# qitianwu/SGFormer

Measured on AMD Instinct MI355X. Metric: SGFormer fwd+bwd nodes/sec on ogbn-products full-graph, higher is better.
Workload: dtype bf16

## Files before the change

include/sgf.h:

```cpp
#ifndef SGF_H_
#define SGF_H_

#include <stddef.h>
#include <stdint.h>

#ifdef __cplusplus
extern "C" {
#endif

#define SGF_VERSION 670

#define SGF_F32 0
#define SGF_BF16 1
#define SGF_F32_BF16X3 2

#define SGF_OK 0
#define SGF_E_INVALID (-1)
#define SGF_E_WORKSPACE (-2)
#define SGF_E_HIP (-3)
#define SGF_E_UNSUPPORTED (-4)

int sgf_version(void);
const char* sgf_last_error(void);
int sgf_reload_env(void);

size_t sgf_csr_workspace_bytes(int64_t nnz, int64_t n);
int sgf_csr_build(const int64_t* edge_index, int64_t nnz, int64_t n, int64_t* rowptr,
                  int32_t* colind, float* val, int32_t* deg, void* workspace,
                  size_t workspace_bytes, void* stream);

int sgf_csr_transpose(const int64_t* edge_index, int64_t nnz, int64_t n, const int32_t* deg,
                      const int64_t* rowptr, const int32_t* colind, int64_t* t_rowptr,
                      int32_t* t_colind, float* t_val, int32_t* is_symmetric, void* workspace,
                      size_t workspace_bytes, void* stream);

size_t sgf_subgraph_workspace_bytes(int64_t nnz, int64_t n);
int sgf_subgraph_plan(const int64_t* edge_index, int64_t nnz, int64_t n, const int64_t* subset,
                      int64_t m, int32_t* relabel, int64_t* total, void* workspace,
                      size_t workspace_bytes, void* stream);
int sgf_subgraph_emit(const int64_t* edge_index, int64_t nnz, int64_t n, const int32_t* relabel,
                      int32_t relabel_nodes, int64_t total, int64_t* out, int64_t* out_eid,
                      void* workspace, size_t workspace_bytes, void* stream);

size_t sgf_subgraph_csr_plan_workspace_bytes(int64_t m);
size_t sgf_subgraph_csr_emit_workspace_bytes(int64_t m, int64_t total);
int sgf_subgraph_csr_plan(const int64_t* rowptr, const int32_t* colind, int64_t n, const int64_t* subset, int64_t m,
                          int32_t* local_of, int64_t* rowptr_b, int32_t* deg_b, int64_t* total, void* workspace,
                          size_t workspace_bytes, void* stream);
int sgf_subgraph_csr_emit(const int64_t* rowptr, const int32_t* colind, int64_t n, const int64_t* subset, int64_t m,
                          int32_t* local_of, const int64_t* rowptr_b, const int32_t* deg_b, int64_t total, int32_t* colind_b,
                          float* val_b, int64_t* edge_index_b, void* workspace, size_t workspace_bytes, void* stream);

size_t sgf_graph_prologue_workspace_bytes(int64_t m, int64_t n);
int sgf_graph_prologue_plan(const int64_t* edge_index, int64_t m, int64_t n, int32_t to_undirected,
                            int32_t remove_self_loops, int32_t add_self_loops, int64_t* total,
                            void* workspace, size_t workspace_bytes, void* stream);
int sgf_graph_prologue_emit(int64_t m, int64_t n, int32_t to_undirected, int32_t add_self_loops,
                            int64_t total, int64_t* out, void* workspace, size_t workspace_bytes,
                            void* stream);

int sgf_spmm(const int64_t* rowptr, const int32_t* colind, const float* val, const void* x,
             int64_t ldx, int64_t n_cols, void* y, int64_t ldy, int64_t n_rows, int32_t d,
             int32_t dtype, void* stream);

int32_t sgf_spmm_segment_len(void);
int32_t sgf_spmm_arm(int32_t d, int32_t dtype, int64_t ldx, int64_t ldy, int64_t n_cols, int32_t aligned16,
                     int32_t stream);
size_t sgf_spmm_split_workspace_bytes(int64_t long_segments, int32_t d);
int sgf_spmm_split(const int64_t* rowptr, const int32_t* colind, const float* val, const void* x,
                   int64_t ldx, int64_t n_cols, void* y, int64_t ldy, int64_t n_rows, int32_t d, int32_t dtype,
                   int64_t long_len, int64_t long_segments, void* workspace, size_t workspace_bytes,
                   void* stream);

size_t sgf_spmm_packed_bytes(int64_t n, int32_t slot_bytes);
int32_t sgf_spmm_packed_supported(int32_t d, int32_t dtype, int64_t ldx, int64_t ldy, int64_t n_cols, int32_t aligned16,
                                  int32_t slot_bytes);
int sgf_spmm_packed(const int64_t* rowptr, const int32_t* colind, const float* val, const void* x, int64_t ldx,
                    int64_t n_cols, const void* packed, int32_t slot_bytes, const int32_t* overflow, void* y, int64_t ldy,
                    int64_t n_rows, int32_t d, int32_t dtype, int64_t long_len, int64_t long_segments, void* workspace,
                    size_t workspace_bytes, void* stream);

int sgf_spmm_stream(const int64_t* rowptr, const int32_t* colind, const float* val, const void* x,
                    int64_t ldx, int64_t n_cols, void* y, int64_t ldy, int64_t n_rows, int32_t d, int32_t dtype,
                    int64_t long_len, int64_t long_segments, void* workspace, size_t workspace_bytes,
                    void* stream);

size_t sgf_reorder_workspace_bytes(int64_t nnz, int64_t n);
int sgf_reorder(const int64_t* edge_index, int64_t nnz, int64_t n, int32_t iters1, int32_t iters2,
                int32_t* perm, int32_t* inv, int32_t* community, void* workspace, size_t workspace_bytes,
                void* stream);
size_t sgf_spmm_plan_workspace_bytes(int64_t nnz, int64_t n, int32_t rows_per_block);
int sgf_spmm_plan(const int64_t* rowptr, const int32_t* colind, const float* val, int64_t n, int64_t nnz,
                  int32_t rows_per_block, int32_t lds_rows, int64_t long_len, int32_t* ecode, float* eval,
                  int32_t* nlds, int32_t* sh_ptr, int32_t* sh_cols, int64_t* stats, void* workspace,
                  size_t workspace_bytes, void* stream);
int32_t sgf_spmm_lds_rows_len(int32_t dtype);
int32_t sgf_spmm_blocked_arm(int32_t d, int32_t dtype, int64_t ldx, int64_t ldy, int64_t n_rows, int32_t rows_per_block,
                             int32_t lds_rows, int32_t aligned16);
int sgf_spmm_blocked(const int64_t* rowptr, const int32_t* ecode, const float* eval, const int32_t* nlds,
                     const int32_t* sh_ptr, const int32_t* sh_cols, const void* x, int64_t ldx, void* y,
                     int64_t ldy, int64_t n_rows, int32_t d, int32_t dtype, int32_t rows_per_block,
                     int32_t lds_rows, int64_t long_len, int64_t long_segments, void* workspace,
                     size_t workspace_bytes, void* stream);

int sgf_spmm_tile_supported(int32_t d, int32_t dtype);
int sgf_spmm_tile_blocks(const int32_t* comm_sorted, int64_t n, int32_t max_rows, int32_t* blk_row,
                         int64_t blk_cap, int64_t* nb_out, void* stream);
size_t sgf_spmm_tile_plan_workspace_bytes(int64_t nnz, int64_t n, int64_t nb);
int sgf_spmm_tile_plan(const int64_t* rowptr, const int32_t* colind, const float* val, int64_t n, int64_t nnz,
                       const int32_t* blk_row, int64_t nb, int32_t cap, int32_t min_count, int64_t long_len,
                       int32_t* ecode, float* eval, int32_t* nlds, int32_t* sh_ptr, int32_t* sh_cols,
                       int64_t* tile_ptr, int64_t* rem_rowptr, int64_t* stats, void* workspace,
                       size_t workspace_bytes, void* stream);
int sgf_spmm_tile_fill(const int64_t* rowptr, const int32_t* ecode, const float* eval, const int32_t* nlds,
                       int64_t n, int64_t nnz, const int32_t* blk_row, int64_t nb, const int64_t* tile_ptr,
                       int64_t n_frag, const int64_t* rem_rowptr, void* tiles, int32_t* rem_col, float* rem_val,
                       void* stream);
int32_t sgf_spmm_tile_sparse_len(void);
size_t sgf_spmm_tile_pack_workspace_bytes(int64_t n_frag);
int sgf_spmm_tile_pack_layout(const int32_t* blk_row, int64_t nb, const int64_t* tile_ptr, const void* tiles,
                              int64_t n_frag, int32_t* grp, int64_t* pool_units, void* workspace,
                              size_t workspace_bytes, void* stream);
int sgf_spmm_tile_pack(const int32_t* blk_row, int64_t nb, const int64_t* tile_ptr, const void* tiles, int64_t n_frag,
                       const int32_t* grp, void* pool, int64_t pool_units, void* stream);
int sgf_spmm_tile(const int32_t* blk_row, int64_t nb, int32_t block_rows, const int32_t* sh_ptr, const int32_t* sh_cols,
                  const int64_t* tile_ptr, const int32_t* grp, const void* pool, const int64_t* rem_rowptr,
                  const int32_t* rem_col, const float* rem_val, const void* x, int64_t ldx, int64_t n_cols, void* y, int64_t ldy,
                  int64_t n_rows, int32_t d, int32_t dtype, int64_t long_len, int64_t long_segments,
                  void* workspace, size_t workspace_bytes, void* stream);

size_t sgf_neighbor_sample_workspace_bytes(int64_t m, int64_t edge_cap);
int sgf_neighbor_sample_mark(int32_t* local_of, const int32_t* ids, int64_t count, int32_t base, void* stream);
int sgf_neighbor_sample_hop(const int64_t* rowptr, const int32_t* colind, const int32_t* frontier, int64_t m,
                            int32_t frontier_local0, int32_t fanout, uint64_t seed, uint64_t batch, int32_t hop,
                            int32_t* local_of, int32_t n_known, int64_t edge_cap, int32_t* edge_src_local,
                            int32_t* edge_dst_local, int32_t* src_global, int32_t* new_nodes, int64_t* counts,
                            void* workspace, size_t workspace_bytes, void* stream);

size_t sgf_neighbor_sample_batch_workspace_bytes(int64_t batch_size, const int32_t* fanouts, int32_t hops, int64_t* node_cap,
                                                  int64_t* edge_cap);
int sgf_neighbor_sample_batch(const int64_t* rowptr, const int32_t* colind, const int32_t* seeds, int64_t batch_size,
                              const int32_t* fanouts, int32_t hops, uint64_t seed, uint64_t batch, int32_t* local_of,
                              int32_t* nodes, int64_t node_cap, int32_t* edge_src_local, int32_t* edge_dst_local,
                              int64_t edge_cap, int64_t* counts, void* workspace, size_t workspace_bytes, void* stream);

int32_t sgf_sampled_csr_supported(int32_t max_fanout);
size_t sgf_sampled_csr_build_workspace_bytes(int64_t node_cap, int64_t edge_cap);
int sgf_sampled_csr_build(const int32_t* edge_src_local, const int32_t* edge_dst_local, const int64_t* counts,
                          int64_t node_cap, int64_t edge_cap, int32_t max_fanout, int64_t* rowptr_b, int32_t* colind_b,
                          float* val_b, int32_t* deg_b, void* workspace, size_t workspace_bytes, void* stream);
size_t sgf_sampled_csr_transpose_workspace_bytes(int64_t n, int64_t nnz);
int sgf_sampled_csr_transpose(const int64_t* rowptr, const int32_t* colind, const float* val, int64_t n, int64_t nnz,
                              int64_t* t_rowptr, int32_t* t_colind, float* t_val, void* workspace, size_t workspace_bytes,
                              void* stream);

int sgf_gather_rows(const void* src, int64_t lds, int32_t src_dtype, int64_t n_src, const void* idx,
                    int32_t idx_is_int64, int64_t n_out, int32_t d, void* dst, int64_t ldd,
                    int32_t dst_dtype, void* stream);
int sgf_pad_rows(const void* src, int64_t lds, int32_t src_dtype, int64_t n_src, const void* idx, int32_t idx_is_int64,
                 int64_t n_out, int32_t d, int32_t d_pad, void* dst, int64_t ldd, int32_t dst_dtype, void* stream);

int64_t sgf_attn_stats_len(int32_t heads, int32_t d);
size_t sgf_attn_workspace_bytes(int64_t n, int32_t heads, int32_t d);
int32_t sgf_attn_max_blocks(void);
int32_t sgf_attn_tile_rows(int32_t kind, int32_t d, int32_t dtype);

int sgf_attn_fwd_reduce(const void* q, int64_t ldq, const void* k, int64_t ldk, const void* v,
                        int64_t ldv, int64_t n, int32_t heads, int32_t v_heads, int32_t d,
                        int32_t dtype, float* stats, void* workspace, size_t workspace_bytes,
                        void* stream);

int sgf_attn_fwd_apply(const void* q, int64_t ldq, const void* v, int64_t ldv, int64_t n,
                       double n_total, int32_t heads, int32_t v_heads, int32_t d, int32_t dtype,
                       const float* stats, void* out, int64_t ldo, float* den, void* o_heads,
                       void* stream);

int64_t sgf_attn_bstats_len(int32_t heads, int32_t d);

int sgf_attn_bwd_reduce(const void* q, int64_t ldq, const void* g, int64_t ldg, const void* o,
                        int64_t ldo, const float* den, int64_t n, int32_t heads, int32_t d,
                        int32_t dtype, float* bstats, void* workspace, size_t workspace_bytes,
                        void* stream);

int sgf_attn_bwd_apply(const void* q, int64_t ldq, const void* k, int64_t ldk, const void* v,
                       int64_t ldv, const void* g, int64_t ldg, const void* o, int64_t ldo,
                       const float* den, int64_t n, double n_total, int32_t heads,
                       int32_t v_heads, int32_t d, int32_t dtype, const float* stats,
                       float* bstats, void* dq, int64_t lddq, void* dk, int64_t lddk,
                       void* dv, int64_t lddv, void* stream);
int sgf_attn_bwd_reduce_heads(const void* q, int64_t ldq, const void* g, int64_t ldg, const void* o, int64_t ldo,
                              const float* den, int64_t n, int32_t heads, int32_t d, int32_t dtype, float* bstats,
                              void* workspace, size_t workspace_bytes, void* stream);
int sgf_attn_bwd_apply_heads(const void* q, int64_t ldq, const void* k, int64_t ldk, const void* v, int64_t ldv, const void* g,
                             int64_t ldg, const void* o, int64_t ldo, const float* den, int64_t n, double n_total,
                             int32_t heads, int32_t v_heads, int32_t d, int32_t dtype, const float* stats, float* bstats,
                             void* dq, int64_t lddq, void* dk, int64_t lddk, void* dv, int64_t lddv, void* stream);

int64_t sgf_attn_h_bstats_len(int32_t d);
int32_t sgf_attn_h_supported(int32_t d, int32_t dtype);
int sgf_attn_h_fwd(const void* h, int64_t ldh, int64_t n, int32_t d, int32_t dtype, const float* M,
                   const float* m, const float* w, const float* beta, void* out, int64_t ldo,
                   float* den, void* stream);
int sgf_attn_h_bwd_reduce(const void* h, int64_t ldh, const void* g, int64_t ldg, const void* o,
                          int64_t ldo, const float* den, int64_t n, int32_t d, int32_t dtype,
                          float* hstats, void* workspace, size_t workspace_bytes, void* stream);
int sgf_attn_h_bwd_apply(const void* h, int64_t ldh, const void* g, int64_t ldg, const void* o,
                         int64_t ldo, const float* den, int64_t n, int32_t d, int32_t dtype,
                         const float* M, const float* w, const float* D, const float* ds, void* dh,
                         int64_t lddh, void* workspace, size_t workspace_bytes, void* stream);
size_t sgf_attn_h_bwd_apply_workspace_bytes(int64_t n, int32_t d, int32_t dtype);
int32_t sgf_attn_h_bwd_split_supported(int32_t d, int32_t dtype);
int sgf_attn_h_bwd_pre(const void* g, int64_t ldg, const void* o, int64_t ldo, const float* den, int64_t n, int32_t d,
                       int32_t dtype, const float* M, const float* w, void* workspace, size_t workspace_bytes,
                       float* rowscal, void* stream);
int sgf_attn_h_bwd_reduce_scaled(const void* h, int64_t ldh, const void* g, int64_t ldg, const float* rowscal, int64_t n,
                                 int32_t d, int32_t dtype, float* hstats, void* workspace, size_t workspace_bytes,
                                 void* stream);
int sgf_attn_h_bwd_post(const void* h, int64_t ldh, int64_t n, int32_t d, int32_t dtype, const float* D, const float* ds,
                        const void* workspace, size_t workspace_bytes, const void* addend, int64_t ldadd, void* dh,
                        int64_t lddh, void* stream);

size_t sgf_attn_h_small_saved_bytes(int32_t d_in, int32_t d_out);
size_t sgf_attn_h_small_workspace_bytes(int32_t d_in, int32_t d_out);
int sgf_attn_h_small_fwd(const float* G, int64_t ldg, const float* s, float n_rows, float n_total, const float* wq,
                         const float* bq, const float* wk, const float* bk, const float* wv, const float* bv, int64_t ldw,
                         int32_t d_in, int32_t d_out, float* M, int64_t ldm, float* m, float* w, float* beta, void* saved,
                         size_t saved_bytes, void* stream);
int sgf_attn_h_small_bwd(const float* dM, int64_t lddm, const float* dw, const float* dm, const float* dbeta, float n_total,
                         int32_t d_in, int32_t d_out, const void* saved, size_t saved_bytes, float* dG2, int64_t lddg,
                         float* ds, float* gwq, float* gbq, float* gwk, float* gbk, float* gwv, float* gbv, int64_t ldgw,
                         void* workspace, size_t workspace_bytes, void* stream);

size_t sgf_gram_workspace_bytes(int64_t n, int32_t m, int32_t k);
int sgf_gram(const void* a, int64_t lda, int32_t m, const void* b, int64_t ldb, int32_t k,
             int64_t n, int32_t dtype, float* c, int64_t ldc, float* colsum_a, void* workspace,
             size_t workspace_bytes, void* stream);
int sgf_gram2(const void* a, int64_t lda, int32_t m, const void* b1, int64_t ldb1, const void* b2, int64_t ldb2, int32_t k,
              int64_t n, int32_t dtype, float* c1, int64_t ldc1, float* c2, int64_t ldc2, float* colsum_a, void* workspace,
              size_t workspace_bytes, void* stream);

int sgf_ln_fwd(const void* x, int64_t ldx, const void* res, int64_t ldr, float a, float b,
               const float* gamma, const float* beta, int32_t relu, float eps, int64_t n,
               int32_t d, int32_t dtype, void* y, int64_t ldy, float* mean, float* rstd,
               void* stream);

size_t sgf_ln_bwd_workspace_bytes(int64_t n, int32_t d);
int sgf_ln_bwd(const void* dy, int64_t lddy, const void* y, int64_t ldy, const void* x,
               int64_t ldx, const void* res, int64_t ldr, float a, float b, const float* gamma,
               int32_t relu, const float* mean, const float* rstd, int64_t n, int32_t d,
               int32_t dtype, void* dx, int64_t lddx, void* dres, int64_t lddres, float* dgamma,
               float* dbeta, void* workspace, size_t workspace_bytes, void* stream);

size_t sgf_colstats_workspace_bytes(int64_t n, int32_t d);
int sgf_colstats(const void* x, int64_t ldx, const float* shift, int64_t n, int32_t d,
                 int32_t dtype, float* stats, void* workspace, size_t workspace_bytes,
                 void* stream);
int sgf_bn_finalize(const float* sums, const float* shift, double n_total, float eps, float momentum, float* running_mean,
                    float* running_var, int32_t d, float* mean, float* rstd, void* stream);
int sgf_bn_apply(const void* x, int64_t ldx, const float* mean, const float* rstd,
                 const float* gamma, const float* beta, const void* res, int64_t ldr,
                 int32_t relu, int64_t n, int32_t d, int32_t dtype, void* y, int64_t ldy,
                 void* stream);
int sgf_bn_apply_packed(const void* x, int64_t ldx, const float* mean, const float* rstd, const float* gamma,
                        const float* beta, const void* res, int64_t ldr, int32_t relu, int64_t n, int32_t d, int32_t dtype,
                        void* y, int64_t ldy, void* packed, int32_t slot_bytes, int32_t* overflow, void* stream);
int sgf_bn_bwd_stats(const void* dy, int64_t lddy, const void* x, int64_t ldx, const float* mean,
                     const float* rstd, const float* gamma, const float* beta, int32_t relu,
                     int64_t n, int32_t d, int32_t dtype, float* stats, void* workspace,
                     size_t workspace_bytes, void* stream);
int sgf_bn_bwd_stats2(const void* dy, int64_t lddy, const void* dy2, int64_t lddy2, const void* x, int64_t ldx,
                      const float* mean, const float* rstd, const float* gamma, const float* beta, int32_t relu, int64_t n,
                      int32_t d, int32_t dtype, float* stats, void* workspace, size_t workspace_bytes, void* stream);
int32_t sgf_gram_ln_bwd_supported(int32_t m, int32_t k, int32_t dtype);
int sgf_gram_ln_bwd(const void* g, int64_t ldg, const void* xin, int64_t ldx, const float* mean, const float* rstd,
                    const float* gamma, const float* beta, int32_t relu, int32_t m, const void* b, int64_t ldb, int32_t k,
                    int64_t n, int32_t dtype, float* c, int64_t ldc, float* colsum, float* dgamma, float* dbeta, void* workspace,
                    size_t workspace_bytes, void* stream);
int32_t sgf_gram_bn_bwd_supported(int32_t m, int32_t k, int32_t dtype);
int sgf_gram_bn_bwd(const void* g1, int64_t ldg1, const void* g2, int64_t ldg2, const void* z, int64_t ldz, const float* mean,
                    const float* rstd, const float* gamma, const float* beta, int32_t relu, const float* stats, float inv_n,
                    int32_t training, int32_t m, const void* b, int64_t ldb, int32_t k, int64_t n, int32_t dtype, float* c,
                    int64_t ldc, float* colsum, void* workspace, size_t workspace_bytes, void* stream);
int32_t sgf_gram2_bn_bwd_supported(int32_t m, int32_t k, int64_t n, int32_t dtype);
int sgf_gram2_bn_bwd(const void* g, int64_t ldg, const void* z, int64_t ldz, const float* mean, const float* rstd,
                     const float* gamma, const float* beta, int32_t relu, const float* stats, float inv_n, int32_t training,
                     int32_t m, const void* b1, int64_t ldb1, const void* b2, int64_t ldb2, int32_t k, int64_t n, int32_t dtype,
                     void* dz, int64_t lddz, float* c1, int64_t ldc1, float* c2, int64_t ldc2, float* colsum, void* workspace,
                     size_t workspace_bytes, void* stream);
int sgf_bn_bwd_apply(const void* dy, int64_t lddy, const void* x, int64_t ldx, const float* mean,
                     const float* rstd, const float* gamma, const float* beta, int32_t relu,
                     const float* stats, float inv_n, int32_t training, int64_t n, int32_t d,
                     int32_t dtype, void* dx, int64_t lddx, void* stream);

int32_t sgf_combine_fc_supported(int32_t d, int32_t classes, int32_t dtype);
int sgf_combine_fc_fwd(const void* x1, int64_t ld1, float a, const void* x2, int64_t ld2, float b,
                       const float* w, const float* bias, int64_t n, int32_t d, int32_t classes,
                       int32_t dtype, float* logits, int64_t ldl, void* stream);
int sgf_combine_fc_bwd(const float* dlogits, int64_t lddl, const float* w, int64_t n, int32_t d,
                       int32_t classes, float a, float b, int32_t dtype, void* dx1, int64_t ld1, void* dx2,
                       int64_t ld2, void* stream);
int sgf_combine_fc_fwd_mapped(const void* x1, int64_t ld1, float a, const void* x2, int64_t ld2, float b, const float* w,
                              const float* bias, int64_t n, int32_t d, int32_t classes, int32_t dtype, float* logits,
                              int64_t ldl, const int32_t* row_map, void* stream);
int sgf_combine_fc_bwd_mapped(const float* dlogits, int64_t lddl, const float* w, int64_t n, int32_t d, int32_t classes,
                              float a, float b, int32_t dtype, void* dx1, int64_t ld1, void* dx2, int64_t ld2,
                              const int32_t* row_map, void* stream);
int sgf_combine_fc_bwd_g(const float* dlogits, int64_t lddl, const float* w, int64_t n, int32_t d, int32_t classes, float a,
                         float b, int32_t dtype, void* dx1, int64_t ld1, void* dx2, int64_t ld2, const int32_t* row_map,
                         void* g_out, int64_t ldg, void* stream);

int32_t sgf_gcn_epilogue_supported(int32_t d_in, int32_t d_out, int32_t dtype);
size_t sgf_gcn_epilogue_workspace_bytes(int64_t n, int32_t d_out);
int sgf_gcn_epilogue_stats(const void* a, int64_t lda, const void* w, int64_t ldw, const float* bias,
                           int64_t n, int32_t d_in, int32_t d_out, int32_t dtype, void* y, int64_t ldy,
                           const float* shift, float* stats, void* workspace, size_t workspace_bytes,
                           void* stream);
int sgf_gcn_epilogue_dx2(const void* dy, int64_t lddy, const void* w1, const void* w2, int64_t ldw, int64_t n, int32_t d,
                         int32_t dtype, void* dx1, int64_t lddx1, void* dx2, int64_t lddx2, int32_t pair, void* stream);

int32_t sgf_gcn_epilogue_dx2_acc_supported(int32_t d, int32_t dtype);
int sgf_gcn_epilogue_dx2_acc(const void* dz, int64_t lddz, const void* w, int64_t ldw, int64_t n, int32_t d, int32_t dtype,
                             void* dy, int64_t lddy, const void* gadd, int64_t ldg, const void* acc_in, int64_t ldai,
                             void* acc_out, int64_t ldao, void* stream);
int sgf_gcn_epilogue_dx(const void* dy, int64_t lddy, const void* w, int64_t ldw, int64_t n, int32_t d_in,
                        int32_t d_out, int32_t dtype, void* dx, int64_t lddx, void* stream);
int sgf_gcn_epilogue_apply(const void* y, int64_t ldy, const float* mean, const float* rstd, const float* gamma,
                           const float* beta, const void* res, int64_t ldr, int32_t relu, int64_t n, int32_t d,
                           int32_t dtype, void* out, int64_t ldo, void* stream);
int32_t sgf_gcn_bn_bwd_dx_supported(int32_t d, int32_t dtype);
size_t sgf_gcn_bn_bwd_dx_workspace_bytes(int64_t n, int32_t d);
int sgf_gcn_bn_bwd_dx(const void* gy, int64_t ldg, const void* z, int64_t ldz, const float* mean, const float* rstd,
                      const float* gamma, const float* beta, int32_t relu, const float* stats, float inv_n,
                      int32_t training, const void* w, int64_t ldw, int64_t n, int32_t d, int32_t dtype, void* dz,
                      int64_t lddz, void* dy, int64_t lddy, const void* acc_in, void* acc_out, size_t acc_bytes,
                      void* dx0, int64_t lddx0, int32_t add_gy, void* workspace, size_t workspace_bytes, void* stream);
int32_t sgf_gcn_epilogue_cat_supported(int32_t d, int32_t dtype);
int sgf_gcn_epilogue_cat(const void* a1, int64_t lda1, const void* a2, int64_t lda2, const void* w, int64_t ldw,
                         const float* bias, int64_t n, int32_t d, int32_t dtype, void* y, int64_t ldy, const float* shift,
                         float* stats, void* workspace, size_t workspace_bytes, void* stream);
size_t sgf_gcn_epilogue_partial_bytes(int64_t n, int32_t d_out);
size_t sgf_gcn_epilogue_dtype_partial_bytes(int64_t n, int32_t d_out, int32_t dtype);
int sgf_gcn_epilogue_partial(const void* a, int64_t lda, const void* w, int64_t ldw, const float* bias, int64_t n,
                             int32_t d_in, int32_t d_out, int32_t dtype, void* partial, size_t partial_bytes,
                             void* stream);
int sgf_gcn_epilogue_stats_add(const void* a, int64_t lda, const void* w, int64_t ldw, const void* partial,
                               size_t partial_bytes, int64_t n, int32_t d_in, int32_t d_out, int32_t dtype,
                               void* y, int64_t ldy, const float* shift, float* stats, void* workspace,
                               size_t workspace_bytes, void* stream);

int32_t sgf_stem_pair_supported(int32_t d_in, int32_t d_out, int32_t dtype);
int32_t sgf_row_lap_rows(int32_t kind, int32_t d, int32_t dtype);
int sgf_stem_pair(const void* x, int64_t ldx, int64_t n, int32_t d_in, const void* w0, int64_t ldw0,
                  const float* bias0, const void* w1, int64_t ldw1, const float* bias1, int32_t d_out, int32_t dtype,
                  void* y0, int64_t ldy0, void* y1, int64_t ldy1, const float* shift0, float* stats0, void* workspace,
                  size_t workspace_bytes, void* stream);

int sgf_gemm(const void* a, int64_t a_rs, int64_t a_cs, int32_t a_dtype, const void* b, int64_t b_rs, int64_t b_cs,
             int32_t b_dtype, int64_t m, int32_t n, int64_t k, float alpha, const float* alpha_dev, const float* bias,
             float beta, const void* addend, int64_t ldadd, int32_t add_dtype, void* c, int64_t ldc, int32_t c_dtype,
             void* stream);

int sgf_axpby(const void* x1, int64_t ld1, float a, const void* x2, int64_t ld2, float b,
              int64_t n, int32_t d, int32_t dtype, void* y, int64_t ldy, void* stream);

int sgf_dropout(const void* x, int64_t ldx, const void* res, int64_t ldr, float p, uint64_t seed,
                int64_t n, int32_t d, int32_t dtype, void* y, int64_t ldy, void* stream);

int sgf_dropout_dev(const void* x, int64_t ldx, const void* res, int64_t ldr, float p,
                    const uint64_t* seed_slot, int64_t n, int32_t d, int32_t dtype, void* y, int64_t ldy,
                    void* stream);

size_t sgf_nll_workspace_bytes(int64_t m);
int sgf_nll_fwd(const void* logits, int64_t ldl, int64_t n, int32_t c, int32_t dtype,
                const int64_t* labels, const int64_t* idx, int64_t m, float* loss_sum,
                void* workspace, size_t workspace_bytes, void* stream);
int sgf_nll_bwd(const void* logits, int64_t ldl, int64_t n, int32_t c, int32_t dtype,
                const int64_t* labels, const int64_t* idx, int64_t m, const float* gout,
                float inv_denom, void* dlogits, int64_t ldd, void* stream);

#define SGF_BCE_TARGET_F32 0
#define SGF_BCE_TARGET_I64 1
#define SGF_BCE_TARGET_CLASS 2
size_t sgf_bce_workspace_bytes(int64_t m, int32_t c);
// ... 130 lines not shown
```

sgformer_amd/_lib.py:

```python
from __future__ import annotations

import ctypes
import os
from ctypes import c_char_p, c_double, c_float, c_int32, c_int64, c_size_t, c_uint64, c_void_p

_HERE = os.path.dirname(os.path.abspath(__file__))
LIB_PATH = os.path.join(_HERE, "lib", "libsgf.so")

SGF_F32 = 0
SGF_BF16 = 1
SGF_F32_BF16X3 = 2
SGF_OK = 0
SGF_E_INVALID = -1
SGF_E_WORKSPACE = -2
SGF_E_HIP = -3
SGF_E_UNSUPPORTED = -4
SGF_BCE_TARGET_F32 = 0
SGF_BCE_TARGET_I64 = 1
SGF_BCE_TARGET_CLASS = 2
SGF_METRIC_TARGET_F32 = 0
SGF_METRIC_TARGET_I64 = 1

_lib = None

_P = c_void_p
SIGNATURES = {
    "sgf_version": (c_int32, []),
    "sgf_last_error": (c_char_p, []),
    "sgf_reload_env": (c_int32, []),
    "sgf_csr_workspace_bytes": (c_size_t, [c_int64, c_int64]),
    "sgf_csr_build": (c_int32, [_P, c_int64, c_int64, _P, _P, _P, _P, _P, c_size_t, _P]),
    "sgf_csr_transpose": (c_int32, [_P, c_int64, c_int64, _P, _P, _P, _P, _P, _P, _P, _P, c_size_t, _P]),
    "sgf_subgraph_workspace_bytes": (c_size_t, [c_int64, c_int64]),
    "sgf_subgraph_plan": (c_int32, [_P, c_int64, c_int64, _P, c_int64, _P, _P, _P, c_size_t, _P]),
    "sgf_subgraph_emit": (c_int32, [_P, c_int64, c_int64, _P, c_int32, c_int64, _P, _P, _P, c_size_t, _P]),
    "sgf_subgraph_csr_plan_workspace_bytes": (c_size_t, [c_int64]),
    "sgf_subgraph_csr_emit_workspace_bytes": (c_size_t, [c_int64, c_int64]),
    "sgf_subgraph_csr_plan": (c_int32, [_P, _P, c_int64, _P, c_int64, _P, _P, _P, _P, _P, c_size_t, _P]),
    "sgf_subgraph_csr_emit": (c_int32, [_P, _P, c_int64, _P, c_int64, _P, _P, _P, c_int64, _P, _P, _P, _P, c_size_t, _P]),
    "sgf_graph_prologue_workspace_bytes": (c_size_t, [c_int64, c_int64]),
    "sgf_graph_prologue_plan": (c_int32, [_P, c_int64, c_int64, c_int32, c_int32, c_int32, _P, _P, c_size_t, _P]),
    "sgf_graph_prologue_emit": (c_int32, [c_int64, c_int64, c_int32, c_int32, c_int64, _P, _P, c_size_t, _P]),
    "sgf_spmm": (c_int32, [_P, _P, _P, _P, c_int64, c_int64, _P, c_int64, c_int64, c_int32, c_int32, _P]),
    "sgf_spmm_segment_len": (c_int32, []),
    "sgf_spmm_arm": (c_int32, [c_int32, c_int32, c_int64, c_int64, c_int64, c_int32, c_int32]),
    "sgf_spmm_split_workspace_bytes": (c_size_t, [c_int64, c_int32]),
    "sgf_spmm_split": (c_int32, [_P, _P, _P, _P, c_int64, c_int64, _P, c_int64, c_int64, c_int32, c_int32, c_int64,
                                 c_int64, _P, c_size_t, _P]),
    "sgf_spmm_packed_bytes": (c_size_t, [c_int64, c_int32]),
    "sgf_spmm_packed_supported": (c_int32, [c_int32, c_int32, c_int64, c_int64, c_int64, c_int32, c_int32]),
    "sgf_spmm_packed": (c_int32, [_P, _P, _P, _P, c_int64, c_int64, _P, c_int32, _P, _P, c_int64, c_int64, c_int32, c_int32,
                                  c_int64, c_int64, _P, c_size_t, _P]),
    "sgf_spmm_stream": (c_int32, [_P, _P, _P, _P, c_int64, c_int64, _P, c_int64, c_int64, c_int32, c_int32, c_int64,
                                  c_int64, _P, c_size_t, _P]),
    "sgf_reorder_workspace_bytes": (c_size_t, [c_int64, c_int64]),
    "sgf_reorder": (c_int32, [_P, c_int64, c_int64, c_int32, c_int32, _P, _P, _P, _P, c_size_t, _P]),
    "sgf_spmm_plan_workspace_bytes": (c_size_t, [c_int64, c_int64, c_int32]),
    "sgf_spmm_plan": (c_int32, [_P, _P, _P, c_int64, c_int64, c_int32, c_int32, c_int64, _P, _P, _P, _P, _P, _P,
                                _P, c_size_t, _P]),
    "sgf_spmm_lds_rows_len": (c_int32, [c_int32]),
    "sgf_spmm_blocked_arm": (c_int32, [c_int32, c_int32, c_int64, c_int64, c_int64, c_int32, c_int32, c_int32]),
    "sgf_spmm_blocked": (c_int32, [_P, _P, _P, _P, _P, _P, _P, c_int64, _P, c_int64, c_int64, c_int32, c_int32,
                                   c_int32, c_int32, c_int64, c_int64, _P, c_size_t, _P]),
    "sgf_spmm_tile_supported": (c_int32, [c_int32, c_int32]),
    "sgf_spmm_tile_blocks": (c_int32, [_P, c_int64, c_int32, _P, c_int64, _P, _P]),
    "sgf_spmm_tile_plan_workspace_bytes": (c_size_t, [c_int64, c_int64, c_int64]),
    "sgf_spmm_tile_plan": (c_int32, [_P, _P, _P, c_int64, c_int64, _P, c_int64, c_int32, c_int32, c_int64, _P, _P, _P,
                                     _P, _P, _P, _P, _P, _P, c_size_t, _P]),
    "sgf_spmm_tile_fill": (c_int32, [_P, _P, _P, _P, c_int64, c_int64, _P, c_int64, _P, c_int64, _P, _P, _P, _P, _P]),
    "sgf_spmm_tile_sparse_len": (c_int32, []),
    "sgf_spmm_tile_pack_workspace_bytes": (c_size_t, [c_int64]),
    "sgf_spmm_tile_pack_layout": (c_int32, [_P, c_int64, _P, _P, c_int64, _P, _P, _P, c_size_t, _P]),
    "sgf_spmm_tile_pack": (c_int32, [_P, c_int64, _P, _P, c_int64, _P, _P, c_int64, _P]),
    "sgf_spmm_tile": (c_int32, [_P, c_int64, c_int32, _P, _P, _P, _P, _P, _P, _P, _P, _P, c_int64, c_int64, _P, c_int64,
                                c_int64, c_int32, c_int32, c_int64, c_int64, _P, c_size_t, _P]),
    "sgf_neighbor_sample_workspace_bytes": (c_size_t, [c_int64, c_int64]),
    "sgf_neighbor_sample_mark": (c_int32, [_P, _P, c_int64, c_int32, _P]),
    "sgf_neighbor_sample_batch_workspace_bytes": (c_size_t, [c_int64, _P, c_int32, _P, _P]),
    "sgf_neighbor_sample_batch": (c_int32, [_P, _P, _P, c_int64, _P, c_int32, c_uint64, c_uint64, _P, _P, c_int64, _P, _P,
                                            c_int64, _P, _P, c_size_t, _P]),
    "sgf_neighbor_sample_hop": (c_int32, [_P, _P, _P, c_int64, c_int32, c_int32, c_uint64, c_uint64, c_int32, _P, c_int32,
                                          c_int64, _P, _P, _P, _P, _P, _P, c_size_t, _P]),
    "sgf_sampled_csr_supported": (c_int32, [c_int32]),
    "sgf_sampled_csr_build_workspace_bytes": (c_size_t, [c_int64, c_int64]),
    "sgf_sampled_csr_build": (c_int32, [_P, _P, _P, c_int64, c_int64, c_int32, _P, _P, _P, _P, _P, c_size_t, _P]),
    "sgf_sampled_csr_transpose_workspace_bytes": (c_size_t, [c_int64, c_int64]),
    "sgf_sampled_csr_transpose": (c_int32, [_P, _P, _P, c_int64, c_int64, _P, _P, _P, _P, c_size_t, _P]),
    "sgf_gather_rows": (c_int32, [_P, c_int64, c_int32, c_int64, _P, c_int32, c_int64, c_int32, _P, c_int64,
                                  c_int32, _P]),
    "sgf_pad_rows": (c_int32, [_P, c_int64, c_int32, c_int64, _P, c_int32, c_int64, c_int32, c_int32, _P, c_int64,
                               c_int32, _P]),
    "sgf_attn_stats_len": (c_int64, [c_int32, c_int32]),
    "sgf_attn_bstats_len": (c_int64, [c_int32, c_int32]),
    "sgf_attn_workspace_bytes": (c_size_t, [c_int64, c_int32, c_int32]),
    "sgf_attn_max_blocks": (c_int32, []),
    "sgf_attn_tile_rows": (c_int32, [c_int32, c_int32, c_int32]),
    "sgf_row_lap_rows": (c_int32, [c_int32, c_int32, c_int32]),
    "sgf_ew_lap_rows": (c_int64, [c_int32, c_int32, c_int32, c_int32]),
    "sgf_attn_fwd_reduce": (c_int32, [_P, c_int64, _P, c_int64, _P, c_int64, c_int64, c_int32, c_int32,
                                      c_int32, c_int32, _P, _P, c_size_t, _P]),
    "sgf_attn_fwd_apply": (c_int32, [_P, c_int64, _P, c_int64, c_int64, c_double, c_int32, c_int32,
                                     c_int32, c_int32, _P, _P, c_int64, _P, _P, _P]),
    "sgf_attn_bwd_reduce": (c_int32, [_P, c_int64, _P, c_int64, _P, c_int64, _P, c_int64, c_int32,
                                      c_int32, c_int32, _P, _P, c_size_t, _P]),
    "sgf_attn_bwd_apply": (c_int32, [_P, c_int64, _P, c_int64, _P, c_int64, _P, c_int64, _P, c_int64,
                                     _P, c_int64, c_double, c_int32, c_int32, c_int32, c_int32, _P, _P,
                                     _P, c_int64, _P, c_int64, _P, c_int64, _P]),
    "sgf_attn_bwd_reduce_heads": (c_int32, [_P, c_int64, _P, c_int64, _P, c_int64, _P, c_int64, c_int32,
                                            c_int32, c_int32, _P, _P, c_size_t, _P]),
    "sgf_attn_bwd_apply_heads": (c_int32, [_P, c_int64, _P, c_int64, _P, c_int64, _P, c_int64, _P, c_int64,
                                           _P, c_int64, c_double, c_int32, c_int32, c_int32, c_int32, _P, _P,
                                           _P, c_int64, _P, c_int64, _P, c_int64, _P]),
    "sgf_attn_h_bstats_len": (c_int64, [c_int32]),
    "sgf_attn_h_fwd": (c_int32, [_P, c_int64, c_int64, c_int32, c_int32, _P, _P, _P, _P, _P, c_int64, _P, _P]),
    "sgf_attn_h_bwd_reduce": (c_int32, [_P, c_int64, _P, c_int64, _P, c_int64, _P, c_int64, c_int32, c_int32,
                                        _P, _P, c_size_t, _P]),
    "sgf_attn_h_bwd_apply": (c_int32, [_P, c_int64, _P, c_int64, _P, c_int64, _P, c_int64, c_int32, c_int32,
                                       _P, _P, _P, _P, _P, c_int64, _P, c_size_t, _P]),
    "sgf_attn_h_bwd_apply_workspace_bytes": (c_size_t, [c_int64, c_int32, c_int32]),
    "sgf_attn_h_bwd_split_supported": (c_int32, [c_int32, c_int32]),
    "sgf_attn_h_supported": (c_int32, [c_int32, c_int32]),
    "sgf_attn_h_bwd_pre": (c_int32, [_P, c_int64, _P, c_int64, _P, c_int64, c_int32, c_int32, _P, _P, _P, c_size_t, _P, _P]),
    "sgf_attn_h_bwd_reduce_scaled": (c_int32, [_P, c_int64, _P, c_int64, _P, c_int64, c_int32, c_int32, _P, _P, c_size_t,
                                               _P]),
    "sgf_attn_h_bwd_post": (c_int32, [_P, c_int64, c_int64, c_int32, c_int32, _P, _P, _P, c_size_t, _P, c_int64, _P,
                                      c_int64, _P]),
    "sgf_attn_h_small_saved_bytes": (c_size_t, [c_int32, c_int32]),
    "sgf_attn_h_small_workspace_bytes": (c_size_t, [c_int32, c_int32]),
    "sgf_attn_h_small_fwd": (c_int32, [_P, c_int64, _P, c_float, c_float, _P, _P, _P, _P, _P, _P, c_int64, c_int32, c_int32,
                                       _P, c_int64, _P, _P, _P, _P, c_size_t, _P]),
    "sgf_attn_h_small_bwd": (c_int32, [_P, c_int64, _P, _P, _P, c_float, c_int32, c_int32, _P, c_size_t, _P, c_int64, _P,
                                       _P, _P, _P, _P, _P, _P, c_int64, _P, c_size_t, _P]),
    "sgf_gram_workspace_bytes": (c_size_t, [c_int64, c_int32, c_int32]),
    "sgf_gram": (c_int32, [_P, c_int64, c_int32, _P, c_int64, c_int32, c_int64, c_int32, _P, c_int64, _P,
                           _P, c_size_t, _P]),
    "sgf_gram2": (c_int32, [_P, c_int64, c_int32, _P, c_int64, _P, c_int64, c_int32, c_int64, c_int32, _P, c_int64, _P,
                            c_int64, _P, _P, c_size_t, _P]),
    "sgf_ln_fwd": (c_int32, [_P, c_int64, _P, c_int64, c_float, c_float, _P, _P, c_int32, c_float,
                             c_int64, c_int32, c_int32, _P, c_int64, _P, _P, _P]),
    "sgf_ln_bwd_workspace_bytes": (c_size_t, [c_int64, c_int32]),
    "sgf_ln_bwd": (c_int32, [_P, c_int64, _P, c_int64, _P, c_int64, _P, c_int64, c_float, c_float, _P,
                             c_int32, _P, _P, c_int64, c_int32, c_int32, _P, c_int64, _P, c_int64, _P,
                             _P, _P, c_size_t, _P]),
    "sgf_colstats_workspace_bytes": (c_size_t, [c_int64, c_int32]),
    "sgf_colstats": (c_int32, [_P, c_int64, _P, c_int64, c_int32, c_int32, _P, _P, c_size_t, _P]),
    "sgf_bn_finalize": (c_int32, [_P, _P, c_double, c_float, c_float, _P, _P, c_int32, _P, _P, _P]),
    "sgf_bn_apply": (c_int32, [_P, c_int64, _P, _P, _P, _P, _P, c_int64, c_int32, c_int64, c_int32,
                               c_int32, _P, c_int64, _P]),
    "sgf_bn_apply_packed": (c_int32, [_P, c_int64, _P, _P, _P, _P, _P, c_int64, c_int32, c_int64, c_int32, c_int32, _P,
                                      c_int64, _P, c_int32, _P, _P]),
    "sgf_bn_bwd_stats": (c_int32, [_P, c_int64, _P, c_int64, _P, _P, _P, _P, c_int32, c_int64, c_int32,
                                   c_int32, _P, _P, c_size_t, _P]),
    "sgf_bn_bwd_stats2": (c_int32, [_P, c_int64, _P, c_int64, _P, c_int64, _P, _P, _P, _P, c_int32, c_int64, c_int32,
                                    c_int32, _P, _P, c_size_t, _P]),
    "sgf_gram_ln_bwd_supported": (c_int32, [c_int32, c_int32, c_int32]),
    "sgf_gram_ln_bwd": (c_int32, [_P, c_int64, _P, c_int64, _P, _P, _P, _P, c_int32, c_int32, _P, c_int64, c_int32, c_int64,
                                  c_int32, _P, c_int64, _P, _P, _P, _P, c_size_t, _P]),
    "sgf_gram_bn_bwd_supported": (c_int32, [c_int32, c_int32, c_int32]),
    "sgf_gram_bn_bwd": (c_int32, [_P, c_int64, _P, c_int64, _P, c_int64, _P, _P, _P, _P, c_int32, _P, c_float, c_int32,
                                  c_int32, _P, c_int64, c_int32, c_int64, c_int32, _P, c_int64, _P, _P, c_size_t, _P]),
    "sgf_gram2_bn_bwd_supported": (c_int32, [c_int32, c_int32, c_int64, c_int32]),
    "sgf_gram2_bn_bwd": (c_int32, [_P, c_int64, _P, c_int64, _P, _P, _P, _P, c_int32, _P, c_float, c_int32, c_int32, _P, c_int64,
                                   _P, c_int64, c_int32, c_int64, c_int32, _P, c_int64, _P, c_int64, _P, c_int64, _P, _P,
                                   c_size_t, _P]),
    "sgf_bn_bwd_apply": (c_int32, [_P, c_int64, _P, c_int64, _P, _P, _P, _P, c_int32, _P, c_float,
                                   c_int32, c_int64, c_int32, c_int32, _P, c_int64, _P]),
    "sgf_dropout": (c_int32, [_P, c_int64, _P, c_int64, c_float, c_uint64, c_int64, c_int32, c_int32, _P,
                              c_int64, _P]),
    "sgf_dropout_dev": (c_int32, [_P, c_int64, _P, c_int64, c_float, _P, c_int64, c_int32, c_int32, _P,
                                  c_int64, _P]),
    "sgf_nll_workspace_bytes": (c_size_t, [c_int64]),
    "sgf_nll_fwd": (c_int32, [_P, c_int64, c_int64, c_int32, c_int32, _P, _P, c_int64, _P, _P, c_size_t, _P]),
    "sgf_nll_bwd": (c_int32, [_P, c_int64, c_int64, c_int32, c_int32, _P, _P, c_int64, _P, c_float, _P,
                              c_int64, _P]),
    "sgf_bce_workspace_bytes": (c_size_t, [c_int64, c_int32]),
    "sgf_bce_fwd": (c_int32, [_P, c_int64, c_int64, c_int32, c_int32, _P, c_int64, c_int32, _P, c_int64, c_float, _P, _P,
                              c_size_t, _P]),
    "sgf_bce_bwd": (c_int32, [_P, c_int64, c_int64, c_int32, c_int32, _P, c_int64, c_int32, _P, c_int64, _P, c_float, _P,
                              c_int64, _P]),
    "sgf_rocauc_workspace_bytes": (c_size_t, [c_int64, c_int32]),
    "sgf_rocauc_counts": (c_int32, [_P, c_int64, c_int64, c_int32, c_int32, _P, c_int64, c_int32, _P, c_int64, _P, _P,
                                    c_size_t, _P]),
    "sgf_argmax_workspace_bytes": (c_size_t, [c_int64, c_int32]),
    "sgf_argmax_count": (c_int32, [_P, c_int64, c_int64, c_int32, c_int32, _P, c_int64, c_int32, _P, c_int64, _P, _P,
                                   c_size_t, _P]),
    "sgf_head_rows_supported": (c_int32, [c_int32, c_int32, c_int32]),
    "sgf_head_rows_fwd_workspace_bytes": (c_size_t, [c_int64]),
    "sgf_head_rows_bwd_workspace_bytes": (c_size_t, [c_int64, c_int32, c_int32]),
    "sgf_head_rows_fwd": (c_int32, [_P, c_int64, c_float, _P, c_int64, c_float, _P, _P, c_int64, c_int32, c_int32, c_int32,
                                    _P, c_int64, _P, c_int64, _P, _P, _P, _P, _P, c_size_t, _P]),
    "sgf_head_rows_bwd": (c_int32, [_P, c_int64, c_float, _P, c_int64, c_float, _P, c_int64, c_int32, c_int32, c_int32,
                                    _P, c_int64, _P, c_int64, _P, c_int64, _P, _P, _P, c_float, _P, c_int64, _P, c_int64,
                                    _P, _P, _P, c_size_t, _P]),
    "sgf_pair_sigmoid_supported": (c_int32, [c_int32, c_int32, c_int32, c_int32]),
    "sgf_pair_sigmoid_workspace_bytes": (c_size_t, [c_int64, c_int64, c_int32]),
    "sgf_pair_sigmoid_lap_rows": (c_int64, [c_int32, c_int32, c_int32, c_int32, c_int32]),
    "sgf_pair_sigmoid_fwd": (c_int32, [_P, c_int64, _P, c_int64, _P, c_int64, c_int64, c_int64, c_int32, c_int32, c_int32,
                                       c_int32, _P, c_int64, _P, _P]),
    "sgf_pair_sigmoid_bwd_q": (c_int32, [_P, c_int64, _P, c_int64, _P, _P, c_int64, _P, c_int64, _P, c_int64, c_int64,
                                         c_int64, c_int32, c_int32, c_int32, c_int32, _P, c_int64, _P, c_size_t, _P]),
    "sgf_pair_sigmoid_bwd_kv": (c_int32, [_P, c_int64, _P, _P, c_int64, _P, c_int64, _P, c_int64, c_int64, c_int64, c_int32,
                                          c_int32, c_int32, c_int32, _P, c_int64, _P, c_int64, _P, c_size_t, _P]),
    "sgf_pair_softmax_supported": (c_int32, [c_int32, c_int32, c_int32, c_int32]),
    "sgf_pair_softmax_workspace_bytes": (c_size_t, [c_int64, c_int64, c_int32]),
    "sgf_pair_softmax_lap_rows": (c_int64, [c_int32, c_int32, c_int32, c_int32, c_int32]),
    "sgf_pair_softmax_fwd": (c_int32, [_P, c_int64, _P, c_int64, _P, c_int64, c_int64, c_int64, c_int32, c_int32, c_int32,
                                       c_int32, c_float, _P, c_int64, _P, _P]),
    "sgf_pair_softmax_bwd_q": (c_int32, [_P, c_int64, _P, c_int64, _P, _P, c_int64, _P, c_int64, _P, c_int64, c_int64,
                                         c_int64, c_int32, c_int32, c_int32, c_int32, c_float, _P, c_int64, _P, c_size_t,
                                         _P]),
    "sgf_pair_softmax_bwd_kv": (c_int32, [_P, c_int64, _P, _P, c_int64, _P, c_int64, _P, c_int64, c_int64, c_int64, c_int32,
                                          c_int32, c_int32, c_int32, c_float, _P, c_int64, _P, c_int64, _P, c_size_t, _P]),
    "sgf_pair_sigmoid_x3_supported": (c_int32, [c_int32, c_int32, c_int32, c_int32]),
    "sgf_pair_sigmoid_x3_lap_rows": (c_int64, [c_int32, c_int32, c_int32, c_int32, c_int32]),
    "sgf_pair_sigmoid_x3_fwd": (c_int32, [_P, c_int64, _P, c_int64, _P, c_int64, c_int64, c_int64, c_int32, c_int32, c_int32,
                                          c_int32, _P, c_int64, _P, _P]),
    "sgf_pair_sigmoid_x3_bwd_q": (c_int32, [_P, c_int64, _P, c_int64, _P, _P, c_int64, _P, c_int64, _P, c_int64, c_int64,
                                            c_int64, c_int32, c_int32, c_int32, c_int32, _P, c_int64, _P, c_size_t, _P]),
    "sgf_pair_sigmoid_x3_bwd_kv": (c_int32, [_P, c_int64, _P, _P, c_int64, _P, c_int64, _P, c_int64, c_int64, c_int64, c_int32,
                                             c_int32, c_int32, c_int32, _P, c_int64, _P, c_int64, _P, c_size_t, _P]),
    "sgf_pair_softmax_x3_supported": (c_int32, [c_int32, c_int32, c_int32, c_int32]),
    "sgf_pair_softmax_x3_lap_rows": (c_int64, [c_int32, c_int32, c_int32, c_int32, c_int32]),
    "sgf_pair_softmax_x3_fwd": (c_int32, [_P, c_int64, _P, c_int64, _P, c_int64, c_int64, c_int64, c_int32, c_int32, c_int32,
                                          c_int32, c_float, _P, c_int64, _P, _P]),
    "sgf_pair_softmax_x3_bwd_q": (c_int32, [_P, c_int64, _P, c_int64, _P, _P, c_int64, _P, c_int64, _P, c_int64, c_int64,
                                            c_int64, c_int32, c_int32, c_int32, c_int32, c_float, _P, c_int64, _P, c_size_t,
                                            _P]),
    "sgf_pair_softmax_x3_bwd_kv": (c_int32, [_P, c_int64, _P, _P, c_int64, _P, c_int64, _P, c_int64, c_int64, c_int64, c_int32,
                                             c_int32, c_int32, c_int32, c_float, _P, c_int64, _P, c_int64, _P, c_size_t, _P]),
    "sgf_gat_supported": (c_int32, [c_int32, c_int32, c_int32]),
    "sgf_gat_lap_rows": (c_int64, [c_int32, c_int32, c_int32, c_int32]),
    "sgf_gat_scores": (c_int32, [_P, c_int64, _P, _P, c_int64, c_int32, c_int32, c_int32, _P, _P, _P]),
    "sgf_gat_fwd": (c_int32, [_P, _P, _P, c_int64, _P, _P, _P, c_int64, c_int64, c_int32, c_int32, c_int32, c_int32, c_float,
                              c_float, c_uint64, _P, c_int64, _P, _P, _P]),
    "sgf_gat_bwd_dst": (c_int32, [_P, _P, _P, c_int64, _P, c_int64, _P, _P, _P, c_int64, c_int64, c_int32, c_int32, c_int32,
                                  c_int32, c_float, c_float, c_uint64, _P, _P, _P]),
    "sgf_gat_bwd_src": (c_int32, [_P, _P, _P, c_int64, _P, c_int64, _P, _P, _P, _P, _P, _P, _P, c_int64, c_int64, c_int32,
                                  c_int32, c_int32, c_int32, c_float, c_float, c_uint64, _P, _P, c_int64, _P]),
    "sgf_sum_n": (c_int32, [_P, _P, c_int32, c_int64, c_int32, c_int32, _P, c_int64, _P]),
    "sgf_colsum_workspace_bytes": (c_size_t, [c_int64, c_int32]),
    "sgf_colsum": (c_int32, [_P, c_int64, c_int64, c_int32, c_int32, _P, _P, c_size_t, _P]),
    "sgf_combine_fc_supported": (c_int32, [c_int32, c_int32, c_int32]),
    "sgf_combine_fc_fwd": (c_int32, [_P, c_int64, c_float, _P, c_int64, c_float, _P, _P, c_int64, c_int32, c_int32,
                                     c_int32, _P, c_int64, _P]),
    "sgf_combine_fc_bwd": (c_int32, [_P, c_int64, _P, c_int64, c_int32, c_int32, c_float, c_float, c_int32, _P,
                                     c_int64, _P, c_int64, _P]),
    "sgf_combine_fc_fwd_mapped": (c_int32, [_P, c_int64, c_float, _P, c_int64, c_float, _P, _P, c_int64, c_int32, c_int32,
                                     c_int32, _P, c_int64, _P, _P]),
    "sgf_combine_fc_bwd_g": (c_int32, [_P, c_int64, _P, c_int64, c_int32, c_int32, c_float, c_float, c_int32, _P, c_int64, _P,
                                       c_int64, _P, _P, c_int64, _P]),
    "sgf_combine_fc_bwd_mapped": (c_int32, [_P, c_int64, _P, c_int64, c_int32, c_int32, c_float, c_float, c_int32, _P,
                                     c_int64, _P, c_int64, _P, _P]),
    "sgf_gcn_epilogue_supported": (c_int32, [c_int32, c_int32, c_int32]),
    "sgf_gcn_epilogue_workspace_bytes": (c_size_t, [c_int64, c_int32]),
    "sgf_gcn_epilogue_stats": (c_int32, [_P, c_int64, _P, c_int64, _P, c_int64, c_int32, c_int32, c_int32, _P, c_int64,
                                         _P, _P, _P, c_size_t, _P]),
    "sgf_gcn_epilogue_dx": (c_int32, [_P, c_int64, _P, c_int64, c_int64, c_int32, c_int32, c_int32, _P, c_int64, _P]),
    "sgf_gcn_epilogue_dx2": (c_int32, [_P, c_int64, _P, _P, c_int64, c_int64, c_int32, c_int32, _P, c_int64, _P, c_int64,
                                       c_int32, _P]),
    "sgf_gcn_epilogue_dx2_acc_supported": (c_int32, [c_int32, c_int32]),
    "sgf_gcn_epilogue_dx2_acc": (c_int32, [_P, c_int64, _P, c_int64, c_int64, c_int32, c_int32, _P, c_int64, _P, c_int64, _P,
                                           c_int64, _P, c_int64, _P]),
    "sgf_gcn_epilogue_apply": (c_int32, [_P, c_int64, _P, _P, _P, _P, _P, c_int64, c_int32, c_int64, c_int32,
                               c_int32, _P, c_int64, _P]),
    "sgf_gcn_bn_bwd_dx_supported": (c_int32, [c_int32, c_int32]),
    "sgf_gcn_bn_bwd_dx_workspace_bytes": (c_size_t, [c_int64, c_int32]),
    "sgf_gcn_bn_bwd_dx": (c_int32, [_P, c_int64, _P, c_int64, _P, _P, _P, _P, c_int32, _P, c_float, c_int32, _P, c_int64,
                                    c_int64, c_int32, c_int32, _P, c_int64, _P, c_int64, _P, _P, c_size_t, _P, c_int64,
                                    c_int32, _P, c_size_t, _P]),
    "sgf_gcn_epilogue_cat_supported": (c_int32, [c_int32, c_int32]),
    "sgf_gcn_epilogue_cat": (c_int32, [_P, c_int64, _P, c_int64, _P, c_int64, _P, c_int64, c_int32, c_int32, _P, c_int64,
                                       _P, _P, _P, c_size_t, _P]),
    "sgf_gcn_epilogue_partial_bytes": (c_size_t, [c_int64, c_int32]),
    "sgf_gcn_epilogue_dtype_partial_bytes": (c_size_t, [c_int64, c_int32, c_int32]),
    "sgf_gcn_epilogue_partial": (c_int32, [_P, c_int64, _P, c_int64, _P, c_int64, c_int32, c_int32, c_int32, _P,
                                           c_size_t, _P]),
    "sgf_gcn_epilogue_stats_add": (c_int32, [_P, c_int64, _P, c_int64, _P, c_size_t, c_int64, c_int32, c_int32,
                                             c_int32, _P, c_int64, _P, _P, _P, c_size_t, _P]),
    "sgf_stem_pair_supported": (c_int32, [c_int32, c_int32, c_int32]),
    "sgf_stem_pair": (c_int32, [_P, c_int64, c_int64, c_int32, _P, c_int64, _P, _P, c_int64, _P, c_int32, c_int32, _P,
                                c_int64, _P, c_int64, _P, _P, _P, c_size_t, _P]),
    "sgf_gemm": (c_int32, [_P, c_int64, c_int64, c_int32, _P, c_int64, c_int64, c_int32, c_int64, c_int32, c_int64, c_float,
                           _P, _P, c_float, _P, c_int64, c_int32, _P, c_int64, c_int32, _P]),
    "sgf_comm_available": (c_int32, []),
    "sgf_comm_unique_id_bytes": (c_int32, []),
    "sgf_comm_unique_id": (c_int32, [_P]),
    "sgf_comm_create": (c_int32, [_P, c_int32, c_int32, _P]),
    "sgf_comm_destroy": (c_int32, [_P]),
    "sgf_comm_all_reduce_f32": (c_int32, [_P, _P, c_int64, _P]),
    "sgf_comm_all_gather": (c_int32, [_P, _P, _P, c_int64, _P]),
    "sgf_comm_all_to_all": (c_int32, [_P, _P, _P, _P, _P, _P, _P, _P]),
    "sgf_axpby": (c_int32, [_P, c_int64, c_float, _P, c_int64, c_float, c_int64, c_int32, c_int32, _P,
                            c_int64, _P]),
}


class SgfError(RuntimeError):
    """A libsgf call returned a non-zero status (mirrors PyTorch: RuntimeError)."""


def load():
    global _lib
    if _lib is not None:
        return _lib
    if not os.path.exists(LIB_PATH):
        raise SgfError(
            f"libsgf.so not found at {LIB_PATH}: build it with `make` (or "
            "`python -c 'import __graft_entry__ as g; g.build()'`).  sgformer_amd has no CPU / "
            "eager fallback by design.")
    import torch
    lib = ctypes.CDLL(LIB_PATH, mode=ctypes.RTLD_GLOBAL)
    for name, (res, args) in SIGNATURES.items():
        fn = getattr(lib, name)
        fn.restype = res
        fn.argtypes = args
    _lib = lib
    return lib


def available() -> bool:
    return os.path.exists(LIB_PATH)


def check(rc: int, what: str):
    if rc != SGF_OK:
        msg = load().sgf_last_error()
        raise SgfError(f"{what} failed (rc={rc}): {msg.decode() if msg else '?'}")


def call(name: str, *args):
    rc = getattr(load(), name)(*args)
    check(rc, name)
```

sgformer_amd/csrc/spmm.hip:

```cpp
#include "common.h"
#include "spmm_shared.h"

#include <climits>
#include <cstdlib>

namespace sgf {
namespace {

constexpr int kWavesPerBlock = 4;

__device__ __forceinline__ void fma4(float4& acc, float v, const float4& x) {
  acc.x = fmaf(v, x.x, acc.x);
  acc.y = fmaf(v, x.y, acc.y);
  acc.z = fmaf(v, x.z, acc.z);
  acc.w = fmaf(v, x.w, acc.w);
}

template <typename T, int UNROLL>
__global__ __launch_bounds__(kWavesPerBlock * 64) void k_spmm_wave(
    const int64_t* __restrict__ rowptr, const int32_t* __restrict__ colind,
    const float* __restrict__ val, const T* __restrict__ x, int64_t ldx, T* __restrict__ y,
    int64_t ldy, int64_t n_rows, int32_t d, LongQueue lq) {
  const int lane = threadIdx.x & 63;
  const int wid = __builtin_amdgcn_readfirstlane(static_cast<int>(threadIdx.x >> 6));
  const int64_t blk = xcd_remap(blockIdx.x, gridDim.x);
  const int64_t row = blk * kWavesPerBlock + wid;
  if (row >= n_rows) return;
  const int64_t e0 = rowptr[row];
  const int64_t e1 = rowptr[row + 1];
  if (e1 - e0 > lq.long_len) {
    push_long_row(lq, row, e1 - e0, lane, 64);
    return;
  }

  for (int f0 = 0; f0 < d; f0 += 256) {
    const int fc = f0 + lane * 4;
    const bool active = fc < d;
    const T* xl = x + (active ? fc : 0);
    float4 acc = make_float4(0.f, 0.f, 0.f, 0.f);
    int64_t e = e0;
    for (; e + UNROLL <= e1; e += UNROLL) {
      int32_t c[UNROLL];
      float v[UNROLL];
      float4 xv[UNROLL];
#pragma unroll
      for (int u = 0; u < UNROLL; ++u) {
        c[u] = colind[e + u];
        v[u] = val[e + u];
      }
#pragma unroll
      for (int u = 0; u < UNROLL; ++u)
        xv[u] = load4<T>(xl + static_cast<int64_t>(c[u]) * ldx);
#pragma unroll
      for (int u = 0; u < UNROLL; ++u) fma4(acc, v[u], xv[u]);
    }
    for (; e < e1; ++e) {
      const int32_t c = colind[e];
      const float v = val[e];
      const float4 xv = load4<T>(xl + static_cast<int64_t>(c) * ldx);
      fma4(acc, v, xv);
    }
    if (active) store4<T>(y + row * ldy + fc, acc);
  }
}

template <typename T> struct BufRow;
template <> struct BufRow<uint16_t> {
  using Raw = u32x2;
  static __device__ __forceinline__ Raw load(__amdgpu_buffer_rsrc_t r, int voff, uint32_t soff) {
    return __builtin_amdgcn_raw_buffer_load_b64(r, voff, static_cast<int>(soff), 0);
  }
  static __device__ __forceinline__ float4 widen(const Raw& v) {
    float4 f;
    f.x = __uint_as_float(v.x << 16);
    f.y = __uint_as_float(v.x & 0xffff0000u);
    f.z = __uint_as_float(v.y << 16);
    f.w = __uint_as_float(v.y & 0xffff0000u);
    return f;
  }
};
template <> struct BufRow<float> {
  using Raw = u32x4;
  static __device__ __forceinline__ Raw load(__amdgpu_buffer_rsrc_t r, int voff, uint32_t soff) {
    return __builtin_amdgcn_raw_buffer_load_b128(r, voff, static_cast<int>(soff), 0);
  }
  static __device__ __forceinline__ float4 widen(const Raw& v) {
    return make_float4(__uint_as_float(v.x), __uint_as_float(v.y), __uint_as_float(v.z), __uint_as_float(v.w));
  }
};

template <typename T, int N>
__device__ __forceinline__ void gather_batch(__amdgpu_buffer_rsrc_t rsrc, int voff, uint32_t pitch,
                                             const int32_t* __restrict__ colind, const float* __restrict__ val,
                                             int e, float4& acc) {
  int32_t c[N];
  float v[N];
  typename BufRow<T>::Raw raw[N];
#pragma unroll
  for (int u = 0; u < N; ++u) {
    c[u] = colind[e + u];
    v[u] = val[e + u];
  }
#pragma unroll
  for (int u = 0; u < N; ++u) raw[u] = BufRow<T>::load(rsrc, voff, static_cast<uint32_t>(c[u]) * pitch);
#pragma unroll
  for (int u = 0; u < N; ++u) fma4(acc, v[u], BufRow<T>::widen(raw[u]));
}

template <typename T, int UNROLL>
__global__ __launch_bounds__(kWavesPerBlock * 64) void k_spmm_row(
    const int64_t* __restrict__ rowptr, const int32_t* __restrict__ colind, const float* __restrict__ val,
    const T* __restrict__ x, uint32_t pitch, uint32_t x_bytes, T* __restrict__ y, int64_t ldy, int64_t n_rows,
    int32_t d, LongQueue lq) {
  const int lane = threadIdx.x & 63;
  const int wid = __builtin_amdgcn_readfirstlane(static_cast<int>(threadIdx.x >> 6));
  const int64_t blk = xcd_remap(blockIdx.x, gridDim.x);
  const int64_t row = blk * kWavesPerBlock + wid;
  if (row >= n_rows) return;
  const int64_t e0 = rowptr[row];
  const int64_t e1 = rowptr[row + 1];
  if (e1 - e0 > lq.long_len) {
    push_long_row(lq, row, e1 - e0, lane, 64);
    return;
  }
  const __amdgpu_buffer_rsrc_t rsrc = __builtin_amdgcn_make_buffer_rsrc(const_cast<T*>(x), 0, x_bytes, 0x00020000);
  const int fc = lane * 4;
  const bool active = fc < d;
  const int voff = active ? fc * static_cast<int>(sizeof(T)) : 0;
  float4 acc = make_float4(0.f, 0.f, 0.f, 0.f);
  const int32_t* __restrict__ ci = colind + e0;
  const float* __restrict__ va = val + e0;
  const int len = static_cast<int>(e1 - e0);
  int i = 0;
  if (UNROLL <= len) {
    int32_t c0[UNROLL], c1[UNROLL];
    float v0[UNROLL], v1[UNROLL];
    typename BufRow<T>::Raw raw[UNROLL];
#pragma unroll
    for (int u = 0; u < UNROLL; ++u) {
      c0[u] = ci[u];
      v0[u] = va[u];
    }
    for (;;) {
#pragma unroll
      for (int u = 0; u < UNROLL; ++u) raw[u] = BufRow<T>::load(rsrc, voff, static_cast<uint32_t>(c0[u]) * pitch);
      i += UNROLL;
      const bool more_a = i + UNROLL <= len;
      if (more_a) {
#pragma unroll
        for (int u = 0; u < UNROLL; ++u) {
          c1[u] = ci[i + u];
          v1[u] = va[i + u];
        }
      }
#pragma unroll
      for (int u = 0; u < UNROLL; ++u) fma4(acc, v0[u], BufRow<T>::widen(raw[u]));
      if (!more_a) break;
#pragma unroll
      for (int u = 0; u < UNROLL; ++u) raw[u] = BufRow<T>::load(rsrc, voff, static_cast<uint32_t>(c1[u]) * pitch);
      i += UNROLL;
      const bool more_b = i + UNROLL <= len;
      if (more_b) {
#pragma unroll
        for (int u = 0; u < UNROLL; ++u) {
          c0[u] = ci[i + u];
          v0[u] = va[i + u];
        }
      }
#pragma unroll
      for (int u = 0; u < UNROLL; ++u) fma4(acc, v1[u], BufRow<T>::widen(raw[u]));
      if (!more_b) break;
    }
  }
  if (i + 4 <= len) { gather_batch<T, 4>(rsrc, voff, pitch, ci, va, i, acc); i += 4; }
  if (i + 2 <= len) { gather_batch<T, 2>(rsrc, voff, pitch, ci, va, i, acc); i += 2; }
  if (i < len) gather_batch<T, 1>(rsrc, voff, pitch, ci, va, i, acc);
  if (active) store4<T>(y + row * ldy + fc, acc);
}

typedef uint32_t u32x3 __attribute__((ext_vector_type(3)));
constexpr int kPackedMaskBytes = 32;
constexpr int kPackedTail = 128;

struct DenseRowLoader {
  static constexpr bool kAhead = false;
  __amdgpu_buffer_rsrc_t rsrc;
  int voff;
  uint32_t pitch;
  template <int N> struct Batch { u32x2 raw[N]; };
  template <int N> __device__ __forceinline__ void request(Batch<N>& b, const int32_t (&c)[N]) const {
#pragma unroll
    for (int u = 0; u < N; ++u) b.raw[u] = BufRow<uint16_t>::load(rsrc, voff, static_cast<uint32_t>(c[u]) * pitch);
  }
  template <int N> __device__ __forceinline__ void follow(Batch<N>&) const {}
  template <int N> __device__ __forceinline__ void apply(const Batch<N>& b, const float (&v)[N], float4& acc) const {
#pragma unroll
    for (int u = 0; u < N; ++u) fma4(acc, v[u], BufRow<uint16_t>::widen(b.raw[u]));
  }
};

template <int S>
struct PackedRowLoader {
  static constexpr bool kAhead = true;
  __amdgpu_buffer_rsrc_t rsrc;
  int mask_voff;
  int shift;
  uint32_t below;
  const uint4* lut;
  template <int N> struct Batch {
    uint32_t slot[N], mw[N], pre[N];
    u32x3 raw[N];
  };
  template <int N> __device__ __forceinline__ void request(Batch<N>& b, const int32_t (&c)[N]) const {
#pragma unroll
    for (int u = 0; u < N; ++u) {
      b.slot[u] = static_cast<uint32_t>(c[u]) * static_cast<uint32_t>(S);
      b.mw[u] = __builtin_amdgcn_raw_buffer_load_b32(rsrc, mask_voff, static_cast<int>(b.slot[u]), 0);
    }
  }
  template <int N> __device__ __forceinline__ void follow(Batch<N>& b) const {
#pragma unroll
    for (int u = 0; u < N; ++u) {
      const int t = __popc(b.mw[u]);
      int s = t + __builtin_amdgcn_update_dpp(0, t, 0x118, 0xf, 0xf, true);
      s += __builtin_amdgcn_update_dpp(0, s, 0x142, 0xa, 0xf, false);
      s += __builtin_amdgcn_update_dpp(0, s, 0x143, 0xc, 0xf, false);
      b.pre[u] = static_cast<uint32_t>(s - t) + __popc(b.mw[u] & below);
      const uint32_t off = ((b.pre[u] & ~1u) << 1) + (b.slot[u] + kPackedMaskBytes);
      b.raw[u] = __builtin_amdgcn_raw_buffer_load_b96(rsrc, static_cast<int>(off), 0, 0);
    }
  }
  template <int N> __device__ __forceinline__ void apply(const Batch<N>& b, const float (&v)[N], float4& acc) const {
#pragma unroll
    for (int u = 0; u < N; ++u) {
      const uint4 sel = lut[(b.mw[u] >> shift) & 15u];
      const uint32_t sh = b.pre[u] << 4;
      const uint32_t lo = __builtin_amdgcn_alignbit(b.raw[u].y, b.raw[u].x, sh);
      const uint32_t hi = __builtin_amdgcn_alignbit(b.raw[u].z, b.raw[u].y, sh);
      float4 f;
      f.x = __uint_as_float(__builtin_amdgcn_perm(hi, lo, sel.x));
      f.y = __uint_as_float(__builtin_amdgcn_perm(hi, lo, sel.y));
      f.z = __uint_as_float(__builtin_amdgcn_perm(hi, lo, sel.z));
      f.w = __uint_as_float(__builtin_amdgcn_perm(hi, lo, sel.w));
      fma4(acc, v[u], f);
    }
  }
};

template <int N, typename L>
__device__ __forceinline__ void gather_batch_with(const L& ld, const int32_t* __restrict__ colind,
                                                  const float* __restrict__ val, int e, float4& acc) {
  int32_t c[N];
  float v[N];
  typename L::template Batch<N> b;
#pragma unroll
  for (int u = 0; u < N; ++u) {
    c[u] = colind[e + u];
    v[u] = val[e + u];
  }
  ld.request(b, c);
  ld.follow(b);
  ld.apply(b, v, acc);
}

template <int UNROLL, typename L>
__device__ __forceinline__ float4 walk_row(const L& ld, const int32_t* __restrict__ ci, const float* __restrict__ va, int len) {
  float4 acc = make_float4(0.f, 0.f, 0.f, 0.f);
  int i = 0;
  if (UNROLL <= len) {
    int32_t c0[UNROLL], c1[UNROLL];
    float v0[UNROLL], v1[UNROLL];
    typename L::template Batch<UNROLL> ba, bb;
#pragma unroll
    for (int u = 0; u < UNROLL; ++u) {
      c0[u] = ci[u];
      v0[u] = va[u];
    }
    ld.request(ba, c0);
    for (;;) {
      i += UNROLL;
      const bool more_a = i + UNROLL <= len;
      if (more_a) {
#pragma unroll
        for (int u = 0; u < UNROLL; ++u) {
          c1[u] = ci[i + u];
          v1[u] = va[i + u];
        }
      }
      ld.follow(ba);
      if (L::kAhead && more_a) ld.request(bb, c1);
      ld.apply(ba, v0, acc);
      if (!more_a) break;
      if (!L::kAhead) ld.request(bb, c1);
      i += UNROLL;
      const bool more_b = i + UNROLL <= len;
      if (more_b) {
#pragma unroll
        for (int u = 0; u < UNROLL; ++u) {
          c0[u] = ci[i + u];
          v0[u] = va[i + u];
        }
      }
      ld.follow(bb);
      if (L::kAhead && more_b) ld.request(ba, c0);
      ld.apply(bb, v1, acc);
      if (!more_b) break;
      if (!L::kAhead) ld.request(ba, c0);
    }
  }
  if (i + 4 <= len) { gather_batch_with<4>(ld, ci, va, i, acc); i += 4; }
  if (i + 2 <= len) { gather_batch_with<2>(ld, ci, va, i, acc); i += 2; }
  if (i < len) gather_batch_with<1>(ld, ci, va, i, acc);
  return acc;
}

template <int S, int UNROLL>
__global__ __launch_bounds__(kWavesPerBlock * 64) void k_spmm_row_packed(
    const int64_t* __restrict__ rowptr, const int32_t* __restrict__ colind, const float* __restrict__ val,
    const uint16_t* __restrict__ x, uint32_t pitch, uint32_t x_bytes, const void* __restrict__ packed, uint32_t packed_bytes,
    const int32_t* __restrict__ overflow, uint16_t* __restrict__ y, int64_t ldy, int64_t n_rows, LongQueue lq) {
  __shared__ uint4 lut[16];
  if (threadIdx.x < 16) {
    uint32_t s[4];
#pragma unroll
    for (int k = 0; k < 4; ++k) {
      const uint32_t i = __popc(threadIdx.x & ((1u << k) - 1u));
      s[k] = (threadIdx.x >> k) & 1u ? ((2u * i + 1u) << 24) | ((2u * i) << 16) | 0x0c0cu : 0x0c0c0c0cu;
    }
    lut[threadIdx.x] = make_uint4(s[0], s[1], s[2], s[3]);
  }
  __syncthreads();
  const int lane = threadIdx.x & 63;
  const int wid = __builtin_amdgcn_readfirstlane(static_cast<int>(threadIdx.x >> 6));
  const int64_t blk = xcd_remap(blockIdx.x, gridDim.x);
  const int64_t row = blk * kWavesPerBlock + wid;
  if (row >= n_rows) return;
  const int64_t e0 = rowptr[row];
  const int64_t e1 = rowptr[row + 1];
  if (e1 - e0 > lq.long_len) {
    push_long_row(lq, row, e1 - e0, lane, 64);
    return;
  }
  const int32_t* __restrict__ ci = colind + e0;
  const float* __restrict__ va = val + e0;
  const int len = static_cast<int>(e1 - e0);
  float4 acc;
  if (*overflow == 0) {
    PackedRowLoader<S> ld;
    ld.rsrc = __builtin_amdgcn_make_buffer_rsrc(const_cast<void*>(packed), 0, packed_bytes, 0x00020000);
    ld.mask_voff = (lane >> 3) * 4;
    ld.shift = (lane & 7) * 4;
    ld.below = (1u << ld.shift) - 1u;
    ld.lut = lut;
    acc = walk_row<UNROLL>(ld, ci, va, len);
  } else {
    DenseRowLoader ld;
    ld.rsrc = __builtin_amdgcn_make_buffer_rsrc(const_cast<uint16_t*>(x), 0, x_bytes, 0x00020000);
    ld.voff = lane * 8;
    ld.pitch = pitch;
    acc = walk_row<UNROLL>(ld, ci, va, len);
  }
  store4<uint16_t>(y + row * ldy + lane * 4, acc);
}

constexpr int kSegRows = 4;

template <typename T, int G>
__global__ __launch_bounds__(kWavesPerBlock * 64) void k_spmm_seg(
    const int64_t* __restrict__ rowptr, const int32_t* __restrict__ colind, const float* __restrict__ val,
    const T* __restrict__ x, uint32_t pitch, uint32_t x_bytes, T* __restrict__ y, int64_t ldy, int64_t n_rows,
    int32_t d, int32_t chunk_blocks, LongQueue lq) {
  using Raw = typename BufRow<T>::Raw;
  const int lane = threadIdx.x & 63;
  const int wid = __builtin_amdgcn_readfirstlane(static_cast<int>(threadIdx.x >> 6));
  const int64_t blk = xcd_remap(blockIdx.x, gridDim.x, chunk_blocks);
  const int64_t r_first = (blk * kWavesPerBlock + wid) * kSegRows;
  if (r_first >= n_rows) return;
  const int nr = n_rows - r_first < kSegRows ? static_cast<int>(n_rows - r_first) : kSegRows;
  const __amdgpu_buffer_rsrc_t rsrc = __builtin_amdgcn_make_buffer_rsrc(const_cast<T*>(x), 0, x_bytes, 0x00020000);
  const int fc = lane * 4;
  const bool active = fc < d;
  const int voff = active ? fc * static_cast<int>(sizeof(T)) : 0;
  T* __restrict__ yl = y + r_first * ldy + (active ? fc : 0);

  const int64_t e_first = rowptr[r_first];
  const int64_t end_abs = rowptr[r_first + 1 + (lane < nr ? lane : nr - 1)];
  const int64_t begin_abs = __shfl_up(end_abs, 1, 64);
  const int64_t len_i = end_abs - (lane == 0 ? e_first : begin_abs);
  const bool long_i = lane < nr && len_i > lq.long_len;
  auto lane64 = [&](int64_t v, int i) -> int64_t {
    const uint32_t lo = __builtin_amdgcn_readlane(static_cast<int>(v & 0xffffffff), i);
    const uint32_t hi = __builtin_amdgcn_readlane(static_cast<int>(v >> 32), i);
    return static_cast<int64_t>((static_cast<uint64_t>(hi) << 32) | lo);
  };
  const int64_t total64 = lane64(end_abs, nr - 1) - e_first;
  const int32_t* __restrict__ ci = colind + e_first;
  const float* __restrict__ va = val + e_first;

  if (__ballot(long_i) != 0 || total64 >= (static_cast<int64_t>(1) << 31)) {
    for (int r = 0; r < nr; ++r) {
      const int64_t re = lane64(end_abs, r);
      const int64_t rb = r == 0 ? e_first : lane64(end_abs, r - 1);
      if (re - rb > lq.long_len) {
        push_long_row(lq, r_first + r, re - rb, lane, 64);
        continue;
      }
      float4 acc = make_float4(0.f, 0.f, 0.f, 0.f);
      for (int64_t e = rb; e < re; ++e)
        fma4(acc, val[e], BufRow<T>::widen(BufRow<T>::load(rsrc, voff, static_cast<uint32_t>(colind[e]) * pitch)));
      if (active) store4<T>(yl + r * ldy, acc);
    }
    return;
  }

  const int rel_v = static_cast<int>(end_abs - e_first);
  const int total = static_cast<int>(total64);
  int row = 0;
  int row_end = __builtin_amdgcn_readlane(rel_v, 0);
  float4 acc = make_float4(0.f, 0.f, 0.f, 0.f);
  auto boundary = [&](int p) {
    while (p == row_end && row < nr) {
      if (active) store4<T>(yl + row * ldy, acc);
      acc = make_float4(0.f, 0.f, 0.f, 0.f);
      ++row;
      row_end = row < nr ? __builtin_amdgcn_readlane(rel_v, row < kSegRows ? row : kSegRows - 1) : 0x7fffffff;
    }
  };

  int pos = 0;
  int32_t c0[G], c1[G];
  float v0[G], v1[G];
  Raw raw[G];
  if (G <= total) {
#pragma unroll
    for (int u = 0; u < G; ++u) {
      c0[u] = ci[u];
      v0[u] = va[u];
    }
    for (;;) {
#pragma unroll
      for (int u = 0; u < G; ++u) raw[u] = BufRow<T>::load(rsrc, voff, static_cast<uint32_t>(c0[u]) * pitch);
      const bool more_a = pos + 2 * G <= total;
      if (more_a) {
#pragma unroll
        for (int u = 0; u < G; ++u) {
          c1[u] = ci[pos + G + u];
          v1[u] = va[pos + G + u];
        }
      }
#pragma unroll
      for (int u = 0; u < G; ++u) {
        if (pos + u == row_end) boundary(pos + u);
        fma4(acc, v0[u], BufRow<T>::widen(raw[u]));
      }
      pos += G;
      if (!more_a) break;
#pragma unroll
      for (int u = 0; u < G; ++u) raw[u] = BufRow<T>::load(rsrc, voff, static_cast<uint32_t>(c1[u]) * pitch);
      const bool more_b = pos + 2 * G <= total;
      if (more_b) {
#pragma unroll
        for (int u = 0; u < G; ++u) {
          c0[u] = ci[pos + G + u];
          v0[u] = va[pos + G + u];
        }
      }
#pragma unroll
      for (int u = 0; u < G; ++u) {
        if (pos + u == row_end) boundary(pos + u);
        fma4(acc, v1[u], BufRow<T>::widen(raw[u]));
      }
      pos += G;
      if (!more_b) break;
    }
  }
  if (pos < total) {
    const int g = total - pos;
#pragma unroll
    for (int u = 0; u < G; ++u) {
      const int p = pos + (u < g ? u : g - 1);
      c0[u] = ci[p];
      v0[u] = va[p];
    }
#pragma unroll
    for (int u = 0; u < G; ++u) raw[u] = BufRow<T>::load(rsrc, voff, static_cast<uint32_t>(c0[u]) * pitch);
#pragma unroll
    for (int u = 0; u < G; ++u) {
      if (u < g) {
        if (pos + u == row_end) boundary(pos + u);
        fma4(acc, v0[u], BufRow<T>::widen(raw[u]));
      }
    }
    pos = total;
  }
  boundary(total);
}

template <int G>
__global__ __launch_bounds__(kWavesPerBlock * 64) void k_spmm_seg_bf16x2(
    const int64_t* __restrict__ rowptr, const int32_t* __restrict__ colind, const float* __restrict__ val,
    const uint16_t* __restrict__ x, uint32_t pitch, uint32_t x_bytes, uint16_t* __restrict__ y, int64_t ldy,
    int64_t n_rows, int32_t d, int32_t chunk_blocks, LongQueue lq) {
  constexpr int P = G / 2;
  const int lane = threadIdx.x & 63;
  const int wid = __builtin_amdgcn_readfirstlane(static_cast<int>(threadIdx.x >> 6));
  const int64_t blk = xcd_remap(blockIdx.x, gridDim.x, chunk_blocks);
  const int64_t r_first = (blk * kWavesPerBlock + wid) * kSegRows;
  if (r_first >= n_rows) return;
  const int nr = n_rows - r_first < kSegRows ? static_cast<int>(n_rows - r_first) : kSegRows;
  const __amdgpu_buffer_rsrc_t rsrc =
      __builtin_amdgcn_make_buffer_rsrc(const_cast<uint16_t*>(x), 0, x_bytes, 0x00020000);
  const int q = lane & 31;
  const bool hi = lane >= 32;
  const uint32_t hmask = hi ? 0xffffffffu : 0u;
  const int fc = q * 8;
  const bool active = fc < d;
  const uint32_t lanebase = active ? static_cast<uint32_t>(fc) * 2u : 0u;
  uint16_t* __restrict__ yl = y + r_first * ldy + (active ? fc : 0);

  auto lane64 = [&](int64_t v, int i) -> int64_t {
    const uint32_t lo = __builtin_amdgcn_readlane(static_cast<int>(v & 0xffffffff), i);
    const uint32_t hi32 = __builtin_amdgcn_readlane(static_cast<int>(v >> 32), i);
    return static_cast<int64_t>((static_cast<uint64_t>(hi32) << 32) | lo);
  };
  const int64_t e_first = rowptr[r_first];
  const int64_t end_abs = rowptr[r_first + 1 + (lane < nr ? lane : nr - 1)];
  const int64_t begin_abs = __shfl_up(end_abs, 1, 64);
  const int64_t len_i = end_abs - (lane == 0 ? e_first : begin_abs);
  const bool long_i = lane < nr && len_i > lq.long_len;
  const int64_t total64 = lane64(end_abs, nr - 1) - e_first;
  const int32_t* __restrict__ ci = colind + e_first;
  const float* __restrict__ va = val + e_first;

  float acc[8];
#pragma unroll
  for (int k = 0; k < 8; ++k) acc[k] = 0.f;
  auto fma8 = [&](float v, const u32x4& r) {
    acc[0] = fmaf(v, __uint_as_float(r.x << 16), acc[0]);
    acc[1] = fmaf(v, __uint_as_float(r.x & 0xffff0000u), acc[1]);
    acc[2] = fmaf(v, __uint_as_float(r.y << 16), acc[2]);
    acc[3] = fmaf(v, __uint_as_float(r.y & 0xffff0000u), acc[3]);
    acc[4] = fmaf(v, __uint_as_float(r.z << 16), acc[4]);
    acc[5] = fmaf(v, __uint_as_float(r.z & 0xffff0000u), acc[5]);
    acc[6] = fmaf(v, __uint_as_float(r.w << 16), acc[6]);
    acc[7] = fmaf(v, __uint_as_float(r.w & 0xffff0000u), acc[7]);
  };
  auto flush_row = [&](int local_row) {
    float t[8];
#pragma unroll
    for (int k = 0; k < 8; ++k) t[k] = acc[k] + __shfl_xor(acc[k], 32, 64);
    if (active && !hi) {
      uint4 o;
      o.x = static_cast<uint32_t>(f32_to_bf16(t[0])) | (static_cast<uint32_t>(f32_to_bf16(t[1])) << 16);
      o.y = static_cast<uint32_t>(f32_to_bf16(t[2])) | (static_cast<uint32_t>(f32_to_bf16(t[3])) << 16);
      o.z = static_cast<uint32_t>(f32_to_bf16(t[4])) | (static_cast<uint32_t>(f32_to_bf16(t[5])) << 16);
      o.w = static_cast<uint32_t>(f32_to_bf16(t[6])) | (static_cast<uint32_t>(f32_to_bf16(t[7])) << 16);
      *reinterpret_cast<uint4*>(yl + local_row * ldy) = o;
    }
#pragma unroll
    for (int k = 0; k < 8; ++k) acc[k] = 0.f;
  };
  auto pair_load = [&](int32_t ca, int32_t cb) -> u32x4 {
    const uint32_t sa = static_cast<uint32_t>(ca) * pitch, sb = static_cast<uint32_t>(cb) * pitch;
    const uint32_t voff = lanebase + (sa ^ ((sa ^ sb) & hmask));
    return __builtin_amdgcn_raw_buffer_load_b128(rsrc, static_cast<int>(voff), 0, 0);
  };
  auto pick = [&](float a, float b) -> float {
    const uint32_t ua = __float_as_uint(a), ub = __float_as_uint(b);
    return __uint_as_float(ua ^ ((ua ^ ub) & hmask));
  };

  if (__ballot(long_i) != 0 || total64 >= (static_cast<int64_t>(1) << 31)) {
    for (int r = 0; r < nr; ++r) {
      const int64_t re = lane64(end_abs, r);
      const int64_t rb = r == 0 ? e_first : lane64(end_abs, r - 1);
      if (re - rb > lq.long_len) {
        push_long_row(lq, r_first + r, re - rb, lane, 64);
        continue;
      }
      for (int64_t e = rb; e < re; ++e) {
        const u32x4 raw = pair_load(colind[e], colind[e]);
        if (!hi) fma8(val[e], raw);
      }
      flush_row(r);
    }
    return;
  }

  const int rel_v = static_cast<int>(end_abs - e_first);
  const int total = static_cast<int>(total64);
  int row = 0;
  int row_end = __builtin_amdgcn_readlane(rel_v, 0);
  auto boundary = [&](int p) {
    while (p == row_end && row < nr) {
      flush_row(row);
      ++row;
      row_end = row < nr ? __builtin_amdgcn_readlane(rel_v, row < kSegRows ? row : kSegRows - 1) : 0x7fffffff;
    }
  };
  auto apply_pair = [&](int p, float v_a, float v_b, const u32x4& raw) {
    if (p == row_end) boundary(p);
    if (p + 1 == row_end) {
      if (!hi) fma8(v_a, raw);
      boundary(p + 1);
      if (hi) fma8(v_b, raw);
    } else {
      fma8(pick(v_a, v_b), raw);
    }
  };

  int pos = 0;
  int32_t c0[G], c1[G];
  float v0[G], v1[G];
  u32x4 raw[P];
  if (G <= total) {
#pragma unroll
    for (int u = 0; u < G; ++u) {
      c0[u] = ci[u];
      v0[u] = va[u];
    }
    for (;;) {
#pragma unroll
      for (int j = 0; j < P; ++j) raw[j] = pair_load(c0[2 * j], c0[2 * j + 1]);
      const bool more_a = pos + 2 * G <= total;
      if (more_a) {
#pragma unroll
        for (int u = 0; u < G; ++u) {
          c1[u] = ci[pos + G + u];
          v1[u] = va[pos + G + u];
        }
      }
#pragma unroll
      for (int j = 0; j < P; ++j) apply_pair(pos + 2 * j, v0[2 * j], v0[2 * j + 1], raw[j]);
      pos += G;
      if (!more_a) break;
#pragma unroll
      for (int j = 0; j < P; ++j) raw[j] = pair_load(c1[2 * j], c1[2 * j + 1]);
      const bool more_b = pos + 2 * G <= total;
      if (more_b) {
#pragma unroll
        for (int u = 0; u < G; ++u) {
          c0[u] = ci[pos + G + u];
          v0[u] = va[pos + G + u];
        }
      }
#pragma unroll
      for (int j = 0; j < P; ++j) apply_pair(pos + 2 * j, v1[2 * j], v1[2 * j + 1], raw[j]);
      pos += G;
      if (!more_b) break;
    }
  }
  if (pos < total) {
    const int g = total - pos;
#pragma unroll
    for (int u = 0; u < G; ++u) {
      const int p = pos + (u < g ? u : g - 1);
      c0[u] = ci[p];
      v0[u] = u < g ? va[p] : 0.f;
    }
#pragma unroll
    for (int j = 0; j < P; ++j) raw[j] = pair_load(c0[2 * j], c0[2 * j + 1]);
#pragma unroll
    for (int j = 0; j < P; ++j) {
// ... 315 lines not shown

constexpr int kBlk2Stage = 8;

template <int DG, int LB>
__global__ __launch_bounds__(512, 2) void k_spmm_blk2(
    const int64_t* __restrict__ rowptr, const int32_t* __restrict__ ecode, const float* __restrict__ eval,
    const int32_t* __restrict__ nlds, const int32_t* __restrict__ sh_ptr, const int32_t* __restrict__ sh_cols,
    const uint16_t* __restrict__ x, uint32_t pitch, uint32_t x_bytes, uint16_t* __restrict__ y, int64_t ldy,
    int64_t n_rows, int32_t d, int32_t rows_per_block, int32_t lds_rows, int32_t chunk_blocks, LongQueue lq,
    int32_t dbg) {
  extern __shared__ __align__(16) unsigned char smem_raw[];
  unsigned char* const tile = smem_raw;
  const int lane = threadIdx.x & 63;
  const int wid = __builtin_amdgcn_readfirstlane(static_cast<int>(threadIdx.x >> 6));
  const int nw = static_cast<int>(blockDim.x >> 6);
  uint2* const scratch = reinterpret_cast<uint2*>(smem_raw + static_cast<size_t>(lds_rows) * 512) + wid * (2 * kPiece);
  const int64_t blk = xcd_remap(blockIdx.x, gridDim.x, chunk_blocks);
  const int q = lane & 31;
  const int hi = lane >> 5;
  const bool active = q * 8 < d;
  const uint32_t lanebase = active ? static_cast<uint32_t>(q) * 16u : 0u;
  const __amdgpu_buffer_rsrc_t rsrc =
      __builtin_amdgcn_make_buffer_rsrc(const_cast<uint16_t*>(x), 0, x_bytes, 0x00020000);
  auto row_load = [&](uint32_t col) -> u32x4 {
    return __builtin_amdgcn_raw_buffer_load_b128(rsrc, static_cast<int>(col * pitch + lanebase), 0, 0);
  };

  const int s0 = sh_ptr[blk];
  const int ns = sh_ptr[blk + 1] - s0;
  for (int u0 = 2 * wid; u0 < ns && !(dbg & 1); u0 += 2 * nw * kBlk2Stage) {
    u32x4 r[kBlk2Stage];
#pragma unroll
    for (int k = 0; k < kBlk2Stage; ++k) {
      const int u = u0 + 2 * nw * k + hi;
      const int uu = u < ns ? u : ns - 1;
      r[k] = row_load(static_cast<uint32_t>(sh_cols[s0 + uu]));
    }
#pragma unroll
    for (int k = 0; k < kBlk2Stage; ++k) {
      const int u = u0 + 2 * nw * k + hi;
      if (u < ns) *reinterpret_cast<u32x4*>(tile + u * 512 + q * 16) = r[k];
    }
  }
  __syncthreads();

  const int64_t r_first = blk * rows_per_block + static_cast<int64_t>(wid) * kBlkRowsPerWave;
  if (r_first >= n_rows) return;
  const int nr = n_rows - r_first < kBlkRowsPerWave ? static_cast<int>(n_rows - r_first) : kBlkRowsPerWave;
  const int64_t nnz = rowptr[n_rows];
  const int64_t rp_v = rowptr[r_first + (lane < nr ? lane : nr)];
  const int32_t nl_v = nlds[r_first + (lane < nr ? lane : nr - 1)];
  auto rp = [&](int i) -> int64_t {
    const uint32_t lo = __builtin_amdgcn_readlane(static_cast<int>(rp_v & 0xffffffff), i);
    const uint32_t hi32 = __builtin_amdgcn_readlane(static_cast<int>(rp_v >> 32), i);
    return static_cast<int64_t>((static_cast<uint64_t>(hi32) << 32) | lo);
  };
  uint16_t* const yl = y + (active ? q * 8 : 0);
  auto store_row = [&](int64_t row, const float (&a)[8]) {
    float t[8];
#pragma unroll
    for (int k = 0; k < 8; ++k) t[k] = a[k] + __shfl_xor(a[k], 32, 64);
    if (active && !hi) {
      uint4 o;
      o.x = static_cast<uint32_t>(f32_to_bf16(t[0])) | (static_cast<uint32_t>(f32_to_bf16(t[1])) << 16);
      o.y = static_cast<uint32_t>(f32_to_bf16(t[2])) | (static_cast<uint32_t>(f32_to_bf16(t[3])) << 16);
      o.z = static_cast<uint32_t>(f32_to_bf16(t[4])) | (static_cast<uint32_t>(f32_to_bf16(t[5])) << 16);
      o.w = static_cast<uint32_t>(f32_to_bf16(t[6])) | (static_cast<uint32_t>(f32_to_bf16(t[7])) << 16);
      *reinterpret_cast<uint4*>(yl + row * ldy) = o;
    }
  };

  int it_i = -1;
  int64_t it_p = 0, it_e1 = 0;
  auto next_piece = [&]() {
    it_p += kPiece;
    while (it_p >= it_e1) {
      ++it_i;
      if (it_i >= nr) return false;
      const int64_t e0 = rp(it_i), e1 = rp(it_i + 1);
      if (e1 - e0 > lq.long_len) {
        push_long_row(lq, r_first + it_i, e1 - e0, lane, 64);
        continue;
      }
      if (e1 == e0) {
        if (active && !hi) *reinterpret_cast<uint4*>(yl + (r_first + it_i) * ldy) = make_uint4(0u, 0u, 0u, 0u);
        continue;
      }
      it_p = e0;
      it_e1 = e1;
    }
    return true;
  };
  auto fetch = [&](int64_t p) -> uint2 {
    int64_t i = p + lane;
    if (i >= nnz) i = nnz - 1;
    return make_uint2(static_cast<uint32_t>(ecode[i]), __float_as_uint(eval[i]));
  };

  it_p = -kPiece;
  it_e1 = -kPiece;
  if (!next_piece()) return;
  uint2 pre = fetch(it_p);
  int buf = 0;
  float acc[8];
#pragma unroll
  for (int k = 0; k < 8; ++k) acc[k] = 0.f;
  auto fma8 = [&](float v, const u32x4& r) {
    acc[0] = fmaf(v, __uint_as_float(r.x << 16), acc[0]);
    acc[1] = fmaf(v, __uint_as_float(r.x & 0xffff0000u), acc[1]);
    acc[2] = fmaf(v, __uint_as_float(r.y << 16), acc[2]);
    acc[3] = fmaf(v, __uint_as_float(r.y & 0xffff0000u), acc[3]);
    acc[4] = fmaf(v, __uint_as_float(r.z << 16), acc[4]);
    acc[5] = fmaf(v, __uint_as_float(r.z & 0xffff0000u), acc[5]);
    acc[6] = fmaf(v, __uint_as_float(r.w << 16), acc[6]);
    acc[7] = fmaf(v, __uint_as_float(r.w & 0xffff0000u), acc[7]);
  };
  for (;;) {
    const int ci = it_i;
    const int64_t cp = it_p, ce1 = it_e1;
    uint2* const sc = scratch + buf * kPiece;
    sc[lane] = pre;
    __builtin_amdgcn_fence(__ATOMIC_RELEASE, "wavefront");
    __builtin_amdgcn_wave_barrier();
    __builtin_amdgcn_fence(__ATOMIC_ACQUIRE, "wavefront");
    const bool more = next_piece();
    if (more) pre = fetch(it_p);

    const int64_t e0 = rp(ci);
    const int64_t el = e0 + __builtin_amdgcn_readlane(nl_v, ci);
    const int len = ce1 - cp < kPiece ? static_cast<int>(ce1 - cp) : kPiece;
    const int l1x = el > cp ? (el - cp < len ? static_cast<int>(el - cp) : len) : 0;
    const int d0 = l1x;
    const int l1 = (dbg & 2) ? 0 : l1x;
    if (cp == e0) {
#pragma unroll
      for (int k = 0; k < 8; ++k) acc[k] = 0.f;
    }
    auto get = [&](int i, int b) -> uint2 {
      const int idx = i + hi;
      uint2 c = sc[idx < b ? idx : b - 1];
      if (idx >= b) c.y = 0u;
      return c;
    };

    uint2 cv[DG];
    u32x4 xv[DG];
    const int ng = (dbg & 4) ? 0 : len - d0;
    if (ng > 0) {
#pragma unroll
      for (int u = 0; u < DG; ++u) cv[u] = get(d0 + 2 * u, len);
#pragma unroll
      for (int u = 0; u < DG; ++u) xv[u] = row_load(cv[u].x);
    }
    for (int j = 0; j < l1; j += 2 * LB) {
      uint2 c[LB];
      u32x4 t[LB];
#pragma unroll
      for (int u = 0; u < LB; ++u) c[u] = get(j + 2 * u, l1);
#pragma unroll
      for (int u = 0; u < LB; ++u)
        t[u] = *reinterpret_cast<const u32x4*>(tile + (c[u].x & 0x7fffffffu) * 512 + q * 16);
#pragma unroll
      for (int u = 0; u < LB; ++u) fma8(__uint_as_float(c[u].y), t[u]);
    }
    if (ng > 0) {
#pragma unroll
      for (int u = 0; u < DG; ++u) fma8(__uint_as_float(cv[u].y), xv[u]);
      for (int g = d0 + 2 * DG; g < len; g += 2 * DG) {
#pragma unroll
        for (int u = 0; u < DG; ++u) cv[u] = get(g + 2 * u, len);
#pragma unroll
        for (int u = 0; u < DG; ++u) xv[u] = row_load(cv[u].x);
#pragma unroll
        for (int u = 0; u < DG; ++u) fma8(__uint_as_float(cv[u].y), xv[u]);
      }
    }
    if (cp + kPiece >= ce1) store_row(r_first + ci, acc);
    if (!more) break;
    buf ^= 1;
  }
}

EnvInt g_blk2{"SGF_SPMM_BLK2", 1};
EnvInt g_chunk_rows{"SGF_SPMM_CHUNK_ROWS", 4096};
#ifdef SGF_PROBES
EnvInt g_blk_debug{"SGF_SPMM_BLK_DEBUG", 0};
#endif
enum Forced { kForceNone = -1, kForceWave, kForceRow, kForceSeg, kForceSeg2, kForceSub };
const char* const kForcedWords[] = {"wave", "row", "seg", "seg2", "sub"};
EnvWord g_forced{"SGF_SPMM_KERNEL", kForcedWords, 5};

struct BlkChoice {
  bool blk2, lean;
  int threads;
  size_t lds_bytes;
  uint64_t x_bytes;
};
template <typename T> constexpr size_t blk_slot_bytes() { return 64 * sizeof(typename Stored<T>::type); }
static_assert(blk_slot_bytes<uint16_t>() == 512, "k_spmm_blk2 lays a staged bf16 row out as 32 lanes x 16 bytes");
BlkChoice choose_blocked(int32_t d, size_t elem_size, int64_t ldx, int64_t ldy, int64_t n_rows, int32_t rows_per_block,
                         int32_t lds_rows, bool aligned16) {
  BlkChoice c;
  c.threads = rows_per_block / kBlkRowsPerWave * 64;
  c.x_bytes = static_cast<uint64_t>(n_rows) * static_cast<uint64_t>(ldx) * elem_size;
  c.lds_bytes = static_cast<size_t>(lds_rows) * (elem_size == 4 ? blk_slot_bytes<float>() : blk_slot_bytes<uint16_t>()) +
                static_cast<size_t>(c.threads / 64) * kScratchPerWave;
  const size_t per_cu = 160 * 1024;
  c.lean = (per_cu / c.lds_bytes) * static_cast<size_t>(c.threads / 64) > 16;
  c.blk2 = elem_size == 2 && d % 8 == 0 && d <= 256 && ldx % 8 == 0 && ldy % 8 == 0 && aligned16 &&
           c.x_bytes < (static_cast<uint64_t>(1) << 32) && c.threads <= 512 && g_blk2.get() != 0;
  return c;
}
bool blk_rows_ok(int32_t rows_per_block) {
  return rows_per_block >= kBlkRowsPerWave && rows_per_block <= 128 && rows_per_block % kBlkRowsPerWave == 0;
}
bool blk_lds_rows_ok(int32_t lds_rows, int32_t dtype) { return lds_rows >= 1 && lds_rows <= sgf_spmm_lds_rows_len(dtype); }

template <typename T>
int launch_blocked(const int64_t* rowptr, const int32_t* ecode, const float* eval, const int32_t* nlds,
                   const int32_t* sh_ptr, const int32_t* sh_cols, const T* x, int64_t ldx, T* y, int64_t ldy,
                   int64_t n_rows, int32_t d, int32_t rows_per_block, int32_t lds_rows, hipStream_t st,
                   const LongQueue& lq, float* partial) {
  const BlkChoice c = choose_blocked(d, sizeof(T), ldx, ldy, n_rows, rows_per_block, lds_rows,
                                     reinterpret_cast<uintptr_t>(x) % 16 == 0 && reinterpret_cast<uintptr_t>(y) % 16 == 0);
  const int threads = c.threads;
  const size_t lds_bytes = c.lds_bytes;
  const bool lean = c.lean;
  const int64_t nb = (n_rows + rows_per_block - 1) / rows_per_block;
  int chunk = 4096 / rows_per_block;
  if (chunk < 1) chunk = 1;
#ifdef SGF_PROBES
  const int dbg = g_blk_debug.get();
#else
  const int dbg = 0;
#endif
  constexpr int DGd = sizeof(T) == 4 ? 4 : 8, DGl = sizeof(T) == 4 ? 2 : 4;
  auto deep_fn = &k_spmm_blk<T, DGd, DGd, 4>;
  auto lean_fn = &k_spmm_blk<T, DGl, DGl, 8>;
  static thread_local size_t attr_set[4] = {0, 0, 0, 0};
  const int which = (sizeof(T) == 4 ? 0 : 2) + (lean ? 1 : 0);
  if (lds_bytes > attr_set[which]) {
    SGF_CHECK_HIP(hipFuncSetAttribute(lean ? reinterpret_cast<const void*>(lean_fn) : reinterpret_cast<const void*>(deep_fn),
                                      hipFuncAttributeMaxDynamicSharedMemorySize, static_cast<int>(lds_bytes)));
    attr_set[which] = lds_bytes;
  }
  if (c.blk2) {
    const size_t lds2 = lds_bytes;
    auto fn2 = &k_spmm_blk2<8, 4>;
    static thread_local size_t attr2 = 0;
    if (lds2 > attr2) {
      SGF_CHECK_HIP(hipFuncSetAttribute(reinterpret_cast<const void*>(fn2), hipFuncAttributeMaxDynamicSharedMemorySize,
                                        static_cast<int>(lds2)));
      attr2 = lds2;
    }
    hipLaunchKernelGGL(fn2, dim3(static_cast<unsigned>(nb)), dim3(threads), lds2, st, rowptr, ecode, eval, nlds, sh_ptr,
                       sh_cols, reinterpret_cast<const uint16_t*>(x), static_cast<uint32_t>(ldx * sizeof(T)),
                       static_cast<uint32_t>(c.x_bytes), reinterpret_cast<uint16_t*>(y), ldy, n_rows, d, rows_per_block,
                       lds_rows, chunk, lq, dbg);
  } else if (lean)
    hipLaunchKernelGGL(lean_fn, dim3(static_cast<unsigned>(nb)), dim3(threads), lds_bytes, st, rowptr, ecode, eval,
                       nlds, sh_ptr, sh_cols, x, ldx, y, ldy, n_rows, d, rows_per_block, lds_rows, chunk, lq, dbg);
  else
    hipLaunchKernelGGL(deep_fn, dim3(static_cast<unsigned>(nb)), dim3(threads), lds_bytes, st, rowptr, ecode, eval,
                       nlds, sh_ptr, sh_cols, x, ldx, y, ldy, n_rows, d, rows_per_block, lds_rows, chunk, lq, dbg);
  SGF_LAUNCH_CHECK();
  return spmm_long_rows(sizeof(T) == 2 ? SGF_BF16 : SGF_F32, rowptr, ecode, eval, x, ldx, d, lq, partial, y, ldy, st);
}

enum class Arm { SegBf16x2, Seg, Row, Wave, Sub };
struct Choice { Arm arm; int lanes_per_row; };
Choice choose_kernel(int32_t d, size_t elem_size, bool fits32, bool pair_ok, bool stream, int forced) {
  const bool pairs = fits32 && elem_size == 2 && pair_ok;
  const bool narrow_stream = d > 64 && d <= 128 && pairs && forced != kForceSub;
  if (d > 128 || narrow_stream) {
    if (pairs && (stream || forced == kForceSeg2 || (narrow_stream && forced == kForceNone))) return {Arm::SegBf16x2, 0};
    if (fits32 && forced == kForceSeg) return {Arm::Seg, 0};
    if (fits32 && forced != kForceWave) return {Arm::Row, 0};
    return {Arm::Wave, 0};
  }
  return {Arm::Sub, d > 64 ? 32 : d > 32 ? 16 : d > 16 ? 8 : d > 8 ? 4 : d > 4 ? 2 : 1};
}

Choice choose_for_operands(int32_t d, size_t elem_size, int64_t ldx, int64_t ldy, int64_t n_cols, bool aligned16,
                           bool stream, uint64_t* x_bytes_out = nullptr) {
  const uint64_t x_bytes = static_cast<uint64_t>(n_cols) * static_cast<uint64_t>(ldx) * elem_size;
  if (x_bytes_out) *x_bytes_out = x_bytes;
  const bool fits32 = d <= 256 && n_cols > 0 && x_bytes < (static_cast<uint64_t>(1) << 32);
  const bool pair_ok = d % 8 == 0 && ldx % 8 == 0 && ldy % 8 == 0 && aligned16;
  return choose_kernel(d, elem_size, fits32, pair_ok, stream, g_forced.get());
}

EnvInt g_packed{"SGF_SPMM_PACKED", 1};
struct PackedOperand {
  const void* slots;
  int32_t slot_bytes;
  const int32_t* overflow;
};
bool packed_rule(const Choice& c, int32_t d, size_t elem_size, int64_t n_cols, int32_t slot_bytes) {
  return g_packed.get() != 0 && c.arm == Arm::Row && elem_size == 2 && d == 256 &&
         (slot_bytes == 384 || slot_bytes == 448) &&
         static_cast<uint64_t>(n_cols) * static_cast<uint64_t>(slot_bytes) + kPackedTail < (static_cast<uint64_t>(1) << 32);
}

template <typename T>
int launch(const int64_t* rowptr, const int32_t* colind, const float* val, const T* x, int64_t ldx, int64_t n_cols,
           T* y, int64_t ldy, int64_t n_rows, int32_t d, hipStream_t st, const LongQueue& lq,
           float* partial, bool stream, const PackedOperand* pk = nullptr) {
  constexpr int UNROLL = 8;
  const dim3 block(kWavesPerBlock * 64);
  uint64_t x_bytes;
  const Choice c = choose_for_operands(d, sizeof(T), ldx, ldy, n_cols,
                                       reinterpret_cast<uintptr_t>(x) % 16 == 0 && reinterpret_cast<uintptr_t>(y) % 16 == 0,
                                       stream, &x_bytes);
  const int64_t nb = (n_rows + kWavesPerBlock - 1) / kWavesPerBlock;
  const int64_t nbs = (n_rows + kWavesPerBlock * kSegRows - 1) / (kWavesPerBlock * kSegRows);
  const int chunk_rows = g_chunk_rows.get() > 0 ? g_chunk_rows.get() : 4096;
  const int chunk = chunk_rows / (kWavesPerBlock * kSegRows) > 0 ? chunk_rows / (kWavesPerBlock * kSegRows) : 1;
#define SGF_SUB(LPR_)                                                                         \
  case LPR_: {                                                                                \
    constexpr int RPB = kWavesPerBlock * (64 / LPR_);                                         \
    const int64_t nbr = (n_rows + RPB - 1) / RPB;                                             \
    hipLaunchKernelGGL((k_spmm_sub<T, LPR_, UNROLL>), dim3(static_cast<unsigned>(nbr)), block, \
                       0, st, rowptr, colind, val, x, ldx, y, ldy, n_rows, d, lq);            \
  } break;
  switch (c.arm) {
    case Arm::SegBf16x2:
      hipLaunchKernelGGL((k_spmm_seg_bf16x2<16>), dim3(static_cast<unsigned>(nbs)), block, 0, st, rowptr, colind, val,
                         reinterpret_cast<const uint16_t*>(x), static_cast<uint32_t>(ldx * sizeof(T)),
                         static_cast<uint32_t>(x_bytes), reinterpret_cast<uint16_t*>(y), ldy, n_rows, d, chunk, lq);
      break;
    case Arm::Seg:
      hipLaunchKernelGGL((k_spmm_seg<T, (sizeof(T) == 4 ? 8 : 16)>), dim3(static_cast<unsigned>(nbs)), block, 0, st,
                         rowptr, colind, val, x, static_cast<uint32_t>(ldx * sizeof(T)),
                         static_cast<uint32_t>(x_bytes), y, ldy, n_rows, d, chunk, lq);
      break;
    case Arm::Row:
      if (pk && packed_rule(c, d, sizeof(T), n_cols, pk->slot_bytes)) {
        const uint32_t pk_bytes = static_cast<uint32_t>(n_cols * pk->slot_bytes + 16);
#define SGF_ROWP(S_)                                                                                                  \
  hipLaunchKernelGGL((k_spmm_row_packed<S_, UNROLL>), dim3(static_cast<unsigned>(nb)), block, 0, st, rowptr, colind, \
                     val, reinterpret_cast<const uint16_t*>(x), static_cast<uint32_t>(ldx * sizeof(T)),               \
                     static_cast<uint32_t>(x_bytes), pk->slots, pk_bytes, pk->overflow, reinterpret_cast<uint16_t*>(y), \
                     ldy, n_rows, lq)
        if (pk->slot_bytes == 384) SGF_ROWP(384);
        else SGF_ROWP(448);
#undef SGF_ROWP
        break;
      }
      hipLaunchKernelGGL((k_spmm_row<T, UNROLL>), dim3(static_cast<unsigned>(nb)), block, 0, st, rowptr, colind,
                         val, x, static_cast<uint32_t>(ldx * sizeof(T)), static_cast<uint32_t>(x_bytes), y, ldy,
                         n_rows, d, lq);
      break;
    case Arm::Wave:
      hipLaunchKernelGGL((k_spmm_wave<T, UNROLL>), dim3(static_cast<unsigned>(nb)), block, 0, st,
                         rowptr, colind, val, x, ldx, y, ldy, n_rows, d, lq);
      break;
    case Arm::Sub:
      switch (c.lanes_per_row) {
        SGF_SUB(32)
        SGF_SUB(16)
        SGF_SUB(8)
        SGF_SUB(4)
        SGF_SUB(2)
        SGF_SUB(1)
      }
      break;
  }
#undef SGF_SUB
  SGF_LAUNCH_CHECK();
  return spmm_long_rows(sizeof(T) == 2 ? SGF_BF16 : SGF_F32, rowptr, colind, val, x, ldx, d, lq, partial, y, ldy, st);
}

}

int spmm_long_rows(int dtype, const int64_t* rowptr, const int32_t* colind, const float* val, const void* x, int64_t ldx,
                   int32_t d, const LongQueue& lq, float* partial, void* y, int64_t ldy, hipStream_t st) {
  if (lq.cap <= 0) return SGF_OK;
  constexpr int UNROLL = 8;
  const dim3 block(kWavesPerBlock * 64);
  const int nb = lq.cap < 2048 ? lq.cap : 2048;
  if (dtype == SGF_BF16) {
    hipLaunchKernelGGL((k_spmm_long_seg<uint16_t, UNROLL>), dim3(nb), block, 0, st, rowptr, colind, val,
                       static_cast<const uint16_t*>(x), ldx, d, lq, partial);
    SGF_LAUNCH_CHECK();
    hipLaunchKernelGGL((k_spmm_long_fin<uint16_t>), dim3(nb), dim3(256), 0, st, lq, partial, d,
                       static_cast<uint16_t*>(y), ldy);
  } else {
    hipLaunchKernelGGL((k_spmm_long_seg<float, UNROLL>), dim3(nb), block, 0, st, rowptr, colind, val,
                       static_cast<const float*>(x), ldx, d, lq, partial);
    SGF_LAUNCH_CHECK();
    hipLaunchKernelGGL((k_spmm_long_fin<float>), dim3(nb), dim3(256), 0, st, lq, partial, d, static_cast<float*>(y), ldy);
  }
  SGF_LAUNCH_CHECK();
  return SGF_OK;
}

}

using namespace sgf;

namespace {
int check_spmm_operands(const char* fn, const void* x, int64_t ldx, const void* y, int64_t ldy, int32_t d, int32_t dtype) {
  SGF_REQUIRE(dtype == SGF_F32 || dtype == SGF_BF16, SGF_E_INVALID, "%s: unknown dtype %d", fn, dtype);
  SGF_REQUIRE(d % 4 == 0 && ldx % 4 == 0 && ldy % 4 == 0 && ldx >= d && ldy >= d, SGF_E_INVALID,
              "%s: d, ldx, ldy must be multiples of 4 with ld >= d (d=%d ldx=%lld ldy=%lld)", fn, d,
              static_cast<long long>(ldx), static_cast<long long>(ldy));
  const size_t esz = dtype == SGF_BF16 ? 2 : 4;
  SGF_REQUIRE(reinterpret_cast<uintptr_t>(x) % (4 * esz) == 0 && reinterpret_cast<uintptr_t>(y) % (4 * esz) == 0,
              SGF_E_INVALID, "%s: x / y must be aligned to 4 elements", fn);
  return SGF_OK;
}

int spmm_common(const int64_t* rowptr, const int32_t* colind, const float* val, const void* x, int64_t ldx,
                int64_t n_cols, void* y, int64_t ldy, int64_t n_rows, int32_t d, int32_t dtype, const LongQueue& lq,
                float* partial, hipStream_t st, const char* fn, bool stream = false, const PackedOperand* pk = nullptr) {
  SGF_REQUIRE(n_rows >= 0 && d >= 0 && n_cols >= 0, SGF_E_INVALID, "%s: negative size", fn);
  if (n_rows == 0 || d == 0) return SGF_OK;
  SGF_REQUIRE(rowptr && x && y, SGF_E_INVALID, "%s: null pointer", fn);
  SGF_REQUIRE(n_rows < (static_cast<int64_t>(1) << 31) * kWavesPerBlock, SGF_E_UNSUPPORTED,
              "%s: n_rows too large for one launch", fn);
  if (const int rc = check_spmm_operands(fn, x, ldx, y, ldy, d, dtype)) return rc;
  if (dtype == SGF_F32)
    return launch<float>(rowptr, colind, val, static_cast<const float*>(x), ldx, n_cols, static_cast<float*>(y), ldy,
                         n_rows, d, st, lq, partial, stream);
  return launch<uint16_t>(rowptr, colind, val, static_cast<const uint16_t*>(x), ldx, n_cols,
                          static_cast<uint16_t*>(y), ldy, n_rows, d, st, lq, partial, stream, pk);
}
}

extern "C" int sgf_spmm(const int64_t* rowptr, const int32_t* colind, const float* val,
                        const void* x, int64_t ldx, int64_t n_cols, void* y, int64_t ldy, int64_t n_rows,
                        int32_t d, int32_t dtype, void* stream) {
  const LongQueue none{nullptr, nullptr, 0, INT64_MAX};
  return spmm_common(rowptr, colind, val, x, ldx, n_cols, y, ldy, n_rows, d, dtype, none, nullptr,
                     static_cast<hipStream_t>(stream), "sgf_spmm");
}

extern "C" int32_t sgf_spmm_segment_len(void) { return kSegLen; }

extern "C" int32_t sgf_spmm_arm(int32_t d, int32_t dtype, int64_t ldx, int64_t ldy, int64_t n_cols, int32_t aligned16,
                                int32_t stream) {
  if (dtype != SGF_F32 && dtype != SGF_BF16) return -1;
  const Choice c = choose_for_operands(d, dtype == SGF_BF16 ? 2 : 4, ldx, ldy, n_cols, aligned16 != 0, stream != 0);
  return static_cast<int32_t>(c.arm) | (c.arm == Arm::Sub ? c.lanes_per_row << 8 : 0);
}

extern "C" size_t sgf_spmm_split_workspace_bytes(int64_t long_segments, int32_t d) {
  if (long_segments < 0 || d < 0) return 0;
  return long_partial_off(long_segments) + static_cast<size_t>(long_segments) * static_cast<size_t>(d) * sizeof(float);
}

int sgf::spmm_long_queue(const char* fn, int64_t long_len, int64_t long_segments, int32_t d, void* workspace,
                         size_t workspace_bytes, hipStream_t st, LongQueue* lq, float** partial) {
  SGF_REQUIRE(long_len >= 1 && long_segments >= 0 && long_segments < (static_cast<int64_t>(1) << 31),
              SGF_E_INVALID, "%s: bad long_len / long_segments", fn);
  *lq = LongQueue{nullptr, nullptr, 0, INT64_MAX};
  *partial = nullptr;
  if (long_segments == 0) return SGF_OK;
  SGF_REQUIRE(workspace && workspace_bytes >= sgf_spmm_split_workspace_bytes(long_segments, d),
              SGF_E_WORKSPACE, "%s: workspace too small", fn);
  char* ws = static_cast<char*>(workspace);
  lq->count = reinterpret_cast<int32_t*>(ws + kLongCountOff);
  lq->entries = reinterpret_cast<LongEntry*>(ws + kLongEntriesOff);
  lq->cap = static_cast<int32_t>(long_segments);
  lq->long_len = long_len;
  *partial = reinterpret_cast<float*>(ws + long_partial_off(long_segments));
  SGF_CHECK_HIP(hipMemsetAsync(lq->count, 0, sizeof(int32_t), st));
  return SGF_OK;
}

static int spmm_split_impl(bool stream_hint, const char* fn, const int64_t* rowptr, const int32_t* colind, const float* val,
                              const void* x, int64_t ldx, int64_t n_cols, void* y, int64_t ldy, int64_t n_rows,
                              int32_t d, int32_t dtype, int64_t long_len, int64_t long_segments,
                              void* workspace, size_t workspace_bytes, void* stream) {
  hipStream_t st = static_cast<hipStream_t>(stream);
  LongQueue lq;
  float* partial;
  if (const int rc = spmm_long_queue(fn, long_len, long_segments, d, workspace, workspace_bytes, st, &lq, &partial)) return rc;
  return spmm_common(rowptr, colind, val, x, ldx, n_cols, y, ldy, n_rows, d, dtype, lq, partial, st, fn, stream_hint);
}

extern "C" int sgf_spmm_split(const int64_t* rowptr, const int32_t* colind, const float* val, const void* x,
                              int64_t ldx, int64_t n_cols, void* y, int64_t ldy, int64_t n_rows, int32_t d,
                              int32_t dtype, int64_t long_len, int64_t long_segments, void* workspace,
                              size_t workspace_bytes, void* stream) {
  return spmm_split_impl(false, "sgf_spmm_split", rowptr, colind, val, x, ldx, n_cols, y, ldy, n_rows, d, dtype,
                         long_len, long_segments, workspace, workspace_bytes, stream);
}

extern "C" size_t sgf_spmm_packed_bytes(int64_t n, int32_t slot_bytes) {
  if (n < 0 || slot_bytes <= 0) return 0;
  return static_cast<size_t>(n) * static_cast<size_t>(slot_bytes) + kPackedTail;
}

extern "C" int32_t sgf_spmm_packed_supported(int32_t d, int32_t dtype, int64_t ldx, int64_t ldy, int64_t n_cols,
                                             int32_t aligned16, int32_t slot_bytes) {
  if (dtype != SGF_F32 && dtype != SGF_BF16) return 0;
  const size_t esz = dtype == SGF_BF16 ? 2 : 4;
  const Choice c = choose_for_operands(d, esz, ldx, ldy, n_cols, aligned16 != 0, false);
  return packed_rule(c, d, esz, n_cols, slot_bytes) ? 1 : 0;
}

extern "C" int sgf_spmm_packed(const int64_t* rowptr, const int32_t* colind, const float* val, const void* x, int64_t ldx,
                               int64_t n_cols, const void* packed, int32_t slot_bytes, const int32_t* overflow, void* y,
                               int64_t ldy, int64_t n_rows, int32_t d, int32_t dtype, int64_t long_len, int64_t long_segments,
                               void* workspace, size_t workspace_bytes, void* stream) {
  const char* fn = "sgf_spmm_packed";
  SGF_REQUIRE(packed && overflow, SGF_E_INVALID, "%s: null pointer", fn);
  SGF_REQUIRE(slot_bytes == 384 || slot_bytes == 448, SGF_E_UNSUPPORTED, "%s: slot_bytes must be 384 or 448", fn);
  SGF_REQUIRE(reinterpret_cast<uintptr_t>(packed) % 128 == 0, SGF_E_INVALID, "%s: the packed buffer must be 128-byte aligned", fn);
  hipStream_t st = static_cast<hipStream_t>(stream);
  LongQueue lq;
  float* partial;
  if (const int rc = spmm_long_queue(fn, long_len, long_segments, d, workspace, workspace_bytes, st, &lq, &partial)) return rc;
  const PackedOperand pk{packed, slot_bytes, overflow};
  return spmm_common(rowptr, colind, val, x, ldx, n_cols, y, ldy, n_rows, d, dtype, lq, partial, st, fn, false, &pk);
}

extern "C" int sgf_spmm_stream(const int64_t* rowptr, const int32_t* colind, const float* val, const void* x,
                               int64_t ldx, int64_t n_cols, void* y, int64_t ldy, int64_t n_rows, int32_t d,
                               int32_t dtype, int64_t long_len, int64_t long_segments, void* workspace,
                               size_t workspace_bytes, void* stream) {
  return spmm_split_impl(true, "sgf_spmm_stream", rowptr, colind, val, x, ldx, n_cols, y, ldy, n_rows, d, dtype,
                         long_len, long_segments, workspace, workspace_bytes, stream);
}

extern "C" int32_t sgf_spmm_lds_rows_len(int32_t dtype) {
  return dtype == SGF_BF16 ? 288 : 144;
}

extern "C" int32_t sgf_spmm_blocked_arm(int32_t d, int32_t dtype, int64_t ldx, int64_t ldy, int64_t n_rows,
                                        int32_t rows_per_block, int32_t lds_rows, int32_t aligned16) {
  if (dtype != SGF_F32 && dtype != SGF_BF16) return -1;
  if (!blk_rows_ok(rows_per_block) || !blk_lds_rows_ok(lds_rows, dtype)) return -1;
  const BlkChoice c = choose_blocked(d, dtype == SGF_BF16 ? 2 : 4, ldx, ldy, n_rows, rows_per_block, lds_rows, aligned16 != 0);
  return c.blk2 ? 0 : c.lean ? 1 : 2;
}

extern "C" int sgf_spmm_blocked(const int64_t* rowptr, const int32_t* ecode, const float* eval,
                                const int32_t* nlds, const int32_t* sh_ptr, const int32_t* sh_cols,
                                const void* x, int64_t ldx, void* y, int64_t ldy, int64_t n_rows, int32_t d,
                                int32_t dtype, int32_t rows_per_block, int32_t lds_rows, int64_t long_len,
                                int64_t long_segments, void* workspace, size_t workspace_bytes, void* stream) {
  const char* fn = "sgf_spmm_blocked";
  SGF_REQUIRE(n_rows >= 0 && d >= 0, SGF_E_INVALID, "%s: negative size", fn);
  if (n_rows == 0 || d == 0) return SGF_OK;
  SGF_REQUIRE(rowptr && ecode && eval && nlds && sh_ptr && sh_cols && x && y, SGF_E_INVALID, "%s: null pointer", fn);
  SGF_REQUIRE(d <= 256, SGF_E_UNSUPPORTED, "%s: d = %d > 256 (one wave per row)", fn, d);
  SGF_REQUIRE(blk_rows_ok(rows_per_block), SGF_E_INVALID, "%s: rows_per_block must be a multiple of %d in [%d, 128]", fn, kBlkRowsPerWave,
              kBlkRowsPerWave);
  SGF_REQUIRE(blk_lds_rows_ok(lds_rows, dtype), SGF_E_INVALID,
              "%s: lds_rows %d outside [1, %d]", fn, lds_rows, sgf_spmm_lds_rows_len(dtype));
  if (const int rc = check_spmm_operands(fn, x, ldx, y, ldy, d, dtype)) return rc;
  hipStream_t st = static_cast<hipStream_t>(stream);
  LongQueue lq;
  float* partial;
  if (const int rc = spmm_long_queue(fn, long_len, long_segments, d, workspace, workspace_bytes, st, &lq, &partial)) return rc;
  if (dtype == SGF_F32)
    return launch_blocked<float>(rowptr, ecode, eval, nlds, sh_ptr, sh_cols, static_cast<const float*>(x), ldx,
                                 static_cast<float*>(y), ldy, n_rows, d, rows_per_block, lds_rows, st, lq, partial);
  return launch_blocked<uint16_t>(rowptr, ecode, eval, nlds, sh_ptr, sh_cols, static_cast<const uint16_t*>(x), ldx,
                                  static_cast<uint16_t*>(y), ldy, n_rows, d, rows_per_block, lds_rows, st, lq, partial);
}
```

sgformer_amd/csrc/spmm_shared.h:

```cpp
#pragma once
#include "common.h"

#include <climits>

namespace sgf {

static constexpr int64_t kChunkBlocks = 1024;

static __device__ __forceinline__ int64_t xcd_remap(int64_t b, int64_t nblocks, int64_t chunk = kChunkBlocks) {
  const int64_t stripe = kNumXCD * chunk;
  const int64_t full = nblocks / stripe * stripe;
  if (b >= full) return b;
  const int64_t xcd = b % kNumXCD;
  const int64_t j = b / kNumXCD;
  return ((j / chunk) * kNumXCD + xcd) * chunk + j % chunk;
}

static constexpr int kSegLen = 1024;

struct LongEntry {
  int32_t row, seg, k, pad;
};

struct LongQueue {
  int32_t* count;
  LongEntry* entries;
  int32_t cap;
  int64_t long_len;
};

static __device__ __forceinline__ void push_long_row(const LongQueue& q, int64_t row, int64_t len, int lane_in_group,
                                              int group_width) {
  const int k = static_cast<int>((len + kSegLen - 1) / kSegLen);
  int base = 0;
  if (lane_in_group == 0) base = atomicAdd(q.count, k);
  base = __shfl(base, (threadIdx.x & 63) - lane_in_group, 64);
  for (int s = lane_in_group; s < k; s += group_width)
    if (base + s < q.cap) q.entries[base + s] = LongEntry{static_cast<int32_t>(row), s, k, 0};
}

typedef uint32_t u32x2 __attribute__((ext_vector_type(2)));
typedef uint32_t u32x4 __attribute__((ext_vector_type(4)));

constexpr size_t kLongCountOff = 0, kLongEntriesOff = 256;
static inline size_t long_partial_off(int64_t long_segments) {
  return kLongEntriesOff + align_up(static_cast<size_t>(long_segments) * sizeof(LongEntry), 256);
}

int spmm_long_queue(const char* fn, int64_t long_len, int64_t long_segments, int32_t d, void* workspace,
                    size_t workspace_bytes, hipStream_t st, LongQueue* lq, float** partial);

int spmm_long_rows(int dtype, const int64_t* rowptr, const int32_t* colind, const float* val, const void* x, int64_t ldx,
                   int32_t d, const LongQueue& lq, float* partial, void* y, int64_t ldy, hipStream_t st);

}
```

sgformer_amd/graph.py:

```python
from __future__ import annotations

import dataclasses
import os
from collections import OrderedDict
from typing import Optional

import torch

from . import _lib
from .kernels import HipKernels, LONG_ROW, _SEGMENT

_F32 = torch.float32


K = HipKernels()


def _has(table, name: str, *args) -> bool:
    fn = getattr(table, name, None)
    return fn is not None and (not args or bool(fn(*args)))


def _env(name: str, default: str = "") -> str:
    return os.environ.get(name, default)


SMALL_GRAPH_NNZ = 1 << 23


def long_row_segments(rowptr: torch.Tensor, nnz: Optional[int] = None, max_row_len: Optional[int] = None) -> int:
    if rowptr.numel() <= 1:
        return 0
    if max_row_len is not None and max_row_len <= LONG_ROW:
        return 0
    if nnz is not None and nnz < SMALL_GRAPH_NNZ:
        return 0 if nnz <= LONG_ROW else nnz // _SEGMENT + nnz // (LONG_ROW + 1) + 1
    lens = rowptr[1:] - rowptr[:-1]
    segs = torch.where(lens > LONG_ROW, (lens + (_SEGMENT - 1)) // _SEGMENT, torch.zeros_like(lens))
    return int(segs.sum())


@dataclasses.dataclass(slots=True)
class EdgeHints:
    trusted: bool = False
    max_in_degree: Optional[int] = None
    csr: Optional[tuple] = None
    csr_t_lazy: bool = False
    symmetric: bool = False
    sharded_graph: object = None

    def attach(self, edge_index: torch.Tensor) -> torch.Tensor:
        edge_index._sgf_hints = self
        return edge_index

    def to(self, device) -> "EdgeHints":
        csr = None if self.csr is None else tuple(t.to(device) for t in self.csr)
        return dataclasses.replace(self, csr=csr, sharded_graph=None)


_NO_HINTS = EdgeHints()


def hints_of(edge_index) -> EdgeHints:
    return getattr(edge_index, "_sgf_hints", _NO_HINTS)


class GraphOperand:
    blocked = False
    tiled = False
    locality = False
    comm_local = None
    blk_row = None
    tile_min_count = None
    n_local = None
    symmetric: Optional[bool] = None
    _t_lazy = False

    def __init__(self):
        self._plans, self._tile_plans, self._halo, self._view, self.forward_calls = {}, {}, {}, None, 0

    def _stored(self, transposed: bool) -> bool:
        if transposed:
            self.transposed()
        return bool(transposed) and not self.symmetric

    def arrays(self, transposed: bool = False):
        if self._stored(transposed):
            return (*self.transposed(), self.t_long_segments)
        return self.rowptr, self.colind, self.val, self.long_segments

    def plan(self, dtype, transposed: bool = False):
        return None

    def halo(self, shard, transposed: bool):
        return None

    def view(self, now: bool = False) -> "GraphView":
        return GraphView(self, None, None)


class CSRGraph(GraphOperand):

    def __init__(self, edge_index: torch.Tensor, num_nodes: int, validate: bool = True):
        super().__init__()
        K.check(edge_index)
        if edge_index.dtype != torch.int64 or edge_index.dim() != 2 or edge_index.shape[0] != 2:
            raise ValueError("edge_index must be an int64 tensor of shape [2, nnz]")
        if num_nodes >= 2 ** 31:
            raise ValueError("num_nodes must be < 2^31 (int32 column indices)")
        ei = edge_index.contiguous()
        n = int(num_nodes)
        hints = hints_of(edge_index)
        if validate and not hints.trusted and ei.shape[1] > 0:
            lo, hi = torch.aminmax(ei)
            if int(lo) < 0 or int(hi) >= n:
                raise IndexError(f"edge_index has node ids outside [0, {n})")
        self.n, self.nnz, self.device = n, int(ei.shape[1]), ei.device
        self.edge_index = ei
        pre = hints.csr
        if pre is not None and pre[0].numel() == n + 1 and pre[1].numel() == self.nnz:
            self.rowptr, self.colind, self.val, self.deg = pre
            self._t_lazy = bool(hints.csr_t_lazy)
        else:
            self.rowptr, self.colind, self.val, self.deg = K.csr_build(ei, n)
        self.long_segments = long_row_segments(self.rowptr, self.nnz, hints.max_in_degree)
        self.t_long_segments = 0
        self._t = None
        if hints.symmetric:
            self.symmetric, self._t, self.t_long_segments = True, (self.rowptr, self.colind, self.val), self.long_segments

    def transposed(self):
        if self._t is None and self._t_lazy:
            self._t = K.sampled_csr_transpose(self.rowptr, self.colind, self.val, self.n)
            self.symmetric = False
            self.t_long_segments = long_row_segments(self._t[0], self.nnz)
        if self._t is None:
            t_rowptr, t_colind, t_val, sym = K.csr_transpose(self.edge_index, self.n, self.deg,
                                                             self.rowptr, self.colind)
            self.symmetric = sym
            self._t = (self.rowptr, self.colind, self.val) if sym else (t_rowptr, t_colind, t_val)
            self.t_long_segments = self.long_segments if sym else long_row_segments(t_rowptr, self.nnz)
        return self._t

    def plan(self, dtype, transposed: bool = False):
        if not self.blocked:
            return None
        key = (self._stored(transposed), dtype)
        if key not in self._plans:
            self._plans[key] = BlockedPlan(*self.arrays(key[0])[:3], self.n, dtype)
        return self._plans[key]

    def tile_plan(self, transposed: bool = False):
        key = self._stored(transposed)
        if key not in self._tile_plans:
            self._tile_plans[key] = TilePlan(*self.arrays(key)[:3], self.n, self.blk_row, min_count=self.tile_min_count)
        return self._tile_plans[key]

    def view(self, now: bool = False) -> "GraphView":
        self.forward_calls += 1
        if self._view is None:
            self._view = GraphView.decide(self, now)
        return self._view if self._view is not None else GraphView(self, None, None)


class WeightedCSRGraph(GraphOperand):

    def __init__(self, edge_index: torch.Tensor, values: torch.Tensor, num_nodes: int):
        super().__init__()
        K.check(edge_index, values)
        n = int(num_nodes)
        self.n, self.nnz, self.device = n, int(edge_index.shape[1]), edge_index.device
        self._src, self._tgt = edge_index[0].contiguous(), edge_index[1].contiguous()
        self._values = values.detach().to(_F32).contiguous()
        self.rowptr, self.colind, self.val = self._sorted(self._tgt, self._src)
        self.long_segments = long_row_segments(self.rowptr, self.nnz)
        self._t, self.t_long_segments, self.symmetric = None, 0, False

    def _sorted(self, rows, cols):
        perm = torch.argsort(rows * self.n + cols, stable=True)
        counts = torch.bincount(rows, minlength=self.n)
        rowptr = torch.zeros(self.n + 1, dtype=torch.int64, device=self.device)
        torch.cumsum(counts, 0, out=rowptr[1:])
        return rowptr, cols[perm].to(torch.int32), self._values[perm]

    def transposed(self):
        if self._t is None:
            self._t = self._sorted(self._src, self._tgt)
            self.t_long_segments = long_row_segments(self._t[0], self.nnz)
        return self._t


def weighted_graph(edge_index: torch.Tensor, edge_weight: torch.Tensor, num_nodes: int, value_fn, tag: str):
    key_tag = (tag, edge_weight.data_ptr(), edge_weight._version, tuple(edge_weight.shape))

    def build(ei, n):
        ei2, vals = value_fn(ei, edge_weight, n)
        g = WeightedCSRGraph(ei2, vals, n)
        g.edge_weight_ref = edge_weight
        return g

    return graph_cache.get(edge_index, num_nodes, factory=build, tag=key_tag)


def _block_shape(dtype):
    cap = K.lds_rows_max(dtype)
    env = _env("SGF_SPMM_BLOCK")
    if env:
        r, c = (int(t) for t in env.split(","))
        return r, min(c, cap)
    return 128, cap


class BlockedPlan:

    def __init__(self, rowptr, colind, val, n: int, dtype, rows_per_block=None, lds_rows=None):
        r, c = _block_shape(dtype)
        self.rows_per_block = int(rows_per_block or r)
        self.lds_rows = int(lds_rows or c)
        (self.ecode, self.eval, self.nlds, self.sh_ptr, self.sh_cols, st) = K.spmm_plan(
            rowptr, colind, val, n, self.rows_per_block, self.lds_rows, LONG_ROW)
        self.lds_entries, self.staged_rows, self.unique_pairs, self.nnz = st
        self.lds_fraction = self.lds_entries / max(self.nnz, 1)


TILE_CAP = 512
TILE_MIN_COUNT = 2
TILE_MAX_ROWS = 128
TILE_SPARSE_DENSITY = 0.12


def _tile_params():
    env = _env("SGF_SPMM_TILE")
    if env:
        c, m, r = (int(t) for t in env.split(","))
        return c, m, r
    return TILE_CAP, TILE_MIN_COUNT, TILE_MAX_ROWS


class TilePlan:

    def __init__(self, rowptr, colind, val, n: int, blk_row: torch.Tensor, cap=None, min_count=None, keep_dense=False):
        c, m, _ = _tile_params()
        self.blk_row, self.nb = blk_row, int(blk_row.numel()) - 1
        self.block_rows = int((blk_row[1:] - blk_row[:-1]).max()) if self.nb > 0 else 1
        self.cap, self.min_count = int(cap or c), int(min_count or m)
        (self.sh_ptr, self.sh_cols, self.tile_ptr, self.tiles, self.rem_rowptr, self.rem_col, self.rem_val,
         st) = K.tile_plan(rowptr, colind, val, n, blk_row, self.cap, self.min_count, LONG_ROW)
        self.tile_entries, self.staged_rows, _, self.nnz, self.fragments, self.rem_entries = st[:6]
        self.tile_fraction = self.tile_entries / max(self.nnz, 1)
        self.tile_density = self.tile_entries / max(self.fragments * 512, 1)
        self.long_segments = long_row_segments(self.rem_rowptr, None)
        self.grp, self.pool, units = K.tile_pack(blk_row, self.tile_ptr, self.tiles, self.fragments)
        self.tile_bytes = units * 16
        if not keep_dense:
            self.tiles = None
        self.bytes = (self.pool.numel() + self.grp.numel() * 4 + self.rem_col.numel() * 8 + self.rem_rowptr.numel() * 8
                      + self.sh_cols.numel() * 4)


REORDER_MIN_NODES = 100_000
REORDER_MIN_LDS_FRACTION = 0.25
REORDER_ITERS = (6, 6)
_reorder_mode = None


def set_reorder_mode(mode: Optional[str]):
    global _reorder_mode
    prev, _reorder_mode = _reorder_mode, mode
    return prev


def _mode() -> str:
    return _reorder_mode or {"0": "never", "1": "always"}.get(_env("SGF_REORDER", "auto"), "auto")


class GraphView:

    def __init__(self, graph, perm, inv, stats=None):
        self.graph, self.perm, self.inv, self.stats = graph, perm, inv, stats or {}

    @staticmethod
    def decide(g: "CSRGraph", now: bool):
        mode = _mode()
        if mode == "never" or K.name != "hip" or g.nnz == 0 or g.nnz >= 2 ** 32 - 1:
            return GraphView(g, None, None, {"reordered": False, "why": "disabled"})
        if mode == "auto":
            if g.n < REORDER_MIN_NODES:
                return GraphView(g, None, None, {"reordered": False, "why": "small graph"})
            if not now and g.forward_calls < 2:
                return None
        perm, inv, comm = K.reorder(g.edge_index, g.n, *REORDER_ITERS)
        g2 = CSRGraph(inv.long()[g.edge_index], g.n, validate=False)
        g2.blk_row = K.tile_blocks(comm[perm.long()].contiguous(), g.n, _tile_params()[2], g.device)
        try:
            tp = g2.tile_plan(False)
        except (ValueError, _lib.SgfError) as e:
            return GraphView(g, None, None, {"reordered": False, "why": f"tile plan unsupported: {e}"})
        if tp.tile_density < TILE_SPARSE_DENSITY and tp.min_count == TILE_MIN_COUNT and not _env("SGF_SPMM_TILE"):
            g2.tile_min_count = TILE_MIN_COUNT + 1
            g2._tile_plans.clear()
            tp = g2.tile_plan(False)
        stats = {"lds_fraction": tp.tile_fraction, "tile_density": tp.tile_density, "blocks": tp.nb,
                 "staged_rows_per_node": tp.staged_rows / max(g.n, 1), "plan_bytes": tp.bytes, "min_count": tp.min_count}
        if tp.tile_fraction < REORDER_MIN_LDS_FRACTION and mode != "always":
            return GraphView(g, None, None, {**stats, "reordered": False, "why": "no reuse to exploit"})
        g2.locality = True
        g2.blocked = _env("SGF_SPMM_BLOCKED", "0") == "1"
        g2.tiled = _env("SGF_SPMM_TILED", "1") == "1" and not g2.blocked
        if not g2.tiled:
            g2._tile_plans.clear()
        stats["kernel"] = ("row-block (LDS-staged)" if g2.blocked else
                           "tiles (matrix cores) + gather remainder for bf16 rows of 128 / 256 features, else stream"
                           if g2.tiled else "stream")
        return GraphView(g2, perm, inv, {**stats, "reordered": True})


def prepare_graph(edge_index: torch.Tensor, num_nodes: int) -> GraphView:
    return graph_cache.get(edge_index, num_nodes).view(now=True)


class _GraphCache:

    def __init__(self, capacity: int = 4):
        self.capacity = capacity
        self._d: "OrderedDict[tuple, CSRGraph]" = OrderedDict()

    def get(self, edge_index: torch.Tensor, num_nodes: int, factory=None, tag=None):
        key = (edge_index.data_ptr(), edge_index._version, tuple(edge_index.shape),
               tuple(edge_index.stride()), str(edge_index.device), int(num_nodes), tag)
        g = self._d.get(key)
        if g is not None:
            self._d.move_to_end(key)
            return g
        g = (factory or CSRGraph)(edge_index, num_nodes)
        g.edge_index_ref = edge_index
        self._d[key] = g
        while len(self._d) > self.capacity:
            self._d.popitem(last=False)
        return g

    def clear(self):
        self._d.clear()


graph_cache = _GraphCache()


def _sharded_spmm(graph, x, shard, transposed: bool):
    rowptr, colind, val, long_segments = graph.arrays(transposed)
    n_local = graph.n_local
    plan = graph.halo(shard, transposed)
    if plan is not None and plan.enabled:
        if plan.n_halo == 0:
            return _own_block_spmm(graph, plan, (rowptr, plan.colind, val, long_segments), x, n_local, transposed)
        if shard.overlap:
            shard.overlapped_exchanges += 1
            own, (rp_h, ci_h, va_h, seg_h) = plan.split(rowptr, val, n_local)
            recv, work, keep = shard.halo_exchange_start(x, plan)
            y = _own_block_spmm(graph, plan, own, x, n_local, transposed)
            work.wait()
            y.add_(K.spmm(rp_h, ci_h, va_h, recv, n_local, long_segments=seg_h))
            del keep
            return y
        return K.spmm(rowptr, plan.colind, val, shard.halo_exchange(x, plan), n_local, long_segments=long_segments)
    d = x.shape[1]
    chunks = shard.gather_chunks(d)
    if chunks <= 1:
        return K.spmm(rowptr, colind, val, shard.all_gather_rows(x), n_local, long_segments=long_segments)
    w = d // chunks
    pending = [shard.all_gather_rows(x[:, c * w:(c + 1) * w].contiguous(), async_op=True) for c in range(chunks)]
    y = torch.empty((n_local, d), dtype=x.dtype, device=x.device)
    for c, (buf, work) in enumerate(pending):
        work.wait()
        K.spmm(rowptr, colind, val, buf, n_local, out=y[:, c * w:(c + 1) * w], long_segments=long_segments)
    return y


def _tile_operand_ok(x: torch.Tensor, out=None) -> bool:
    return (_has(K, "tile_supported", x.shape[1], x.dtype)
            and x.shape[0] * max(x.stride(0), x.shape[1]) * 2 < 2 ** 32 - 2048
            and (out is None or (out.stride(0) % 8 == 0 and out.data_ptr() % 16 == 0)))


def _own_block_spmm(graph, plan, own, x, n_local: int, transposed: bool):
    rp, ci, va, segs = own
    if not graph.locality:
        return K.spmm(rp, ci, va, x, n_local, long_segments=segs)
    if (_tile_operand_ok(x) and graph.comm_local is not None and _env("SGF_SPMM_TILED", "1") == "1" and n_local >= 256):
        if plan.own_tile_plan is None:
            try:
                blk_row = K.tile_blocks(graph.comm_local, n_local, _tile_params()[2], x.device)
                tp = TilePlan(rp, ci, va, n_local, blk_row)
                plan.own_tile_plan = tp if tp.tile_fraction >= REORDER_MIN_LDS_FRACTION else False
            except (ValueError, _lib.SgfError):
                plan.own_tile_plan = False
        if plan.own_tile_plan:
            return K.spmm_tile(plan.own_tile_plan, x, n_local)
    return K.spmm(rp, ci, va, x, n_local, long_segments=segs, stream_hint=True)


class _SpMM(torch.autograd.Function):
    @staticmethod
    def forward(ctx, x, graph, shard, packed=None):
        K.check(x)
        ctx.graph, ctx.shard = graph, shard
        if shard is not None:
            return _sharded_spmm(graph, x, shard, False)
        return spmm_on(graph, x, False, packed=packed)

    @staticmethod
    def backward(ctx, gy):
        graph, shard = ctx.graph, ctx.shard
        if shard is not None:
            return _sharded_spmm(graph, gy.contiguous(), shard, True), None, None, None
        return spmm_on(graph, gy.contiguous(), True), None, None, None


def spmm_packed_slot(graph, x_shape, dtype, slot_bytes: int) -> int:
    if not slot_bytes or not _has(K, "spmm_packed_supported") or graph.blocked or graph.tiled or graph.locality:
        return 0
    return slot_bytes if K.spmm_packed_supported(x_shape, dtype, slot_bytes) else 0


def spmm_on(graph, x: torch.Tensor, transposed: bool, out=None, packed=None) -> torch.Tensor:
    rp, ci, va, segs = graph.arrays(transposed)
    plan = graph.plan(x.dtype, transposed) if (graph.blocked and x.shape[1] <= 256) else None
    if plan is not None:
        return K.spmm_blocked(rp, plan, x, graph.n, out=out, long_segments=segs)
    if graph.tiled:
        if _tile_operand_ok(x, out):
            return K.spmm_tile(graph.tile_plan(transposed), x, graph.n, out=out)
        if not K.tile_supported(x.shape[1], x.dtype) and graph._tile_plans:
            graph._tile_plans.clear()
    if graph.locality:
        return K.spmm(rp, ci, va, x, graph.n, out=out, long_segments=segs, stream_hint=True)
    if packed is not None and not transposed and out is None:
        return K.spmm_packed(rp, ci, va, x, packed, graph.n, long_segments=segs)
    return K.spmm(rp, ci, va, x, graph.n, out=out, long_segments=segs)


def spmm(graph, x: torch.Tensor, shard=None, packed=None) -> torch.Tensor:
    return _SpMM.apply(x, graph, shard, packed)
```

sgformer_amd/kernels.py:

```python
from __future__ import annotations

import ctypes
import os
from typing import Optional

import torch

from . import _lib

_F32 = torch.float32
_BF16 = torch.bfloat16

LONG_ROW = 1024
_SEGMENT = 1024

counters = {"spmm_packed": 0}


class PackedRows:
    __slots__ = ("slots", "slot_bytes", "n", "overflow")

    def __init__(self, slots, slot_bytes, n, overflow):
        self.slots, self.slot_bytes, self.n, self.overflow = slots, slot_bytes, n, overflow


def _ptr(t: Optional[torch.Tensor]):
    return None if t is None else ctypes.c_void_p(t.data_ptr())


def _stream_handle(device) -> int:
    return torch.cuda.current_stream(device).cuda_stream


def _stream(device) -> ctypes.c_void_p:
    return ctypes.c_void_p(_stream_handle(device))


def _dtype_code(dtype) -> int:
    if dtype == _F32:
        return _lib.SGF_F32
    if dtype == _BF16:
        return _lib.SGF_BF16
    raise TypeError(f"sgformer_amd kernels take float32 or bfloat16 storage, got {dtype}")


def _code(t: torch.Tensor) -> int:
    return _dtype_code(t.dtype)


_X3_PRECISIONS = ("high", "medium")


def f32_matmul_code() -> int:
    return _lib.SGF_F32_BF16X3 if torch.get_float32_matmul_precision() in _X3_PRECISIONS else _lib.SGF_F32


_x3_cache: "dict[tuple, bool]" = {}


def _mm_code(t: torch.Tensor, query: Optional[str] = None, *shape) -> int:
    code = _code(t)
    if code != _lib.SGF_F32 or f32_matmul_code() != _lib.SGF_F32_BF16X3:
        return code
    if query is None:
        return _lib.SGF_F32_BF16X3
    key = (query,) + tuple(int(v) for v in shape)
    ok = _x3_cache.get(key)
    if ok is None:
        ok = _x3_cache[key] = bool(getattr(_lib.load(), query)(*key[1:], _lib.SGF_F32_BF16X3))
    return _lib.SGF_F32_BF16X3 if ok else _lib.SGF_F32


def _ld(t: Optional[torch.Tensor]) -> int:
    return 0 if t is None else t.stride(0)


def _rows(t: Optional[torch.Tensor]) -> Optional[torch.Tensor]:
    if t is None:
        return None
    if t.stride(-1) != 1 or t.stride(0) % 4 != 0 or t.data_ptr() % (4 * t.element_size()) != 0:
        t = t.contiguous()
        if t.shape[0] > 1 and t.stride(0) % 4 != 0:
            raise ValueError(f"feature dimension {t.shape[-1]} must be a multiple of 4")
    return t


_workspaces: "dict[tuple, torch.Tensor]" = {}


_capture_scope = None


def begin_capture_scope() -> dict:
    global _capture_scope
    _capture_scope = {}
    return _capture_scope


def end_capture_scope():
    global _capture_scope
    _capture_scope = None


class SeedBank:

    def __init__(self, device, capacity: int = 64):
        self.seeds = torch.zeros(int(capacity), dtype=torch.int64, device=device)
        self.used = 0

    def take(self) -> int:
        if self.used >= self.seeds.numel():
            raise RuntimeError(f"sgformer_amd: more than {self.seeds.numel()} dropout calls in one captured step")
        self.used += 1
        return self.used - 1


_seed_scope = None


def begin_seed_scope(bank: SeedBank) -> SeedBank:
    global _seed_scope
    _seed_scope = bank
    return bank


def end_seed_scope():
    global _seed_scope
    _seed_scope = None


def seed_scope():
    return _seed_scope


def _fresh_bytes(device, nbytes: int) -> torch.Tensor:
    return torch.empty(max(int(nbytes), 256), dtype=torch.uint8, device=device)


def _workspace(device, name: str, nbytes: int) -> torch.Tensor:
    if torch.cuda.is_available() and torch.cuda.is_current_stream_capturing():
        if _capture_scope is None:
            return _fresh_bytes(device, nbytes)
        cache, key = _capture_scope, (device.index, name)
    else:
        cache, key = _workspaces, (device.index, name, _stream_handle(device))
    ws = cache.get(key)
    if ws is None or ws.numel() < nbytes:
        ws = cache[key] = _fresh_bytes(device, nbytes)
    return ws


_NO_SCRATCH = (None, 0)

_constant_bytes: "dict[str, int]" = {}


def _const_bytes(query: str, *args) -> int:
    n = _constant_bytes.get(query)
    if n is None:
        n = _constant_bytes[query] = int(getattr(_lib.load(), query)(*args))
    return n


def _scratch(device, name: Optional[str], nbytes: int):
    ws = _fresh_bytes(device, nbytes) if name is None else _workspace(device, name, nbytes)
    return ws, ws.numel()


def _long_row_scratch(device, long_segments: int, d: int):
    if long_segments <= 0:
        return _NO_SCRATCH
    return _scratch(device, "spmm_long", _lib.load().sgf_spmm_split_workspace_bytes(long_segments, d))


def _stats_scratch(device, n: int, d: int, want_stats: bool):
    if not want_stats:
        return _NO_SCRATCH
    return _scratch(device, "gcn_epi", _lib.load().sgf_gcn_epilogue_workspace_bytes(n, d))


_PLAIN = frozenset((int, float, bool, type(None)))
_Tensor = torch.Tensor


def _launch(device, name: str, *args):
    argv = [a if type(a) in _PLAIN else (a.data_ptr() if isinstance(a, _Tensor) else a) for a in args]
    argv.append(_stream_handle(device))
    if torch.cuda.current_device() == device.index:
        _lib.call(name, *argv)
    else:
        with torch.cuda.device(device):
            _lib.call(name, *argv)


def _rows16(t: torch.Tensor) -> torch.Tensor:
    if t.stride(-1) != 1 or (t.stride(0) * t.element_size()) % 16 != 0 or t.data_ptr() % 16 != 0:
        t = t.contiguous()
    return t


def _pair_gram() -> bool:
    return os.environ.get("SGF_GRAM_PAIR", "1") != "0"


def _one_pass_cat() -> bool:
    return os.environ.get("SGF_GCN_CAT", "1") != "0"


class HipKernels:

    name = "hip"

    @staticmethod
    def check(*tensors):
        for t in tensors:
            if t is not None and not t.is_cuda:
                raise RuntimeError(
                    "sgformer_amd runs on MI355X only: got a CPU tensor.  There is no CPU fallback; "
                    "move the model and its inputs to the GPU (the reference's CPU evaluation path, "
                    "large/eval.py:36-65, is outside this library's scope).")

    @staticmethod
    def csr_build(ei: torch.Tensor, n: int):
        dev, nnz = ei.device, int(ei.shape[1])
        rowptr = torch.empty(n + 1, dtype=torch.int64, device=dev)
        colind = torch.empty(nnz, dtype=torch.int32, device=dev)
        val = torch.empty(nnz, dtype=_F32, device=dev)
        deg = torch.empty(n, dtype=torch.int32, device=dev)
        _launch(dev, "sgf_csr_build", ei, nnz, n, rowptr, colind, val, deg,
                *_scratch(dev, None, _lib.load().sgf_csr_workspace_bytes(nnz, n)))
        return rowptr, colind, val, deg

    @staticmethod
    def csr_transpose(ei: torch.Tensor, n: int, deg, rowptr, colind):
        dev, nnz = ei.device, int(ei.shape[1])
        t_rowptr = torch.empty(n + 1, dtype=torch.int64, device=dev)
        t_colind = torch.empty(nnz, dtype=torch.int32, device=dev)
        t_val = torch.empty(nnz, dtype=_F32, device=dev)
        flag = torch.zeros(1, dtype=torch.int32, device=dev)
        _launch(dev, "sgf_csr_transpose", ei, nnz, n, deg, rowptr, colind, t_rowptr, t_colind, t_val, flag,
                *_scratch(dev, None, _lib.load().sgf_csr_workspace_bytes(nnz, n)))
        return t_rowptr, t_colind, t_val, bool(int(flag.item()))

    @staticmethod
    def subgraph(ei: torch.Tensor, n: int, subset: torch.Tensor, relabel_nodes: bool, want_eid: bool):
        dev, nnz, m = ei.device, int(ei.shape[1]), int(subset.numel())
        relabel = torch.empty(max(n, 1), dtype=torch.int32, device=dev)
        total = torch.zeros(1, dtype=torch.int64, device=dev)
        scratch = _scratch(dev, "subgraph", _lib.load().sgf_subgraph_workspace_bytes(nnz, n))
        _launch(dev, "sgf_subgraph_plan", ei, nnz, n, subset, m, relabel, total, *scratch)
        k = int(total.item())
        out = torch.empty((2, k), dtype=torch.int64, device=dev)
        eid = torch.empty(k, dtype=torch.int64, device=dev) if want_eid else None
        _launch(dev, "sgf_subgraph_emit", ei, nnz, n, relabel, int(relabel_nodes), k, out, eid, *scratch)
        return out, eid

    @staticmethod
    def subgraph_csr(rowptr, colind, n: int, subset: torch.Tensor, local_of: torch.Tensor, want_edges: bool):
        dev, m = rowptr.device, int(subset.numel())
        lib = _lib.load()
        rowptr_b = torch.empty(m + 1, dtype=torch.int64, device=dev)
        deg_b = torch.empty(m + 1, dtype=torch.int32, device=dev)
        total = torch.empty(3, dtype=torch.int64, device=dev)
        _launch(dev, "sgf_subgraph_csr_plan", rowptr, colind, n, subset, m, local_of, rowptr_b, deg_b, total,
                *_scratch(dev, "subgraph_csr_plan", lib.sgf_subgraph_csr_plan_workspace_bytes(m)))
        try:
            t, bad, longest = total.tolist()
            t = 0 if bad else int(t)
            colind_b = torch.empty(t, dtype=torch.int32, device=dev)
            val_b = torch.empty(t, dtype=_F32, device=dev)
            ei_b = torch.empty((2, t), dtype=torch.int64, device=dev) if want_edges else None
            scratch = _scratch(dev, "subgraph_csr_emit", lib.sgf_subgraph_csr_emit_workspace_bytes(m, t))
        except BaseException:
            local_of.fill_(-1)
            raise
        _launch(dev, "sgf_subgraph_csr_emit", rowptr, colind, n, subset, m, local_of, rowptr_b, deg_b, t, colind_b, val_b,
                ei_b, *scratch)
        if bad:
            return None
        return rowptr_b, colind_b, val_b, deg_b[:m], ei_b, int(longest)

    @staticmethod
    def sampled_csr_supported(max_fanout: int) -> bool:
        return bool(_lib.load().sgf_sampled_csr_supported(int(max_fanout)))

    @staticmethod
    def sampled_csr_build(e_src: torch.Tensor, e_dst: torch.Tensor, counts: torch.Tensor, node_cap: int, edge_cap: int,
                          max_fanout: int):
        dev = e_src.device
        rowptr_b = torch.empty(node_cap + 1, dtype=torch.int64, device=dev)
        colind_b = torch.empty(max(edge_cap, 1), dtype=torch.int32, device=dev)
        val_b = torch.empty(max(edge_cap, 1), dtype=_F32, device=dev)
        deg_b = torch.empty(node_cap + 1, dtype=torch.int32, device=dev)
        _launch(dev, "sgf_sampled_csr_build", e_src, e_dst, counts, node_cap, edge_cap, int(max_fanout), rowptr_b, colind_b,
                val_b, deg_b,
                *_scratch(dev, "sampled_csr_build", _lib.load().sgf_sampled_csr_build_workspace_bytes(node_cap, edge_cap)))
        return rowptr_b, colind_b, val_b, deg_b

    @staticmethod
    def sampled_csr_transpose(rowptr, colind, val, n: int):
        dev, nnz = rowptr.device, int(colind.numel())
        t_rowptr = torch.empty(n + 1, dtype=torch.int64, device=dev)
        t_colind = torch.empty(nnz, dtype=torch.int32, device=dev)
        t_val = torch.empty(nnz, dtype=_F32, device=dev)
        _launch(dev, "sgf_sampled_csr_transpose", rowptr, colind, val, n, nnz, t_rowptr, t_colind, t_val,
                *_scratch(dev, "sampled_csr_transpose", _lib.load().sgf_sampled_csr_transpose_workspace_bytes(n, nnz)))
        return t_rowptr, t_colind, t_val

    @staticmethod
    def graph_prologue(ei: torch.Tensor, n: int, undirected: bool, remove_loops: bool, add_loops: bool):
        dev, m = ei.device, int(ei.shape[1])
        total = torch.zeros(1, dtype=torch.int64, device=dev)
        scratch = _scratch(dev, None, _lib.load().sgf_graph_prologue_workspace_bytes(m, n))
        _launch(dev, "sgf_graph_prologue_plan", ei, m, n, int(undirected), int(remove_loops), int(add_loops), total, *scratch)
        k = int(total.item())
        out = torch.empty((2, k), dtype=torch.int64, device=dev)
        _launch(dev, "sgf_graph_prologue_emit", m, n, int(undirected), int(add_loops), k, out, *scratch)
        return out

# ... 825 lines not shown
```

sgformer_amd/ours.py:

```python
from __future__ import annotations

from dataclasses import dataclass
from typing import Optional

import torch
import torch.nn as nn
import torch.nn.functional as F

from . import head_rows, ops

__all__ = ["GraphConvLayer", "GraphConv", "TransConvLayer", "TransConv", "SGFormer",
           "full_attention_conv"]

_NO_SHARD = None

DEFAULT_COMPUTE_DTYPE = None

import os as _os
OVERLAP_BRANCHES = _os.environ.get("SGF_OVERLAP", "1") == "1"
OVERLAP_MIN_NODES = 65536

PACKED_SLOT_BYTES = (384, 0, 0)
_side_streams = {}


def _side_stream(device):
    s = _side_streams.get(device.index)
    if s is None:
        s = _side_streams[device.index] = torch.cuda.Stream(device=device)
    return s


class _Holder:
    _x_cache = None


import weakref as _weakref
_entry_cache = _weakref.WeakKeyDictionary()


def _stem_w(lin: nn.Linear, x):
    f = lin.weight.shape[1]
    pad = x.shape[1] - f
    if pad != 0 and x.shape[1] not in ((f + 3) // 4 * 4, (f + 7) // 8 * 8):
        raise RuntimeError(f"input has {x.shape[1]} features, the layer expects {f}")
    return lin.weight if pad == 0 else F.pad(lin.weight, (0, pad))


def _entry_width(f: int, cdt) -> int:
    q = 8 if cdt == torch.bfloat16 else 4
    return (f + q - 1) // q * q


def _lin(x, lin: nn.Linear):
    return ops.linear(x, _stem_w(lin, x), lin.bias)


def _drop(x, p, training, res=None):
    if training and p is not None and p > 0.0:
        if x.dim() == 2 and x.shape[1] % 4 == 0:
            return ops.dropout_res(x, res, float(p))
        x = F.dropout(x, p=p, training=True)
        return x if res is None else x + res
    if p is None:
        raise TypeError("dropout probability is None (pass --trans_dropout / --gnn_dropout)")
    return x if res is None else x + res


def full_attention_conv(qs, ks, vs, output_attn=False, shard=None):
    n, h, d = qs.shape
    qk = torch.cat([qs.reshape(n, h * d), ks.reshape(n, h * d)], dim=1)
    if vs.shape[1] == h:
        qkv = torch.cat([qk, vs.reshape(n, h * d)], dim=1)
        out = ops.attention(qkv, None, h, d, shard, per_head=h > 1)
    else:
        out = ops.attention(qk, vs.reshape(n, d), h, d, shard, per_head=h > 1)
    out = out.reshape(n, h, d)
    if output_attn:
        return out, _attention_matrix(qs, ks)
    return out


def _attention_matrix(qs, ks):
    n = qs.shape[0]
    qn = qs / torch.norm(qs, p=2)
    kn = ks / torch.norm(ks, p=2)
    attention = torch.einsum("nhm,lhm->nlh", qn, kn).mean(dim=-1)
    normalizer = (torch.einsum("nhm,hm->nh", qn, kn.sum(dim=0)) + n).mean(dim=-1, keepdim=True)
    return attention / normalizer


class _BNBook:

    def __init__(self, module: nn.Module, bn: nn.BatchNorm1d):
        self.module, self.bn = module, bn

    def use_batch(self) -> bool:
        bn = self.bn
        return self.module.training or not bn.track_running_stats or bn.running_mean is None

    def _tracks(self, count: float) -> bool:
        if count <= 1 and self.module.training:
            raise ValueError("Expected more than 1 value per channel when training")
        bn = self.bn
        return self.module.training and bn.track_running_stats and bn.running_mean is not None

    def from_sums(self, stats):
        bn = self.bn
        track = self._tracks(stats.count)
        if ops._has(ops.K, "bn_finalize") and (not track or (bn.momentum is not None and bn.running_mean.dtype == torch.float32)):
            with torch.no_grad():
                if track:
                    bn.num_batches_tracked += 1
                mean, rstd = ops.K.bn_finalize(stats.sums, stats.shift, stats.count, bn.eps,
                                               float(bn.momentum) if track else 0.0,
                                               bn.running_mean if track else None, bn.running_var if track else None)
            return mean, rstd, stats.count, True
        return self.from_moments(*stats.moments())

    def from_moments(self, mean, var, count):
        bn = self.bn
        if self._tracks(count):
            with torch.no_grad():
                bn.num_batches_tracked += 1
                m = bn.momentum if bn.momentum is not None else 1.0 / float(bn.num_batches_tracked)
                bn.running_mean.mul_(1.0 - m).add_(mean.to(bn.running_mean.dtype), alpha=m)
                unbiased = var * (count / max(count - 1.0, 1.0))
                bn.running_var.mul_(1.0 - m).add_(unbiased.to(bn.running_var.dtype), alpha=m)
        return mean, torch.rsqrt(var + bn.eps), count, True

    def running(self, count: float = 0.0):
        bn = self.bn
        return bn.running_mean.float(), torch.rsqrt(bn.running_var.float() + bn.eps), count, False


@dataclass
class _Stems:
    trans: torch.Tensor
    trans_normed: bool = False
    gcn: Optional[torch.Tensor] = None
    gcn_stats: Optional[tuple] = None
    gcn_first: Optional[torch.Tensor] = None
    pack: Optional[dict] = None


class GraphConvLayer(nn.Module):

    def __init__(self, in_channels, out_channels, use_weight=True, use_init=False):
        super().__init__()
        self.use_init = use_init
        self.use_weight = use_weight
        in_channels_ = 2 * in_channels if use_init else in_channels
        self.W = nn.Linear(in_channels_, out_channels)
        self._shard = _NO_SHARD

    def reset_parameters(self):
        self.W.reset_parameters()

    def propagate(self, x, edge_index, packed=None):
        shard = self._shard
        if isinstance(edge_index, ops.CSRGraph):
            graph = edge_index
        elif shard is not None and not shard.local_graph:
            graph = shard.graph_for(edge_index)
        else:
            graph = ops.graph_cache.get(edge_index, x.shape[0])
        shard = None if (shard is not None and shard.local_graph) else shard
        return ops.spmm(graph, x, shard, packed if shard is None else None)

    def forward(self, x, edge_index, x0, bn_stats=False):
        shard = self._shard
        y = self.propagate(x, edge_index)
        if self.use_init:
            if bn_stats:
                return ops.linear_bn_stats((y, x0), self.W.weight, self.W.bias, shard)
            y = ops.linear_cat((y, x0), self.W.weight, self.W.bias)
        elif self.use_weight:
            if bn_stats:
                return ops.linear_bn_stats(y, self.W.weight, self.W.bias, shard)
            y = _lin(y, self.W)
        return (y, None) if bn_stats else y


class GraphConv(nn.Module):

    def __init__(self, in_channels, hidden_channels, num_layers=2, dropout=0.5, use_bn=True,
                 use_residual=True, use_weight=True, use_init=False, use_act=True):
        super().__init__()
        self.convs = nn.ModuleList()
        self.fcs = nn.ModuleList()
        self.fcs.append(nn.Linear(in_channels, hidden_channels))
        self.bns = nn.ModuleList()
        self.bns.append(nn.BatchNorm1d(hidden_channels))
        for _ in range(num_layers):
            self.convs.append(GraphConvLayer(hidden_channels, hidden_channels, use_weight, use_init))
            self.bns.append(nn.BatchNorm1d(hidden_channels))
        self.dropout = dropout
        self.activation = F.relu
        self.use_bn = use_bn
        self.use_residual = use_residual
        self.use_act = use_act
        self._shard = _NO_SHARD

    def reset_parameters(self):
        for conv in self.convs:
            conv.reset_parameters()
        for bn in self.bns:
            bn.reset_parameters()
        for fc in self.fcs:
            fc.reset_parameters()

    def _bn_act_res(self, bn: nn.BatchNorm1d, x, res, relu, stats=None):
        shard, book = self._shard, _BNBook(self, bn)
        if book.use_batch():
            mean, rstd, n_tot, used = book.from_moments(*(stats if stats is not None else ops.batch_stats(x, shard)))
        else:
            mean, rstd, n_tot, used = book.running(float(x.shape[0]))
        return ops.bn_act_res(x, res, bn.weight, bn.bias, mean, rstd, relu, used, n_tot, shard)

    @property
    def _drop_on(self) -> bool:
        return self.training and self.dropout is not None and self.dropout > 0.0

    def pack_request(self, layer: int, n: int, dtype, edge_index):
        slot = PACKED_SLOT_BYTES[layer] if layer < len(PACKED_SLOT_BYTES) else 0
        if (not slot or self._drop_on or self._shard is not None or ops.K.name != "hip" or layer >= len(self.convs)
                or self.convs[layer]._shard is not None or torch.cuda.is_current_stream_capturing()):
            return None
        if isinstance(edge_index, ops.CSRGraph):
            graph = edge_index
        elif torch.is_tensor(edge_index):
            graph = ops.graph_cache.get(edge_index, n)
        else:
            return None
        d = self.fcs[0].out_features
        slot = ops.spmm_packed_slot(graph, (n, d), dtype, slot)
        return {"slot_bytes": slot, "out": None} if slot else None

    def fused_stem_ok(self, x) -> bool:
        d = self.fcs[0].out_features
        return (self.use_bn and not self._drop_on and len(self.convs) > 0 and all(c.use_init for c in self.convs)
                and x.dim() == 2 and x.dtype == torch.bfloat16
                and all(tuple(c.W.weight.shape) == (d, 2 * d) for c in self.convs)
                and ops._has(ops.K, "gcn_bn_bwd_dx_supported", d, x.dtype)
                and ops._switch("SGF_GCN_FUSED", True) and ops._switch("SGF_STEM_FUSED", True))

    def _fused_layers(self, x0):
        return (self.use_bn and not self._drop_on and len(self.convs) > 0 and all(c.use_init for c in self.convs)
                and all(ops.gcn_layer_fused_ok(x0, c.W.weight) for c in self.convs))

    def _stage(self, bn, x, res, relu, stats=None):
        fuse_res = res is not None and not self._drop_on
        if self.use_bn:
            x = self._bn_act_res(bn, x, res if fuse_res else None, relu, stats)
        else:
            if relu:
                x = torch.relu(x)
            if fuse_res:
                x = x + res
        return _drop(x, self.dropout, self.training, res if (res is not None and not fuse_res) else None)

    def forward(self, x, edge_index, stem=None):
        ops._require_cuda(x, None if isinstance(edge_index, ops.CSRGraph) else edge_index)
        x_first = packed = None
        if stem is not None and stem.gcn_first is not None:
            x, x_first = stem.gcn, stem.gcn_first
            packed = stem.pack.pop("out", None) if stem.pack is not None else None
        else:
            if stem is not None:
                x, stats0 = stem.gcn, stem.gcn_stats
            else:
                x, stats0 = _lin(x, self.fcs[0]), None
            x = self._stage(self.bns[0], x, None, True, stats0)
        if self._fused_layers(x):
            x0, chain = x, ops.GradChain()
            if x_first is not None:
                x = x_first
            for i, conv in enumerate(self.convs):
                bn = self.bns[i + 1]
                y = conv.propagate(x, edge_index, packed)
                packed = None
                req = self.pack_request(i + 1, x0.shape[0], x0.dtype, edge_index) if self.use_act else None
                x = ops.linear_bn_act_res(y, x0, conv.W.weight, conv.W.bias, bn.weight, bn.bias, _BNBook(self, bn),
                                          self.use_act, self.use_residual, self._shard, chain, i == 0, req)
                packed = req.pop("out", None) if req is not None else None
            return x
        uses_init = [c.use_init for c in self.convs]
        k = 1 + sum(uses_init) + (len(self.convs) if self.use_residual else 0)
        hub = list(ops.fan_out(x, k)) if k <= 8 else [x] * k
        x = hub.pop()
        for i, conv in enumerate(self.convs):
            want = self.use_bn and _BNBook(self, self.bns[i + 1]).use_batch()
            x0 = hub.pop() if uses_init[i] else None
            if want:
                x, stats = conv(x, edge_index, x0, bn_stats=True)
            else:
                x, stats = conv(x, edge_index, x0), None
            x = self._stage(self.bns[i + 1], x, hub.pop() if self.use_residual else None, self.use_act, stats)
        return x


class TransConvLayer(nn.Module):

    def __init__(self, in_channels, out_channels, num_heads, use_weight=True):
        super().__init__()
        self.Wk = nn.Linear(in_channels, out_channels * num_heads)
        self.Wq = nn.Linear(in_channels, out_channels * num_heads)
        if use_weight:
            self.Wv = nn.Linear(in_channels, out_channels * num_heads)
        self.out_channels = out_channels
        self.num_heads = num_heads
        self.use_weight = use_weight
        self._shard = _NO_SHARD

    def reset_parameters(self):
        self.Wk.reset_parameters()
        self.Wq.reset_parameters()
        if self.use_weight:
            self.Wv.reset_parameters()

    def _project(self, query_input, source_input):
        ws = [self.Wq.weight, self.Wk.weight] + ([self.Wv.weight] if self.use_weight else [])
        bs = [self.Wq.bias, self.Wk.bias] + ([self.Wv.bias] if self.use_weight else [])
        if query_input is source_input:
            return ops.linear(query_input, torch.cat(ws, 0), torch.cat(bs, 0))
        q = ops.linear(query_input, ws[0], bs[0])
        kv = ops.linear(source_input, torch.cat(ws[1:], 0), torch.cat(bs[1:], 0))
        return torch.cat([q, kv], 1)

    def forward(self, query_input, source_input, output_attn=False, grad_tap=None):
        ops._require_cuda(query_input, source_input)
        h, d = self.num_heads, self.out_channels
        if (h == 1 and query_input is source_input and not output_attn and query_input.shape[1] == d
                and d % 4 == 0 and d <= 256):
            wv, bv = (self.Wv.weight, self.Wv.bias) if self.use_weight else (None, None)
            return ops.attention_from_input(query_input, self.Wq.weight, self.Wq.bias, self.Wk.weight,
                                            self.Wk.bias, wv, bv, self._shard, tap=grad_tap)
        qkv = self._project(query_input, source_input)
        v_ext = None
        if not self.use_weight:
            if source_input.shape[1] != d:
                raise RuntimeError(f"use_weight=False needs in_channels == out_channels ({d})")
            v_ext = source_input
        final_output = ops.attention(qkv, v_ext, h, d, self._shard)
        if output_attn:
            n = qkv.shape[0]
            qs = qkv[:, :h * d].reshape(n, h, d)
            ks = qkv[:, h * d:2 * h * d].reshape(n, h, d)
            return final_output, _attention_matrix(qs, ks)
        return final_output


class TransConv(nn.Module):

    def __init__(self, in_channels, hidden_channels, num_layers=2, num_heads=1, dropout=0.5,
                 use_bn=True, use_residual=True, use_weight=True, use_act=True, alpha=None,
                 layer_cls=None):
        super().__init__()
        layer_cls = layer_cls or TransConvLayer
        self.convs = nn.ModuleList()
        self.fcs = nn.ModuleList()
        self.fcs.append(nn.Linear(in_channels, hidden_channels))
        self.bns = nn.ModuleList()
        self.bns.append(nn.LayerNorm(hidden_channels))
        for _ in range(num_layers):
            self.convs.append(layer_cls(hidden_channels, hidden_channels, num_heads=num_heads,
                                        use_weight=use_weight))
            self.bns.append(nn.LayerNorm(hidden_channels))
        self.dropout = dropout
        self.activation = F.relu
        self.use_bn = use_bn
        self.use_residual = use_residual
        self.use_act = use_act
        self.alpha = alpha

    _attn_post_act = True

    def reset_parameters(self):
        for conv in self.convs:
            conv.reset_parameters()
        for bn in self.bns:
            bn.reset_parameters()
        for fc in self.fcs:
            fc.reset_parameters()

    def _mix(self):
        return (0.5, 0.5) if self.alpha is None else (float(self.alpha), 1.0 - float(self.alpha))

    def _ln(self, ln: nn.LayerNorm, x, res, a, b, relu):
        if res is None and not self.use_bn and not relu:
            return x
        gamma, beta = (ln.weight, ln.bias) if self.use_bn else (None, None)
        return ops.ln_res_act(x, res, a, b, gamma, beta, relu, ln.eps)

    def _embed(self, x, training, stem=None):
        if stem is not None and stem.trans_normed:
            return _drop(stem.trans, self.dropout, training)
        x = _lin(x, self.fcs[0]) if stem is None else stem.trans
        x = self._ln(self.bns[0], x, None, 1.0, 0.0, True)
        return _drop(x, self.dropout, training)

    def forward(self, x, stem=None):
        ops._require_cuda(x)
        x = self._embed(x, self.training, stem)
        layer_ = [x]
        a, b = self._mix()
        for i, conv in enumerate(self.convs):
            if self.use_residual and layer_[i] is x:
                holder = {}
                h = conv(x, x, grad_tap=holder)
                x = self._ln(self.bns[i + 1], h, ops.grad_tap(x, holder), a, b, self.use_act)
            elif self.use_residual:
                h = conv(x, x)
                x = self._ln(self.bns[i + 1], h, layer_[i], a, b, self.use_act)
            else:
                h = conv(x, x)
                x = self._ln(self.bns[i + 1], h, None, 1.0, 0.0, self.use_act)
            x = _drop(x, self.dropout, self.training)
            layer_.append(x)
        return x

    def get_attentions(self, x):
        x = self._embed(x, False)
        layer_, attentions = [x], []
        a, b = self._mix()
        for i, conv in enumerate(self.convs):
            h, attn = conv(x, x, output_attn=True)
            attentions.append(attn)
            res = layer_[i] if self.use_residual else None
            x = self._ln(self.bns[i + 1], h, res, a if res is not None else 1.0,
                         b if res is not None else 0.0, self.use_act and self._attn_post_act)
            layer_.append(x)
        return torch.stack(attentions, dim=0)


class SGFormer(nn.Module):

    def __init__(self, in_channels, hidden_channels, out_channels,
                 trans_num_layers=1, trans_num_heads=1, trans_dropout=0.5, trans_use_bn=True,
                 trans_use_residual=True, trans_use_weight=True, trans_use_act=True,
                 gnn_num_layers=1, gnn_dropout=0.5, gnn_use_weight=True, gnn_use_init=False,
                 gnn_use_bn=True, gnn_use_residual=True, gnn_use_act=True,
                 use_graph=True, graph_weight=0.8, aggregate='add', alpha=None, compute_dtype='default',
                 trans_cls=None):
        super().__init__()
        self.compute_dtype = DEFAULT_COMPUTE_DTYPE if isinstance(compute_dtype, str) else compute_dtype
        self.logits_dtype = None
        self.trans_conv = (trans_cls or TransConv)(
            in_channels, hidden_channels, num_layers=trans_num_layers, num_heads=trans_num_heads,
            dropout=trans_dropout, use_bn=trans_use_bn, use_residual=trans_use_residual,
            use_weight=trans_use_weight, use_act=trans_use_act, alpha=alpha)
        self.graph_conv = GraphConv(in_channels, hidden_channels, gnn_num_layers, gnn_dropout,
                                    gnn_use_bn, gnn_use_residual, gnn_use_weight, gnn_use_init,
                                    gnn_use_act)
        self.use_graph = use_graph
        self.graph_weight = graph_weight
        self.aggregate = aggregate
        self.overlap_branches = OVERLAP_BRANCHES
        if aggregate == 'add':
            self.fc = nn.Linear(hidden_channels, out_channels)
        elif aggregate == 'cat':
            self.fc = nn.Linear(2 * hidden_channels, out_channels)
        else:
            raise ValueError(f'Invalid aggregate type:{aggregate}')
        self.params1 = list(self.trans_conv.parameters())
        self.params2 = list(self.graph_conv.parameters()) if self.graph_conv is not None else []
        self.params2.extend(list(self.fc.parameters()))

    def _forward_on_gpu_from_host(self, x, edge_index):
        if not torch.cuda.is_available():
            ops._require_cuda(x)
        if torch.is_grad_enabled():
            raise RuntimeError("sgformer_amd: CPU tensors with autograd enabled — there is no CPU fallback "
                               "and training runs on MI355X only; move the model and inputs to the GPU")
        dev = torch.device("cuda", torch.cuda.current_device())
        state = {k: v.to(dev) for k, v in list(self.named_parameters()) + list(self.named_buffers())}
        out = torch.func.functional_call(self, state, (x.to(dev), edge_index.to(dev)))
        for k, v in self.named_buffers():
            v.copy_(state[k])
        return out.to(x.device)

    def forward(self, x, edge_index):
        return self._forward(x, edge_index)

    def forward_rows(self, x, edge_index, rows):
        if isinstance(rows, bool) or not (isinstance(rows, int) or torch.is_tensor(rows)):
            raise TypeError(f"forward_rows: rows must be an int, an int64 index tensor or a bool mask, got {type(rows).__name__}")
        return self._forward(x, edge_index, rows)

    def _forward(self, x, edge_index, rows=None, ce_labels=None):
        if rows is None and not x.is_cuda and ops.K.name == "hip" and not next(self.parameters()).is_cuda:
            return self._forward_on_gpu_from_host(x, edge_index)
        ops._require_cuda(x, edge_index)
        out_dtype = x.dtype if getattr(self, 'logits_dtype', None) is None else self.logits_dtype
        cdt = self.compute_dtype if self.compute_dtype is not None else x.dtype
        seeds = getattr(edge_index, "_sgf_seed_count", None) if rows is None else None
        if seeds is not None and not head_rows.seed_head_enabled():
            seeds = None
        if rows is None and ops.hints_of(edge_index).csr is not None:
            from . import graphed
            out = graphed.maybe_step(self, x, edge_index, cdt, out_dtype)
            if out is not None:
                return out
        view = None
        if self.use_graph and self.graph_conv._shard is None and ops.K.name == "hip":
            view = ops.graph_cache.get(edge_index, x.shape[0]).view()
            edge_index = view.graph
        repart = None
        shard = self.graph_conv._shard if self.use_graph else None
        if shard is not None and not shard.local_edges and not shard.local_graph:
            repart = shard.repartition_for(edge_index)
            if repart is not None:
                x, edge_index = repart.to_new(x), repart.edge_index
        perm = view.perm if view is not None else None
        f = x.shape[1]
        fp = _entry_width(f, cdt)
        pad = fp != f and not x.requires_grad and ops._has(ops.K, "pad_rows")
        if x.requires_grad:
            if perm is not None:
                x = ops.permute_rows(x, view.perm, view.inv, cdt)
            elif x.dtype != cdt:
                x = x.to(cdt)
        elif perm is not None or pad or x.dtype != cdt:
            holder = view if view is not None else _entry_cache.setdefault(self, _Holder())
            key = (x.data_ptr(), x._version, tuple(x.shape), x.dtype, cdt, bool(pad), perm is not None)
            hit = getattr(holder, "_x_cache", None)
            if hit is None or hit[0] != key:
                if pad:
                    xe = ops.K.pad_rows(x, perm, fp, cdt)
                elif perm is not None:
                    xe = ops.permute_rows(x, view.perm, view.inv, cdt)
                else:
                    xe = x.to(cdt)
                hit = (key, xe, x)
                holder._x_cache = hit
            x = hit[1]
        if rows is not None or seeds is not None:
            if repart is not None or shard is not None:
                if rows is not None:
                    raise NotImplementedError("sgformer_amd: forward_rows is not available on the node-sharded path")
                seeds = None
            elif torch.cuda.is_available() and torch.cuda.is_current_stream_capturing():
                seeds = None
            elif perm is not None:
                if rows is None:
                    seeds = None
                else:
                    if isinstance(rows, int):
                        if not 0 <= rows <= x.shape[0]:
                            raise IndexError(f"forward_rows: a prefix of {rows} rows of {x.shape[0]}")
                        rows = view.inv[:rows].long()
                    else:
                        rows = view.inv.long()[rows.to(view.inv.device)]
        return self._core(x, edge_index, view, repart, out_dtype, rows=rows, lazy_seeds=seeds, ce_labels=ce_labels)

    def _entry_copy_uncached(self, x, cdt):
        f = x.shape[1]
        fp = _entry_width(f, cdt)
        if fp != f and ops._has(ops.K, "pad_rows"):
            return ops.K.pad_rows(x, None, fp, cdt)
        return x if x.dtype == cdt else x.to(cdt)

    def _core(self, x, edge_index, view, repart, out_dtype, rows=None, lazy_seeds=None, ce_labels=None):
        stem = None
        gc, tc = (self.graph_conv if self.use_graph else None), self.trans_conv
        both = gc is not None and hasattr(tc, "fcs") and hasattr(gc, "fcs") and hasattr(gc, "bns")
        wg, wt = (_stem_w(gc.fcs[0], x), _stem_w(tc.fcs[0], x)) if both else (None, None)
        if both and gc.fused_stem_ok(x) and ops.stem_pair_bn_supported(x, wg, wt):
            bn0 = gc.bns[0]
            ln = None
            if getattr(tc, "use_bn", False) and hasattr(tc, "bns") and ops.stem_ln_supported(x, wt):
                ln = (tc.bns[0].weight, tc.bns[0].bias, tc.bns[0].eps, True)
            req = gc.pack_request(0, x.shape[0], x.dtype, edge_index)
            x0a, x0b, yt = ops.stem_pair_bn(x, wg, gc.fcs[0].bias, wt, tc.fcs[0].bias,
                                            bn0.weight, bn0.bias, _BNBook(gc, bn0), gc._shard, ln, req)
            stem = _Stems(trans=yt, trans_normed=ln is not None, gcn=x0a, gcn_first=x0b, pack=req)
        elif both and ops.stem_pair_supported(x, wg, wt):
            want = gc.use_bn and _BNBook(gc, gc.bns[0]).use_batch()
            (yg, yt), st = ops.stem_pair(x, wg, gc.fcs[0].bias, wt, tc.fcs[0].bias,
                                         want_stats0=want, shard=gc._shard)
            stem = _Stems(trans=yt, gcn=yg, gcn_stats=st)

        def trans_branch():
# ... 70 lines not shown
```

Baseline: 29.46 million.

## Add compressed-row coded SpMM path for the second forward GCN layer

Adds a per-row scaled compact encoding of bf16 feature rows (384-byte slots instead of 512) plus a pre-scaled edge-value array, and a row SpMM kernel that gathers the coded slots and decodes them in registers. Rows that cannot be encoded are flagged through a sign bit on the edge value and fall back to full bf16 loads. The aim is to cut gather bandwidth in the bandwidth-bound SpMM. It is only enabled for the fwd2 layer on large graphs, and each call pays for two extra encoding kernels plus a memset.

Result: faster. 30.20 million, median of 6 (+2.5%).

```diff
diff --git a/include/sgf.h b/include/sgf.h
--- a/include/sgf.h
+++ b/include/sgf.h
@@ -8,7 +8,7 @@
 extern "C" {
 #endif
 
-#define SGF_VERSION 670
+#define SGF_VERSION 671
 
 #define SGF_F32 0
 #define SGF_BF16 1
@@ -79,6 +79,17 @@
                     int64_t n_cols, const void* packed, int32_t slot_bytes, const int32_t* overflow, void* y, int64_t ldy,
                     int64_t n_rows, int32_t d, int32_t dtype, int64_t long_len, int64_t long_segments, void* workspace,
                     size_t workspace_bytes, void* stream);
+
+size_t sgf_spmm_coded_bytes(int64_t n);
+int32_t sgf_spmm_coded_supported(int32_t d, int32_t dtype, int64_t ldx, int64_t ldy, int64_t n_cols, int32_t aligned16);
+int sgf_spmm_code_rows(const void* x, int64_t ldx, int64_t n, void* coded, uint8_t* scale_u8, int32_t* n_escaped,
+                       void* stream);
+int sgf_spmm_code_values(const int32_t* colind, const float* val, int64_t nnz, const uint8_t* scale_u8, float* val_coded,
+                         int32_t* n_unsupported, void* stream);
+int sgf_spmm_coded(const int64_t* rowptr, const int32_t* colind, const float* val, const float* val_coded, const void* x,
+                   int64_t ldx, int64_t n_cols, const void* coded, const int32_t* n_unsupported, void* y, int64_t ldy,
+                   int64_t n_rows, int32_t d, int32_t dtype, int64_t long_len, int64_t long_segments, void* workspace,
+                   size_t workspace_bytes, void* stream);
 
 int sgf_spmm_stream(const int64_t* rowptr, const int32_t* colind, const float* val, const void* x,
                     int64_t ldx, int64_t n_cols, void* y, int64_t ldy, int64_t n_rows, int32_t d, int32_t dtype,
diff --git a/sgformer_amd/_lib.py b/sgformer_amd/_lib.py
--- a/sgformer_amd/_lib.py
+++ b/sgformer_amd/_lib.py
@@ -51,6 +51,12 @@
     "sgf_spmm_packed_supported": (c_int32, [c_int32, c_int32, c_int64, c_int64, c_int64, c_int32, c_int32]),
     "sgf_spmm_packed": (c_int32, [_P, _P, _P, _P, c_int64, c_int64, _P, c_int32, _P, _P, c_int64, c_int64, c_int32, c_int32,
                                   c_int64, c_int64, _P, c_size_t, _P]),
+    "sgf_spmm_coded_bytes": (c_size_t, [c_int64]),
+    "sgf_spmm_coded_supported": (c_int32, [c_int32, c_int32, c_int64, c_int64, c_int64, c_int32]),
+    "sgf_spmm_code_rows": (c_int32, [_P, c_int64, c_int64, _P, _P, _P, _P]),
+    "sgf_spmm_code_values": (c_int32, [_P, _P, c_int64, _P, _P, _P, _P]),
+    "sgf_spmm_coded": (c_int32, [_P, _P, _P, _P, _P, c_int64, c_int64, _P, _P, _P, c_int64, c_int64, c_int32, c_int32,
+                                 c_int64, c_int64, _P, c_size_t, _P]),
     "sgf_spmm_stream": (c_int32, [_P, _P, _P, _P, c_int64, c_int64, _P, c_int64, c_int64, c_int32, c_int32, c_int64,
                                   c_int64, _P, c_size_t, _P]),
     "sgf_reorder_workspace_bytes": (c_size_t, [c_int64, c_int64]),
diff --git a/sgformer_amd/coded.py b/sgformer_amd/coded.py
--- /dev/null
+++ b/sgformer_amd/coded.py
@@ -0,0 +1,59 @@
+from __future__ import annotations
+
+import torch
+
+from . import _lib
+from . import kernels as _k
+
+_BF16 = torch.bfloat16
+
+escape_log = None
+
+
+def spmm_coded_supported(x_shape, dtype) -> bool:
+    n, d = int(x_shape[0]), int(x_shape[1])
+    if dtype != _BF16 or n == 0:
+        return False
+    return bool(_lib.load().sgf_spmm_coded_supported(d, _k._dtype_code(dtype), d, d, n, 1))
+
+
+def spmm_code_rows(x: torch.Tensor):
+    n, d = x.shape
+    if x.dtype != _BF16 or d != 256 or x.stride(1) != 1:
+        raise ValueError("spmm_code_rows: bf16 rows of 256 contiguous columns")
+    dev = x.device
+    slots = torch.empty(max(int(_lib.load().sgf_spmm_coded_bytes(n)), 1), dtype=torch.uint8, device=dev)
+    scale = torch.empty(max(n, 1), dtype=torch.uint8, device=dev)
+    n_escaped = torch.empty(1, dtype=torch.int32, device=dev)
+    _k._launch(dev, "sgf_spmm_code_rows", x, x.stride(0), n, slots, scale, n_escaped)
+    return slots, scale, n_escaped
+
+
+def spmm_code_values(colind: torch.Tensor, val: torch.Tensor, scale: torch.Tensor):
+    dev, nnz = val.device, int(val.numel())
+    val_coded = torch.empty(max(nnz, 1), dtype=torch.float32, device=dev)
+    n_unsupported = torch.empty(1, dtype=torch.int32, device=dev)
+    _k._launch(dev, "sgf_spmm_code_values", colind, val, nnz, scale, val_coded, n_unsupported)
+    return val_coded, n_unsupported
+
+
+def spmm_coded(rowptr, colind, val, val_coded, x: torch.Tensor, slots, n_unsupported, n_rows: int,
+               long_segments: int = 0) -> torch.Tensor:
+    x = _k._rows(x)
+    d = x.shape[1]
+    y = torch.empty((n_rows, d), dtype=x.dtype, device=x.device)
+    if n_rows == 0 or d == 0:
+        return y
+    _k._launch(x.device, "sgf_spmm_coded", rowptr, colind, val, val_coded, x, x.stride(0), x.shape[0], slots, n_unsupported, y,
+               y.stride(0), n_rows, d, _k._code(x), _k.LONG_ROW, long_segments,
+               *_k._long_row_scratch(x.device, long_segments, d))
+    _k.counters["spmm_coded"] += 1
+    return y
+
+
+def install(table):
+    table.spmm_coded_supported = spmm_coded_supported
+    table.spmm_code_rows = spmm_code_rows
+    table.spmm_code_values = spmm_code_values
+    table.spmm_coded = spmm_coded
+    return table
diff --git a/sgformer_amd/csrc/spmm.hip b/sgformer_amd/csrc/spmm.hip
--- a/sgformer_amd/csrc/spmm.hip
+++ b/sgformer_amd/csrc/spmm.hip
@@ -188,7 +188,7 @@
   int voff;
   uint32_t pitch;
   template <int N> struct Batch { u32x2 raw[N]; };
-  template <int N> __device__ __forceinline__ void request(Batch<N>& b, const int32_t (&c)[N]) const {
+  template <int N> __device__ __forceinline__ void request(Batch<N>& b, const int32_t (&c)[N], const float (&)[N]) const {
 #pragma unroll
     for (int u = 0; u < N; ++u) b.raw[u] = BufRow<uint16_t>::load(rsrc, voff, static_cast<uint32_t>(c[u]) * pitch);
   }
@@ -211,7 +211,7 @@
     uint32_t slot[N], mw[N], pre[N];
     u32x3 raw[N];
   };
-  template <int N> __device__ __forceinline__ void request(Batch<N>& b, const int32_t (&c)[N]) const {
+  template <int N> __device__ __forceinline__ void request(Batch<N>& b, const int32_t (&c)[N], const float (&)[N]) const {
 #pragma unroll
     for (int u = 0; u < N; ++u) {
       b.slot[u] = static_cast<uint32_t>(c[u]) * static_cast<uint32_t>(S);
@@ -258,7 +258,7 @@
     c[u] = colind[e + u];
     v[u] = val[e + u];
   }
-  ld.request(b, c);
+  ld.request(b, c, v);
   ld.follow(b);
   ld.apply(b, v, acc);
 }
@@ -276,7 +276,7 @@
       c0[u] = ci[u];
       v0[u] = va[u];
     }
-    ld.request(ba, c0);
+    ld.request(ba, c0, v0);
     for (;;) {
       i += UNROLL;
       const bool more_a = i + UNROLL <= len;
@@ -288,10 +288,10 @@
         }
       }
       ld.follow(ba);
-      if (L::kAhead && more_a) ld.request(bb, c1);
+      if (L::kAhead && more_a) ld.request(bb, c1, v1);
       ld.apply(ba, v0, acc);
       if (!more_a) break;
-      if (!L::kAhead) ld.request(bb, c1);
+      if (!L::kAhead) ld.request(bb, c1, v1);
       i += UNROLL;
       const bool more_b = i + UNROLL <= len;
       if (more_b) {
@@ -302,10 +302,10 @@
         }
       }
       ld.follow(bb);
-      if (L::kAhead && more_b) ld.request(ba, c0);
+      if (L::kAhead && more_b) ld.request(ba, c0, v0);
       ld.apply(bb, v1, acc);
       if (!more_b) break;
-      if (!L::kAhead) ld.request(ba, c0);
+      if (!L::kAhead) ld.request(ba, c0, v0);
     }
   }
   if (i + 4 <= len) { gather_batch_with<4>(ld, ci, va, i, acc); i += 4; }
@@ -359,6 +359,92 @@
     ld.voff = lane * 8;
     ld.pitch = pitch;
     acc = walk_row<UNROLL>(ld, ci, va, len);
+  }
+  store4<uint16_t>(y + row * ldy + lane * 4, acc);
+}
+
+struct CodedRowLoader {
+  static constexpr bool kAhead = false;
+  __amdgpu_buffer_rsrc_t rc, rx;
+  int voff_w, voff_h, voff_x;
+  uint32_t sel;
+  uint32_t pitch;
+  template <int N> struct Batch { uint32_t w[N], h[N]; };
+  static __device__ __forceinline__ bool escaped(float v) { return (__float_as_uint(v) >> 31) != 0u; }
+  template <int N> __device__ __forceinline__ void request(Batch<N>& b, const int32_t (&c)[N], const float (&v)[N]) const {
+#pragma unroll
+    for (int u = 0; u < N; ++u) {
+      if (escaped(v[u])) {
+        const u32x2 r = BufRow<uint16_t>::load(rx, voff_x, static_cast<uint32_t>(c[u]) * pitch);
+        b.w[u] = r.x;
+        b.h[u] = r.y;
+      } else {
+        const uint32_t slot = static_cast<uint32_t>(c[u]) * static_cast<uint32_t>(kCodedSlot);
+        b.w[u] = __builtin_amdgcn_raw_buffer_load_b32(rc, voff_w, static_cast<int>(slot), 0);
+        b.h[u] = __builtin_amdgcn_raw_buffer_load_b32(rc, voff_h, static_cast<int>(slot), 0);
+      }
+    }
+  }
+  template <int N> __device__ __forceinline__ void follow(Batch<N>&) const {}
+  template <int N> __device__ __forceinline__ void apply(const Batch<N>& b, const float (&v)[N], float4& acc) const {
+#pragma unroll
+    for (int u = 0; u < N; ++u) {
+      float4 f;
+      if (escaped(v[u])) {
+        u32x2 r;
+        r.x = b.w[u];
+        r.y = b.h[u];
+        f = BufRow<uint16_t>::widen(r);
+      } else {
+        const uint32_t w = b.w[u];
+        const uint32_t z = ((w >> 4) & 0x07800780u) | (__builtin_amdgcn_perm(0u, b.h[u], sel) & 0x807f807fu);
+        f.x = __uint_as_float((w << 16) & 0x87ff0000u);
+        f.y = __uint_as_float(w & 0x87ff0000u);
+        f.z = __uint_as_float(z << 16);
+        f.w = __uint_as_float(z & 0xffff0000u);
+      }
+      fma4(acc, __uint_as_float(__float_as_uint(v[u]) & 0x7fffffffu), f);
+    }
+  }
+};
+
+template <int UNROLL>
+__global__ __launch_bounds__(kWavesPerBlock * 64) void k_spmm_row_coded(
+    const int64_t* __restrict__ rowptr, const int32_t* __restrict__ colind, const float* __restrict__ val,
+    const float* __restrict__ val_coded, const uint16_t* __restrict__ x, uint32_t pitch, uint32_t x_bytes,
+    const void* __restrict__ coded, uint32_t coded_bytes, const int32_t* __restrict__ n_unsupported,
+    uint16_t* __restrict__ y, int64_t ldy, int64_t n_rows, LongQueue lq) {
+  const int lane = threadIdx.x & 63;
+  const int wid = __builtin_amdgcn_readfirstlane(static_cast<int>(threadIdx.x >> 6));
+  const int64_t blk = xcd_remap(blockIdx.x, gridDim.x);
+  const int64_t row = blk * kWavesPerBlock + wid;
+  if (row >= n_rows) return;
+  const int64_t e0 = rowptr[row];
+  const int64_t e1 = rowptr[row + 1];
+  if (e1 - e0 > lq.long_len) {
+    push_long_row(lq, row, e1 - e0, lane, 64);
+    return;
+  }
+  const int32_t* __restrict__ ci = colind + e0;
+  const int len = static_cast<int>(e1 - e0);
+  const __amdgpu_buffer_rsrc_t rx = __builtin_amdgcn_make_buffer_rsrc(const_cast<uint16_t*>(x), 0, x_bytes, 0x00020000);
+  float4 acc;
+  if (*n_unsupported == 0) {
+    CodedRowLoader ld;
+    ld.rc = __builtin_amdgcn_make_buffer_rsrc(const_cast<void*>(coded), 0, coded_bytes, 0x00020000);
+    ld.rx = rx;
+    ld.voff_w = lane * 4;
+    ld.voff_h = 256 + (lane >> 1) * 4;
+    ld.voff_x = lane * 8;
+    ld.sel = (lane & 1) ? 0x03030202u : 0x01010000u;
+    ld.pitch = pitch;
+    acc = walk_row<UNROLL>(ld, ci, val_coded + e0, len);
+  } else {
+    DenseRowLoader ld;
+    ld.rsrc = rx;
+    ld.voff = lane * 8;
+    ld.pitch = pitch;
+    acc = walk_row<UNROLL>(ld, ci, val + e0, len);
   }
   store4<uint16_t>(y + row * ldy + lane * 4, acc);
 }
@@ -1280,10 +1366,21 @@
          static_cast<uint64_t>(n_cols) * static_cast<uint64_t>(slot_bytes) + kPackedTail < (static_cast<uint64_t>(1) << 32);
 }
 
+EnvInt g_coded{"SGF_SPMM_CODED", 1};
+struct CodedOperand {
+  const void* slots;
+  const float* val_coded;
+  const int32_t* n_unsupported;
+};
+bool coded_rule(const Choice& c, int32_t d, size_t elem_size, int64_t n_cols) {
+  return g_coded.get() != 0 && c.arm == Arm::Row && elem_size == 2 && d == 256 &&
+         static_cast<uint64_t>(n_cols) * static_cast<uint64_t>(kCodedSlot) < (static_cast<uint64_t>(1) << 32);
+}
+
 template <typename T>
 int launch(const int64_t* rowptr, const int32_t* colind, const float* val, const T* x, int64_t ldx, int64_t n_cols,
            T* y, int64_t ldy, int64_t n_rows, int32_t d, hipStream_t st, const LongQueue& lq,
-           float* partial, bool stream, const PackedOperand* pk = nullptr) {
+           float* partial, bool stream, const PackedOperand* pk = nullptr, const CodedOperand* cd = nullptr) {
   constexpr int UNROLL = 8;
   const dim3 block(kWavesPerBlock * 64);
   uint64_t x_bytes;
@@ -1325,6 +1422,13 @@
 #undef SGF_ROWP
         break;
       }
+      if (cd && coded_rule(c, d, sizeof(T), n_cols)) {
+        hipLaunchKernelGGL((k_spmm_row_coded<UNROLL>), dim3(static_cast<unsigned>(nb)), block, 0, st, rowptr, colind, val,
+                           cd->val_coded, reinterpret_cast<const uint16_t*>(x), static_cast<uint32_t>(ldx * sizeof(T)),
+                           static_cast<uint32_t>(x_bytes), cd->slots, static_cast<uint32_t>(n_cols * kCodedSlot),
+                           cd->n_unsupported, reinterpret_cast<uint16_t*>(y), ldy, n_rows, lq);
+        break;
+      }
       hipLaunchKernelGGL((k_spmm_row<T, UNROLL>), dim3(static_cast<unsigned>(nb)), block, 0, st, rowptr, colind,
                          val, x, static_cast<uint32_t>(ldx * sizeof(T)), static_cast<uint32_t>(x_bytes), y, ldy,
                          n_rows, d, lq);
@@ -1391,7 +1495,8 @@
 
 int spmm_common(const int64_t* rowptr, const int32_t* colind, const float* val, const void* x, int64_t ldx,
                 int64_t n_cols, void* y, int64_t ldy, int64_t n_rows, int32_t d, int32_t dtype, const LongQueue& lq,
-                float* partial, hipStream_t st, const char* fn, bool stream = false, const PackedOperand* pk = nullptr) {
+                float* partial, hipStream_t st, const char* fn, bool stream = false, const PackedOperand* pk = nullptr,
+                const CodedOperand* cd = nullptr) {
   SGF_REQUIRE(n_rows >= 0 && d >= 0 && n_cols >= 0, SGF_E_INVALID, "%s: negative size", fn);
   if (n_rows == 0 || d == 0) return SGF_OK;
   SGF_REQUIRE(rowptr && x && y, SGF_E_INVALID, "%s: null pointer", fn);
@@ -1402,7 +1507,7 @@
     return launch<float>(rowptr, colind, val, static_cast<const float*>(x), ldx, n_cols, static_cast<float*>(y), ldy,
                          n_rows, d, st, lq, partial, stream);
   return launch<uint16_t>(rowptr, colind, val, static_cast<const uint16_t*>(x), ldx, n_cols,
-                          static_cast<uint16_t*>(y), ldy, n_rows, d, st, lq, partial, stream, pk);
+                          static_cast<uint16_t*>(y), ldy, n_rows, d, st, lq, partial, stream, pk, cd);
 }
 }
 
@@ -1493,6 +1598,29 @@
   if (const int rc = spmm_long_queue(fn, long_len, long_segments, d, workspace, workspace_bytes, st, &lq, &partial)) return rc;
   const PackedOperand pk{packed, slot_bytes, overflow};
   return spmm_common(rowptr, colind, val, x, ldx, n_cols, y, ldy, n_rows, d, dtype, lq, partial, st, fn, false, &pk);
+}
+
+extern "C" int32_t sgf_spmm_coded_supported(int32_t d, int32_t dtype, int64_t ldx, int64_t ldy, int64_t n_cols,
+                                            int32_t aligned16) {
+  if (dtype != SGF_F32 && dtype != SGF_BF16) return 0;
+  const size_t esz = dtype == SGF_BF16 ? 2 : 4;
+  const Choice c = choose_for_operands(d, esz, ldx, ldy, n_cols, aligned16 != 0, false);
+  return coded_rule(c, d, esz, n_cols) ? 1 : 0;
+}
+
+extern "C" int sgf_spmm_coded(const int64_t* rowptr, const int32_t* colind, const float* val, const float* val_coded,
+                              const void* x, int64_t ldx, int64_t n_cols, const void* coded, const int32_t* n_unsupported,
+                              void* y, int64_t ldy, int64_t n_rows, int32_t d, int32_t dtype, int64_t long_len,
+                              int64_t long_segments, void* workspace, size_t workspace_bytes, void* stream) {
+  const char* fn = "sgf_spmm_coded";
+  SGF_REQUIRE(coded && val_coded && n_unsupported, SGF_E_INVALID, "%s: null pointer", fn);
+  SGF_REQUIRE(reinterpret_cast<uintptr_t>(coded) % 128 == 0, SGF_E_INVALID, "%s: the coded buffer must be 128-byte aligned", fn);
+  hipStream_t st = static_cast<hipStream_t>(stream);
+  LongQueue lq;
+  float* partial;
+  if (const int rc = spmm_long_queue(fn, long_len, long_segments, d, workspace, workspace_bytes, st, &lq, &partial)) return rc;
+  const CodedOperand cd{coded, val_coded, n_unsupported};
+  return spmm_common(rowptr, colind, val, x, ldx, n_cols, y, ldy, n_rows, d, dtype, lq, partial, st, fn, false, nullptr, &cd);
 }
 
 extern "C" int sgf_spmm_stream(const int64_t* rowptr, const int32_t* colind, const float* val, const void* x,
diff --git a/sgformer_amd/csrc/spmm_coded.hip b/sgformer_amd/csrc/spmm_coded.hip
--- /dev/null
+++ b/sgformer_amd/csrc/spmm_coded.hip
@@ -0,0 +1,198 @@
+#include "common.h"
+#include "spmm_shared.h"
+
+namespace sgf {
+namespace {
+
+constexpr int kRowsPerWave = 4;
+constexpr int kWaves = 4;
+
+__device__ __forceinline__ uint32_t wave_max_uniform(uint32_t v) {
+  auto dpp = [](uint32_t x, auto ctrl, auto row_mask) {
+    return static_cast<uint32_t>(__builtin_amdgcn_update_dpp(0, static_cast<int>(x), decltype(ctrl)::value,
+                                                             decltype(row_mask)::value, 0xf, false));
+  };
+  auto mx = [](uint32_t a, uint32_t b) { return a > b ? a : b; };
+  v = mx(v, dpp(v, std::integral_constant<int, 0x111>{}, std::integral_constant<int, 0xf>{}));
+  v = mx(v, dpp(v, std::integral_constant<int, 0x112>{}, std::integral_constant<int, 0xf>{}));
+  v = mx(v, dpp(v, std::integral_constant<int, 0x114>{}, std::integral_constant<int, 0xf>{}));
+  v = mx(v, dpp(v, std::integral_constant<int, 0x118>{}, std::integral_constant<int, 0xf>{}));
+  v = mx(v, dpp(v, std::integral_constant<int, 0x142>{}, std::integral_constant<int, 0xa>{}));
+  v = mx(v, dpp(v, std::integral_constant<int, 0x143>{}, std::integral_constant<int, 0xc>{}));
+  return static_cast<uint32_t>(__builtin_amdgcn_readlane(static_cast<int>(v), 63));
+}
+
+__global__ __launch_bounds__(kWaves * 64) void k_code_rows(const uint16_t* __restrict__ x, int64_t ldx, int64_t n,
+                                                           uint8_t* __restrict__ coded, uint8_t* __restrict__ scale) {
+  const int lane = threadIdx.x & 63;
+  const int64_t r0 = (static_cast<int64_t>(blockIdx.x) * kWaves + (threadIdx.x >> 6)) * kRowsPerWave;
+  if (r0 >= n) return;
+  uint2 raw[kRowsPerWave];
+#pragma unroll
+  for (int k = 0; k < kRowsPerWave; ++k) {
+    const int64_t r = r0 + k < n ? r0 + k : n - 1;
+    raw[k] = *reinterpret_cast<const uint2*>(x + r * ldx + lane * 4);
+  }
+#pragma unroll
+  for (int k = 0; k < kRowsPerWave; ++k) {
+    if (r0 + k >= n) break;
+    const uint32_t b[4] = {raw[k].x & 0xffffu, raw[k].x >> 16, raw[k].y & 0xffffu, raw[k].y >> 16};
+    uint32_t ek[4], hi = 0, bad = 0;
+#pragma unroll
+    for (int j = 0; j < 4; ++j) {
+      ek[j] = (b[j] >> 7) & 0xffu;
+      bad |= (ek[j] == 255u) | ((ek[j] == 0u) & ((b[j] & 0x7fu) != 0u));
+      hi = ek[j] > hi ? ek[j] : hi;
+    }
+    const uint32_t top = wave_max_uniform(hi);
+    const uint32_t E = top != 0u ? top : 15u;
+#pragma unroll
+    for (int j = 0; j < 4; ++j) bad |= (ek[j] != 0u) & (ek[j] + 14u < E);
+    const bool esc = __ballot(bad != 0) != 0;
+    uint32_t w = 0, h = 0;
+    if (!esc) {
+      uint32_t c[4], e[4];
+#pragma unroll
+      for (int j = 0; j < 4; ++j) {
+        e[j] = ek[j] != 0u ? ek[j] + 15u - E : 0u;
+        c[j] = (b[j] & 0x807fu) | (e[j] << 7);
+      }
+      w = c[0] | (e[2] << 11) | ((c[1] | (e[3] << 11)) << 16);
+      h = ((b[2] >> 8) & 0x80u) | (b[2] & 0x7fu) | ((((b[3] >> 8) & 0x80u) | (b[3] & 0x7fu)) << 8);
+    }
+    uint8_t* slot = coded + (r0 + k) * kCodedSlot;
+    reinterpret_cast<uint32_t*>(slot)[lane] = w;
+    reinterpret_cast<uint16_t*>(slot + 256)[lane] = static_cast<uint16_t>(h);
+    if (lane == 0) scale[r0 + k] = esc ? kCodedEscaped : static_cast<uint8_t>(E);
+  }
+}
+
+constexpr int kCountBytesPerThread = 16;
+
+__global__ __launch_bounds__(256) void k_count_escaped(const uint8_t* __restrict__ scale, int64_t n, int32_t* __restrict__ n_escaped) {
+  const int64_t i = (static_cast<int64_t>(blockIdx.x) * 256 + threadIdx.x) * kCountBytesPerThread;
+  int cnt = 0;
+  if (i + kCountBytesPerThread <= n) {
+    const uint4 q = *reinterpret_cast<const uint4*>(scale + i);
+    const uint32_t w[4] = {q.x, q.y, q.z, q.w};
+#pragma unroll
+    for (int j = 0; j < 4; ++j)
+#pragma unroll
+      for (int b = 0; b < 4; ++b) cnt += ((w[j] >> (8 * b)) & 0xffu) == kCodedEscaped;
+  } else {
+    for (int64_t j = i; j < n; ++j) cnt += scale[j] == kCodedEscaped;
+  }
+#pragma unroll
+  for (int off = 32; off > 0; off >>= 1) cnt += __shfl_xor(cnt, off, 64);
+  __shared__ int part[4];
+  if ((threadIdx.x & 63) == 0) part[threadIdx.x >> 6] = cnt;
+  __syncthreads();
+  if (threadIdx.x == 0) {
+    const int total = part[0] + part[1] + part[2] + part[3];
+    if (total) atomicAdd(n_escaped, total);
+  }
+}
+
+__device__ __forceinline__ float code_value(float v, uint32_t E) {
+  const uint32_t u = __float_as_uint(v);
+  const int ev = static_cast<int>((u >> 23) & 0xffu);
+  const int en = ev + static_cast<int>(E) - 15;
+  const bool ok = (u >> 31) == 0u && ev >= 1 && ev <= 254 && E != kCodedEscaped && en >= 1 && en <= 254;
+  return ok ? __uint_as_float((u & 0x807fffffu) | (static_cast<uint32_t>(en) << 23)) : __uint_as_float(u ^ 0x80000000u);
+}
+
+__device__ __forceinline__ int signbit32(float v) { return static_cast<int>(__float_as_uint(v) >> 31); }
+
+constexpr int kValuesPerThread = 4;
+
+__global__ __launch_bounds__(256) void k_code_values(const int32_t* __restrict__ colind, const float* __restrict__ val,
+                                                     int64_t nnz, const uint8_t* __restrict__ scale,
+                                                     float* __restrict__ val_coded, int32_t* __restrict__ n_unsupported) {
+  const int64_t i = (static_cast<int64_t>(blockIdx.x) * 256 + threadIdx.x) * kValuesPerThread;
+  int neg = 0;
+  if (i + kValuesPerThread <= nnz) {
+    const int4 c = *reinterpret_cast<const int4*>(colind + i);
+    const float4 v = *reinterpret_cast<const float4*>(val + i);
+    const uint32_t e0 = scale[c.x], e1 = scale[c.y], e2 = scale[c.z], e3 = scale[c.w];
+    float4 o;
+    o.x = code_value(v.x, e0);
+    o.y = code_value(v.y, e1);
+    o.z = code_value(v.z, e2);
+    o.w = code_value(v.w, e3);
+    *reinterpret_cast<float4*>(val_coded + i) = o;
+    neg = signbit32(v.x) + signbit32(v.y) + signbit32(v.z) + signbit32(v.w);
+  } else {
+    for (int64_t j = i; j < nnz; ++j) {
+      const float v = val[j];
+      val_coded[j] = code_value(v, scale[colind[j]]);
+      neg += signbit32(v);
+    }
+  }
+  const unsigned long long any = __ballot(neg != 0);
+  if (any) {
+#pragma unroll
+    for (int off = 32; off > 0; off >>= 1) neg += __shfl_xor(neg, off, 64);
+    if ((threadIdx.x & 63) == 0) atomicAdd(n_unsupported, neg);
+  }
+}
+
+}
+}
+
+using namespace sgf;
+
+extern "C" size_t sgf_spmm_coded_bytes(int64_t n) {
+  if (n < 0) return 0;
+  return static_cast<size_t>(n) * kCodedSlot;
+}
+
+extern "C" int sgf_spmm_code_rows(const void* x, int64_t ldx, int64_t n, void* coded, uint8_t* scale_u8, int32_t* n_escaped,
+                                  void* stream) {
+  const char* fn = "sgf_spmm_code_rows";
+  SGF_REQUIRE(n >= 0, SGF_E_INVALID, "%s: negative size", fn);
+  SGF_REQUIRE(n_escaped, SGF_E_INVALID, "%s: null pointer", fn);
+  hipStream_t st = static_cast<hipStream_t>(stream);
+  if (n == 0) {
+    SGF_CHECK_HIP(hipMemsetAsync(n_escaped, 0, sizeof(int32_t), st));
+    return SGF_OK;
+  }
+  SGF_REQUIRE(x && coded && scale_u8, SGF_E_INVALID, "%s: null pointer", fn);
+  SGF_REQUIRE(ldx >= 256 && ldx % 4 == 0 && reinterpret_cast<uintptr_t>(x) % 8 == 0, SGF_E_INVALID,
+              "%s: bf16 rows of 256 columns, ldx a multiple of 4, x 8-byte aligned (ldx=%lld)", fn,
+              static_cast<long long>(ldx));
+  SGF_REQUIRE(reinterpret_cast<uintptr_t>(coded) % 128 == 0, SGF_E_INVALID, "%s: the coded buffer must be 128-byte aligned", fn);
+  SGF_REQUIRE(reinterpret_cast<uintptr_t>(scale_u8) % 16 == 0, SGF_E_INVALID, "%s: scale_u8 must be 16-byte aligned", fn);
+  constexpr int64_t rows_per_block = kWaves * kRowsPerWave;
+  const int64_t nb = (n + rows_per_block - 1) / rows_per_block;
+  SGF_REQUIRE(nb < (static_cast<int64_t>(1) << 31), SGF_E_UNSUPPORTED, "%s: n too large for one launch", fn);
+  SGF_CHECK_HIP(hipMemsetAsync(n_escaped, 0, sizeof(int32_t), st));
+  hipLaunchKernelGGL(k_code_rows, dim3(static_cast<unsigned>(nb)), dim3(kWaves * 64), 0, st, static_cast<const uint16_t*>(x),
+                     ldx, n, static_cast<uint8_t*>(coded), scale_u8);
+  SGF_LAUNCH_CHECK();
+  constexpr int64_t count_per_block = 256 * kCountBytesPerThread;
+  hipLaunchKernelGGL(k_count_escaped, dim3(static_cast<unsigned>((n + count_per_block - 1) / count_per_block)), dim3(256), 0, st,
+                     scale_u8, n, n_escaped);
+  SGF_LAUNCH_CHECK();
+  return SGF_OK;
+}
+
+extern "C" int sgf_spmm_code_values(const int32_t* colind, const float* val, int64_t nnz, const uint8_t* scale_u8,
+                                    float* val_coded, int32_t* n_unsupported, void* stream) {
+  const char* fn = "sgf_spmm_code_values";
+  SGF_REQUIRE(nnz >= 0, SGF_E_INVALID, "%s: negative size", fn);
+  SGF_REQUIRE(n_unsupported, SGF_E_INVALID, "%s: null pointer", fn);
+  hipStream_t st = static_cast<hipStream_t>(stream);
+  SGF_REQUIRE(nnz == 0 || (colind && val && scale_u8 && val_coded), SGF_E_INVALID, "%s: null pointer", fn);
+  SGF_REQUIRE(reinterpret_cast<uintptr_t>(colind) % 16 == 0 && reinterpret_cast<uintptr_t>(val) % 16 == 0 &&
+                  reinterpret_cast<uintptr_t>(val_coded) % 16 == 0,
+              SGF_E_INVALID, "%s: colind, val and val_coded must be 16-byte aligned", fn);
+  constexpr int64_t per_block = 256 * kValuesPerThread;
+  const int64_t nb = (nnz + per_block - 1) / per_block;
+  SGF_REQUIRE(nb < (static_cast<int64_t>(1) << 31), SGF_E_UNSUPPORTED, "%s: nnz too large for one launch", fn);
+  SGF_CHECK_HIP(hipMemsetAsync(n_unsupported, 0, sizeof(int32_t), st));
+  if (nnz == 0) return SGF_OK;
+  hipLaunchKernelGGL(k_code_values, dim3(static_cast<unsigned>(nb)), dim3(256), 0, st, colind, val, nnz, scale_u8, val_coded,
+                     n_unsupported);
+  SGF_LAUNCH_CHECK();
+  return SGF_OK;
+}
diff --git a/sgformer_amd/csrc/spmm_shared.h b/sgformer_amd/csrc/spmm_shared.h
--- a/sgformer_amd/csrc/spmm_shared.h
+++ b/sgformer_amd/csrc/spmm_shared.h
@@ -42,6 +42,9 @@
 typedef uint32_t u32x2 __attribute__((ext_vector_type(2)));
 typedef uint32_t u32x4 __attribute__((ext_vector_type(4)));
 
+constexpr int kCodedSlot = 384;
+constexpr uint8_t kCodedEscaped = 255;
+
 constexpr size_t kLongCountOff = 0, kLongEntriesOff = 256;
 static inline size_t long_partial_off(int64_t long_segments) {
   return kLongEntriesOff + align_up(static_cast<size_t>(long_segments) * sizeof(LongEntry), 256);
diff --git a/sgformer_amd/graph.py b/sgformer_amd/graph.py
--- a/sgformer_amd/graph.py
+++ b/sgformer_amd/graph.py
@@ -8,12 +8,13 @@
 import torch
 
 from . import _lib
+from . import coded as _coded
 from .kernels import HipKernels, LONG_ROW, _SEGMENT
 
 _F32 = torch.float32
 
 
-K = HipKernels()
+K = _coded.install(HipKernels())
 
 
 def _has(table, name: str, *args) -> bool:
@@ -401,19 +402,20 @@
 
 class _SpMM(torch.autograd.Function):
     @staticmethod
-    def forward(ctx, x, graph, shard, packed=None):
+    def forward(ctx, x, graph, shard, packed=None, layer=None):
         K.check(x)
-        ctx.graph, ctx.shard = graph, shard
+        ctx.graph, ctx.shard, ctx.layer = graph, shard, layer
         if shard is not None:
             return _sharded_spmm(graph, x, shard, False)
-        return spmm_on(graph, x, False, packed=packed)
+        return spmm_on(graph, x, False, packed=packed, coded_class=None if layer is None else f"fwd{layer}")
 
     @staticmethod
     def backward(ctx, gy):
         graph, shard = ctx.graph, ctx.shard
         if shard is not None:
-            return _sharded_spmm(graph, gy.contiguous(), shard, True), None, None, None
-        return spmm_on(graph, gy.contiguous(), True), None, None, None
+            return _sharded_spmm(graph, gy.contiguous(), shard, True), None, None, None, None
+        coded_class = None if ctx.layer is None else f"bwd{ctx.layer}"
+        return spmm_on(graph, gy.contiguous(), True, coded_class=coded_class), None, None, None, None
 
 
 def spmm_packed_slot(graph, x_shape, dtype, slot_bytes: int) -> int:
@@ -422,7 +424,26 @@
     return slot_bytes if K.spmm_packed_supported(x_shape, dtype, slot_bytes) else 0
 
 
-def spmm_on(graph, x: torch.Tensor, transposed: bool, out=None, packed=None) -> torch.Tensor:
+CODED_MIN_NODES = 65536
+CODED_CLASSES = frozenset({"fwd2"})
+
+
+def _coded_ok(graph, x: torch.Tensor, out, packed, coded_class) -> bool:
+    return (coded_class in CODED_CLASSES and packed is None and out is None and x.dim() == 2 and x.shape[1] == 256
+            and x.dtype == torch.bfloat16 and x.shape[0] >= CODED_MIN_NODES and x.is_contiguous()
+            and _has(K, "spmm_coded") and not torch.cuda.is_current_stream_capturing()
+            and K.spmm_coded_supported(x.shape, x.dtype))
+
+
+def _spmm_coded(coded_class, rp, ci, va, x: torch.Tensor, n: int, segs: int) -> torch.Tensor:
+    slots, scale, n_escaped = K.spmm_code_rows(x)
+    if _coded.escape_log is not None:
+        _coded.escape_log.append((coded_class, n_escaped, x.shape[0]))
+    val_coded, n_unsupported = K.spmm_code_values(ci, va, scale)
+    return K.spmm_coded(rp, ci, va, val_coded, x, slots, n_unsupported, n, long_segments=segs)
+
+
+def spmm_on(graph, x: torch.Tensor, transposed: bool, out=None, packed=None, coded_class=None) -> torch.Tensor:
     rp, ci, va, segs = graph.arrays(transposed)
     plan = graph.plan(x.dtype, transposed) if (graph.blocked and x.shape[1] <= 256) else None
     if plan is not None:
@@ -436,8 +457,10 @@
         return K.spmm(rp, ci, va, x, graph.n, out=out, long_segments=segs, stream_hint=True)
     if packed is not None and not transposed and out is None:
         return K.spmm_packed(rp, ci, va, x, packed, graph.n, long_segments=segs)
+    if _coded_ok(graph, x, out, packed, coded_class):
+        return _spmm_coded(coded_class, rp, ci, va, x, graph.n, segs)
     return K.spmm(rp, ci, va, x, graph.n, out=out, long_segments=segs)
 
 
-def spmm(graph, x: torch.Tensor, shard=None, packed=None) -> torch.Tensor:
-    return _SpMM.apply(x, graph, shard, packed)
+def spmm(graph, x: torch.Tensor, shard=None, packed=None, layer=None) -> torch.Tensor:
+    return _SpMM.apply(x, graph, shard, packed, layer)
diff --git a/sgformer_amd/kernels.py b/sgformer_amd/kernels.py
--- a/sgformer_amd/kernels.py
+++ b/sgformer_amd/kernels.py
@@ -14,7 +14,7 @@
 LONG_ROW = 1024
 _SEGMENT = 1024
 
-counters = {"spmm_packed": 0}
+counters = {"spmm_packed": 0, "spmm_coded": 0}
 
 
 class PackedRows:
diff --git a/sgformer_amd/ours.py b/sgformer_amd/ours.py
--- a/sgformer_amd/ours.py
+++ b/sgformer_amd/ours.py
@@ -157,7 +157,7 @@
     def reset_parameters(self):
         self.W.reset_parameters()
 
-    def propagate(self, x, edge_index, packed=None):
+    def propagate(self, x, edge_index, packed=None, layer=None):
         shard = self._shard
         if isinstance(edge_index, ops.CSRGraph):
             graph = edge_index
@@ -166,7 +166,7 @@
         else:
             graph = ops.graph_cache.get(edge_index, x.shape[0])
         shard = None if (shard is not None and shard.local_graph) else shard
-        return ops.spmm(graph, x, shard, packed if shard is None else None)
+        return ops.spmm(graph, x, shard, packed if shard is None else None, layer)
 
     def forward(self, x, edge_index, x0, bn_stats=False):
         shard = self._shard
@@ -278,7 +278,7 @@
                 x = x_first
             for i, conv in enumerate(self.convs):
                 bn = self.bns[i + 1]
-                y = conv.propagate(x, edge_index, packed)
+                y = conv.propagate(x, edge_index, packed, i + 1)
                 packed = None
                 req = self.pack_request(i + 1, x0.shape[0], x0.dtype, edge_index) if self.use_act else None
                 x = ops.linear_bn_act_res(y, x0, conv.W.weight, conv.W.bias, bn.weight, bn.bias, _BNBook(self, bn),
```
